# denyingmxd/CFPNet

Hardware: AMD Instinct MI355X
Metric: depth maps/sec @ 480x640 bf16 (whole job; per_gpu = value / n_gpus); abs_rel vs CPU oracle (higher is better)
Workload: dtype bf16; 1 GPU; batch=8 480x640 RGB + 8x8-zone ToF, eval forward incl. the prob output [B,256,H/2,W/2] written in the storage dtype (bf16: 2 bytes/element); layers=hist2image combine1 image x2 (CFPNet), parallelism=single GPU

## Files before the change

### cfpnet_amd/csrc/conv3x3_halo.hip

```cpp
#include "igemm_core.h"

namespace {

__device__ __attribute__((aligned(16))) unsigned int g_zero16h[4] = {0u, 0u, 0u, 0u};

using gptr_t = const __attribute__((address_space(1))) void*;
using lptr_t = __attribute__((address_space(3))) void*;
__device__ __forceinline__ void glds16(const void* g, unsigned char* lds_wave_base) {
  __builtin_amdgcn_global_load_lds((gptr_t)g, (lptr_t)lds_wave_base, 16, 0, 0);
}
template <int N> __device__ __forceinline__ void wait_vmcnt() { asm volatile("s_waitcnt vmcnt(%0)" ::"n"(N) : "memory"); }

struct HaloP {
  int PP;
  int CPT;
  int tiles_x, tiles_y;
  int n_blocks;
  FastDiv dcpt;
};

template <typename H, int NT, int WN, int STAGES, bool UP = false, int STRIDE = 1>
__global__ __launch_bounds__(256, 2) void conv3x3_halo_kernel(ConvP p, HaloP hp) {
  constexpr int WM = 4 / WN;
  constexpr int TH = 4 * WM;
  constexpr int HC = 15 * STRIDE + 3;
  constexpr int HPIX = ((TH - 1) * STRIDE + 3) * HC;
  static_assert(!(UP && STRIDE != 1), "the upsampling loader is stride 1");
  constexpr int NPAD = NT * WN * 16;
  constexpr int NBG = NPAD / 8;
  constexpr int NB = (NBG + 3) / 4;
  constexpr int WSTAGE = NPAD * 128;
  constexpr int LB = UP ? 4 : 6;
  static_assert((STAGES - 2) * NB <= 63, "vmcnt field");
  extern __shared__ __attribute__((aligned(16))) unsigned char smem[];
  unsigned char* sW = smem;
  unsigned char* sX = smem + STAGES * WSTAGE;

  const int tid = threadIdx.x;
  const int lane = tid & 63;
  const int wave = __builtin_amdgcn_readfirstlane(tid >> 6);
  const int wm = wave / WN, wn = wave % WN;
  const int fr = lane & 15, fq = lane >> 4;
  const int rsub = lane >> 3;
  const int lc = (lane & 7) ^ rsub;

  int bid = xcd_remap(blockIdx.x, gridDim.x);
  const int n_base = (bid % hp.n_blocks) * NPAD; bid /= hp.n_blocks;
  const int tx_ = bid % hp.tiles_x; bid /= hp.tiles_x;
  const int ty_ = bid % hp.tiles_y;
  const int b = bid / hp.tiles_y;
  const int x0 = tx_ * 16, y0 = ty_ * TH;

  const H* __restrict__ in = reinterpret_cast<const H*>(p.in) + (long long)b * p.H * p.W * p.in_ld;
  const H* __restrict__ wt = reinterpret_cast<const H*>(p.w);
  const H* zsrc = reinterpret_cast<const H*>(g_zero16h);
  const int nk = (p.K + 63) >> 6;

  const H* b_ptr[NB];
  unsigned b_okmask = 0;
#pragma unroll
  for (int j = 0; j < NB; ++j) {
    const int n = n_base + ((j * 4 + wave) % NBG) * 8 + rsub;
    const bool ok = n < p.Cout;
    if (ok) b_okmask |= 1u << j;
    b_ptr[j] = wt + (long long)(ok ? n : 0) * p.K;
  }
  auto issue = [&](int ks, int buf) {
    unsigned char* s = sW + buf * WSTAGE;
    const int kk = (ks * 8 + lc) * 8;
    const bool kok = kk < p.K;
#pragma unroll
    for (int j = 0; j < NB; ++j) {
      const bool ok = kok && ((b_okmask >> j) & 1u);
      glds16(ok ? b_ptr[j] + kk : zsrc, s + ((j * 4 + wave) % NBG) * 1024);
    }
  };
#pragma unroll
  for (int s = 0; s < STAGES - 1; ++s)
    if (s < nk) issue(s, s);

  {
    const int nitems = HPIX * hp.CPT;
    const H* __restrict__ low = nullptr;
    int upc = 0;
    if constexpr (UP) { low = reinterpret_cast<const H*>(p.up_src) + (long long)b * p.up_H * p.up_W * p.up_ld; upc = p.up_C >> 3; }
    for (int base = 0; base < nitems; base += 256 * LB) {
      u32x4 v[LB][UP ? 4 : 1];
      int dst[LB];
      float lyx[LB][UP ? 2 : 1];
      bool blend[LB];
#pragma unroll
      for (int n = 0; n < LB; ++n) {
        const int i = base + tid + n * 256;
        unsigned upx, uch;
        fd_rowcol((unsigned)i, hp.dcpt, upx, uch);
        const int px = (int)upx, ch = (int)uch;
        const int hy = px / HC, hx = px - hy * HC;
        const int y = y0 * STRIDE - p.pad_t + hy, x = x0 * STRIDE - p.pad_l + hx;
        const bool ok = i < nitems && (unsigned)y < (unsigned)p.H && (unsigned)x < (unsigned)p.W;
        dst[n] = i < nitems ? px * hp.PP + ch * 16 : -1;
        blend[n] = false;
#pragma unroll
        for (int t = 0; t < (UP ? 4 : 1); ++t) v[n][t] = u32x4{0u, 0u, 0u, 0u};
        if constexpr (UP) {
          if (ch < upc) {
            blend[n] = ok;
            const float fy = p.up_sy * (float)y, fx = p.up_sx * (float)x;
            const int ys = (int)fy, xs = (int)fx;
            lyx[n][0] = fy - (float)ys; lyx[n][1] = fx - (float)xs;
            if (ok) {
              const int dyo = (ys < p.up_H - 1 ? 1 : 0) * p.up_W * p.up_ld, dxo = (xs < p.up_W - 1 ? 1 : 0) * p.up_ld;
              const H* s00 = low + (ys * p.up_W + xs) * p.up_ld + ch * 8;
              v[n][0] = *reinterpret_cast<const u32x4*>(s00); v[n][1] = *reinterpret_cast<const u32x4*>(s00 + dxo);
              v[n][2] = *reinterpret_cast<const u32x4*>(s00 + dyo); v[n][3] = *reinterpret_cast<const u32x4*>(s00 + dyo + dxo);
            }
            continue;
          }
        }
        if (ok) v[n][0] = *reinterpret_cast<const u32x4*>(in + (y * p.W + x) * p.in_ld + ch * 8);
      }
#pragma unroll
      for (int n = 0; n < LB; ++n) {
        if (dst[n] < 0) continue;
        if constexpr (UP) {
          if (blend[n]) {
            float t[4][8], o[8];
#pragma unroll
            for (int q = 0; q < 4; ++q) Vec<H>::load(reinterpret_cast<const H*>(&v[n][q]), t[q]);
            const float ly1 = lyx[n][0], lx1 = lyx[n][1], ly0 = 1.f - ly1, lx0 = 1.f - lx1;
#pragma unroll
            for (int e = 0; e < 8; ++e) o[e] = ly0 * (lx0 * t[0][e] + lx1 * t[1][e]) + ly1 * (lx0 * t[2][e] + lx1 * t[3][e]);
            Vec<H>::store(reinterpret_cast<H*>(sX + dst[n]), o);
            continue;
          }
        }
        *reinterpret_cast<u32x4*>(sX + dst[n]) = v[n][0];
      }
    }
  }

  f32x4 acc[4][NT];
#pragma unroll
  for (int g = 0; g < 4; ++g)
#pragma unroll
    for (int j = 0; j < NT; ++j) acc[g][j] = f32x4{0.f, 0.f, 0.f, 0.f};

  const int ntap_chunks = 9 * hp.CPT;
  int c_cc, c_dx = 0, c_off = 0, c_idx = fq;
  {
    const int tap = fq / hp.CPT;
    c_cc = fq - tap * hp.CPT;
    c_dx = tap;
    while (c_dx >= 3) { c_dx -= 3; c_off += HC * hp.PP; }
    c_off += c_dx * hp.PP;
  }
  const unsigned char* xrow = sX + ((wm * 4 * STRIDE) * HC + fr * STRIDE) * hp.PP;
  const int growb = STRIDE * HC * hp.PP;

  for (int ks = 0; ks < nk; ++ks) {
    const int buf = ks % STAGES;
    const int ahead = min(nk - 1 - ks, STAGES - 2);
    if (ahead >= 2) wait_vmcnt<(STAGES > 3 ? 2 : 1) * NB>();
    else if (ahead == 1) wait_vmcnt<NB>();
    else wait_vmcnt<0>();
    asm volatile("s_waitcnt lgkmcnt(0)" ::: "memory");
    __builtin_amdgcn_s_barrier();
    asm volatile("" ::: "memory");
    if (ks + STAGES - 1 < nk) issue(ks + STAGES - 1, (ks + STAGES - 1) % STAGES);
    const unsigned char* cW = sW + buf * WSTAGE + (wn * NT * 16) * 128;
#pragma unroll
    for (int s = 0; s < 2; ++s) {
      s16x8 wf[NT], xf[4];
      const int pc = ((s * 4 + fq) ^ (fr & 7)) * 16;
#pragma unroll
      for (int j = 0; j < NT; ++j) wf[j] = *reinterpret_cast<const s16x8*>(cW + (j * 16 + fr) * 128 + pc);
      const bool live = c_idx < ntap_chunks;
      const int xo = c_off + c_cc * 16;
#pragma unroll
      for (int g = 0; g < 4; ++g) xf[g] = *reinterpret_cast<const s16x8*>(live ? xrow + g * growb + xo : sX);
#pragma unroll
      for (int g = 0; g < 4; ++g)
#pragma unroll
        for (int j = 0; j < NT; ++j) acc[g][j] = mfma16<H>(wf[j], xf[g], acc[g][j]);
      c_idx += 4;
      c_cc += 4;
      while (c_cc >= hp.CPT) {
        c_cc -= hp.CPT;
        c_off += hp.PP;
        if (++c_dx == 3) { c_dx = 0; c_off += (HC - 3) * hp.PP; }
      }
    }
  }

  H* __restrict__ out = reinterpret_cast<H*>(p.out) + (long long)b * p.Ho * p.Wo * p.out_ld;
  const H* __restrict__ res = p.res ? reinterpret_cast<const H*>(p.res) + (long long)b * p.Ho * p.Wo * p.res_ld : nullptr;
  const int x = x0 + fr;
  f32x4 sc[NT], sh[NT];
#pragma unroll
  for (int j = 0; j < NT; ++j) {
    const int n = n_base + (wn * NT + j) * 16 + fq * 4;
    const bool ok = n < p.Cout;
    sc[j] = (ok && p.scale) ? *reinterpret_cast<const f32x4*>(p.scale + n) : f32x4{1.f, 1.f, 1.f, 1.f};
    sh[j] = (ok && p.shift) ? *reinterpret_cast<const f32x4*>(p.shift + n) : f32x4{0.f, 0.f, 0.f, 0.f};
  }
  with_act(p.act, [&](auto A) {
#pragma unroll
    for (int g = 0; g < 4; ++g) {
      const int y = y0 + wm * 4 + g;
      const bool pix_ok = y < p.Ho && x < p.Wo;
      const long long pix = (long long)y * p.Wo + x;
#pragma unroll
      for (int j = 0; j < NT; ++j) {
        const int n = n_base + (wn * NT + j) * 16 + fq * 4;
        float yv[4];
#pragma unroll
        for (int r = 0; r < 4; ++r) yv[r] = act_c16<decltype(A)::value>(acc[g][j][r] * sc[j][r] + sh[j][r]);
        uint2 pk;
        pk.x = pack2<H>(yv[0], yv[1]);
        pk.y = pack2<H>(yv[2], yv[3]);
        if (!(pix_ok && n < p.Cout)) continue;
        if (res) {
          const uint2 rr = *reinterpret_cast<const uint2*>(res + pix * p.res_ld + n);
          const H* ph = reinterpret_cast<const H*>(&pk);
          const H* rh = reinterpret_cast<const H*>(&rr);
          float o[4];
#pragma unroll
          for (int r = 0; r < 4; ++r) o[r] = to_f32<H>(ph[r]) + to_f32<H>(rh[r]);
          H oh[4];
#pragma unroll
          for (int r = 0; r < 4; ++r) oh[r] = from_f32<H>(o[r]);
          pk = *reinterpret_cast<const uint2*>(oh);
        }
        *reinterpret_cast<uint2*>(out + pix * p.out_ld + n) = pk;
      }
    }
  });
}

int g_halo_odd_pitch = 0;
int g_halo_stages = 0;

struct HCfg { int nt, wn; };
constexpr HCfg kHCfg[] = {
    {1, 1},
    {2, 1},
    {4, 1},
    {2, 2},
    {4, 2},
    {5, 2},
    {7, 2},
    {1, 2},
};
constexpr int kNumHCfg = sizeof(kHCfg) / sizeof(kHCfg[0]);

template <typename H, int NT, int WN, bool UP = false, int STRIDE = 1>
int launch_h(const ConvP& p, hipStream_t s) {
  constexpr int TH = 4 * (4 / WN);
  constexpr int NPAD = NT * WN * 16;
  HaloP hp;
  hp.n_blocks = cdiv(p.Cout, NPAD);
  hp.CPT = p.Cin / 8;
  hp.dcpt = make_fastdiv((unsigned)hp.CPT);
  if ((long long)p.H * p.W * p.in_ld >= (1ll << 31)) return -1;
  int slots = hp.CPT;
  if (STRIDE == 1 && hp.CPT > 1) { while ((slots & 3) != 2) ++slots; }
  else if ((slots & 1) == 0) ++slots;
  if (g_halo_odd_pitch) { slots = hp.CPT; if ((slots & 1) == 0) ++slots; }
  hp.PP = slots * 16;
  hp.tiles_x = cdiv(p.Wo, 16); hp.tiles_y = cdiv(p.Ho, TH);
  const int hpix = ((TH - 1) * STRIDE + 3) * (15 * STRIDE + 3);
  const size_t halo = (size_t)hpix * hp.PP;
  const long long tiles = (long long)p.B * hp.tiles_x * hp.tiles_y * hp.n_blocks;
  int stages = g_halo_stages ? g_halo_stages : 2;
  const size_t lds = (size_t)stages * NPAD * 128 + halo;
  if (lds > 160 * 1024 || tiles >= (1ll << 31)) return -1;
#define HL(ST)                                                                                                                      \
  do {                                                                                                                              \
    auto k = conv3x3_halo_kernel<H, NT, WN, ST, UP, STRIDE>;                                                                        \
    static bool attr = false;                                                                                                       \
    if (!attr) { if (hipFuncSetAttribute((const void*)k, hipFuncAttributeMaxDynamicSharedMemorySize, 160 * 1024) != hipSuccess) return -2; attr = true; } \
    hipLaunchKernelGGL(k, dim3((unsigned)tiles), dim3(256), lds, s, p, hp);                                                         \
  } while (0)
  if constexpr (UP || STRIDE != 1) { HL(2); } else { if (stages == 4) HL(4); else if (stages == 3) HL(3); else HL(2); }
#undef HL
  return 0;
}

}

int conv3x3_halo_num_variants() { return kNumHCfg; }
void conv3x3_halo_debug_stages(int v) { g_halo_stages = v; }
void conv3x3_halo_debug_odd_pitch(int v) { g_halo_odd_pitch = v; }

bool conv3x3_halo_takes(const ConvP& p) {
  return p.KH == 3 && p.KW == 3 && (p.stride == 1 || (p.stride == 2 && p.up_src == nullptr)) && p.dil <= 1 && p.Cin % 8 == 0 && p.Cin >= 8 && p.Cin <= 128 && p.Cout % 8 == 0 &&
         p.Cout <= 512 && p.ln_gamma == nullptr && p.rows_per_batch == 0 && p.k2 == 0 && p.K == 9 * p.Cin &&
         p.pad_t >= 0 && p.pad_l >= 0 && p.pad_t <= 2 && p.pad_l <= 2;
}

int conv3x3_halo_launch(int v, const ConvP& p, hipStream_t s) {
  if (v < 0) {
    const long long t16 = (long long)p.B * cdiv(p.Wo, 16) * cdiv(p.Ho, 16);
    if (p.up_src != nullptr && p.Cout > 64) return -3;
    if (p.up_src != nullptr) v = p.Cout <= 32 ? 7 : 3;
    else if (p.Cout <= 16) v = 0;
    else if (p.Cout <= 32) v = t16 >= 1024 ? 1 : 7;
    else if (p.Cout <= 64) v = t16 >= 1024 ? 2 : 3;
    else if (p.Cout <= 128) v = 4;
    else if (p.Cout <= 160) v = 5;
    else v = 4;
  }
  if (v >= kNumHCfg) return -3;
  if (p.up_src != nullptr) {
#define HU(NT, WN) (p.f16 ? launch_h<f16_t, NT, WN, true>(p, s) : launch_h<bf16_t, NT, WN, true>(p, s))
    switch (v) {
      case 0: return HU(1, 1);
      case 1: return HU(2, 1);
      case 2: return HU(4, 1);
      case 3: return HU(2, 2);
      case 7: return HU(1, 2);
      default: return -3;
    }
#undef HU
  }
  if (p.stride == 2) {
#define HS(NT, WN) (p.f16 ? launch_h<f16_t, NT, WN, false, 2>(p, s) : launch_h<bf16_t, NT, WN, false, 2>(p, s))
    switch (v) {
      case 0: return HS(1, 1);
      case 1: return HS(2, 1);
      case 2: return HS(4, 1);
      case 3: return HS(2, 2);
      case 4: return HS(4, 2);
      case 5: return HS(5, 2);
      case 7: return HS(1, 2);
      default: return -3;
    }
#undef HS
  }
#define HV(NT, WN) (p.f16 ? launch_h<f16_t, NT, WN>(p, s) : launch_h<bf16_t, NT, WN>(p, s))
  switch (v) {
    case 0: return HV(1, 1);
    case 1: return HV(2, 1);
    case 2: return HV(4, 1);
    case 3: return HV(2, 2);
    case 4: return HV(4, 2);
    case 5: return HV(5, 2);
    case 6: return HV(7, 2);
    case 7: return HV(1, 2);
    default: return -3;
  }
#undef HV
}
```

### cfpnet_amd/csrc/igemm_core.h

```cpp
#pragma once
#include "common.h"

struct ConvP {
  const void* in;
  const void* w;
  void* out;
  const void* res;
  const float* scale;
  const float* shift;
  int in_ld, out_ld, res_ld;
  int B, H, W, Cin, Ho, Wo, Cout;
  int KH, KW, stride, pad_t, pad_l;
  int M, K;
  int act;
  int pointwise;
  const float* ln_gamma;
  const float* ln_beta;
  float ln_eps;
  int rows_per_batch;
  long long w_bstride;
  int f16;
  int k2;
  const void* up_src;
  int up_ld, up_C, up_H, up_W;
  float up_sy, up_sx;
  int probe;
  float* mom;
  int dil;
};

int igemm2_num_variants();
void igemm2_variant_shape(int v, int* bm, int* bn, int* stages);
int igemm2_launch(int v, const ConvP& p, float* slabs, int splits, hipStream_t s);

int igemm_x3_num_variants();
void igemm_x3_variant_shape(int v, int* bm, int* bn, int* stages);
constexpr int CFP_TICKET_SLOTS = 1024;
int igemm_x3_launch(int v, const ConvP& p, float* slabs, int splits, hipStream_t s, unsigned* tickets = nullptr);
int bin_head_x3_launch(const void* x, int x_ld, const void* w, const float* bias, const float* centers, float* prob, float* pred, int B, int HW,
                       int Cin, hipStream_t s);

int conv3x3_halo_x3_num_variants();
bool conv3x3_halo_x3_takes(const ConvP& p);
size_t conv3x3_halo_x3_lds(int v, const ConvP& p);
int conv3x3_halo_x3_launch(int v, const ConvP& p, hipStream_t s);

int conv3x3_num_variants();
void conv3x3_variant_shape(int v, int* th, int* bn);
int conv3x3_launch(int v, const ConvP& p, hipStream_t s);

int conv3x3_halo_num_variants();
void conv3x3_halo_debug_stages(int v);
void conv3x3_halo_debug_odd_pitch(int v);
bool conv3x3_halo_takes(const ConvP& p);
int conv3x3_halo_launch(int v, const ConvP& p, hipStream_t s);

template <typename T, int BN, int NTHR>
__device__ __forceinline__ void tile_moments(const T* sC, int CP, int rows_valid, int n0, int Cout, float* __restrict__ mom_tile, int tid) {
  constexpr int TPC = NTHR / BN;
  static_assert(NTHR % BN == 0 && TPC >= 1 && TPC <= 64 && (TPC & (TPC - 1)) == 0, "threads per channel");
  const int c = tid / TPC, part = tid % TPC;
  const float shift = to_f32<T>(sC[c]);
  float n = 0.f, s1 = 0.f, s2 = 0.f;
  for (int r = part; r < rows_valid; r += TPC) {
    const float v = to_f32<T>(sC[r * CP + c]) - shift;
    s1 += v; s2 = fmaf(v, v, s2); n += 1.f;
  }
  float mean = n > 0.f ? shift + s1 / n : 0.f;
  float m2 = n > 0.f ? fmaxf(s2 - s1 * s1 / n, 0.f) : 0.f;
#pragma unroll
  for (int o = 1; o < TPC; o <<= 1) {
    const float bn = __shfl_xor(n, o, 64), bmean = __shfl_xor(mean, o, 64), bm2 = __shfl_xor(m2, o, 64);
    const bool up = (part & o) != 0;
    const float an = up ? bn : n, amean = up ? bmean : mean, am2 = up ? bm2 : m2;
    const float cn = up ? n : bn, cmean = up ? mean : bmean, cm2 = up ? m2 : bm2;
    const float tn = an + cn;
    if (tn > 0.f) {
      const float d = cmean - amean, f = cn / tn;
      mean = amean + d * f; m2 = am2 + cm2 + d * d * an * f; n = tn;
    } else { mean = 0.f; m2 = 0.f; n = 0.f; }
  }
  if (part == 0 && n0 + c < Cout) { mom_tile[n0 + c] = mean; mom_tile[Cout + n0 + c] = m2; }
}

__device__ __forceinline__ int swz(int row, int chunk) {
  int q = (row >> 2) & 3;
  int g = (4 - q) & 3;
  return chunk ^ g;
}

template <typename T, int BM, int BN, int WM, int WN>
__device__ __forceinline__ void igemm_mainloop(const ConvP& p, int m0, int n0, int ks_begin, int ks_end,
                                               unsigned char* smem, f32x4 (&acc)[BM / WM / 16][BN / WN / 16]) {
  constexpr int VE = Vec<T>::N;
  constexpr int BK = 4 * VE;
  constexpr int TM = BM / WM / 16;
  constexpr int TN = BN / WN / 16;
  constexpr int A_ROWS = BM / 64;
  constexpr int B_ROWS = (BN + 63) / 64;
  constexpr bool kBf16 = sizeof(T) == 2;
  auto sA = [&](int st) -> unsigned char* { return smem + st * ((BM + BN) * 64); };
  auto sB = [&](int st) -> unsigned char* { return smem + st * ((BM + BN) * 64) + BM * 64; };

  const int tid = threadIdx.x;
  const int lane = tid & 63;
  const int wave = tid >> 6;
  const int wm = wave / WN, wn = wave % WN;

  const T* __restrict__ in = reinterpret_cast<const T*>(p.in);
  const T* __restrict__ wt = reinterpret_cast<const T*>(p.w);

  const int ld_row = tid >> 2;
  const int ld_chunk = tid & 3;
  long long a_base[A_ROWS];
  int a_hi0[A_ROWS], a_wi0[A_ROWS];
  bool a_ok[A_ROWS];
#pragma unroll
  for (int i = 0; i < A_ROWS; ++i) {
    int m = m0 + ld_row + 64 * i;
    a_ok[i] = m < p.M;
    int mm = a_ok[i] ? m : 0;
    if (p.pointwise) {
      a_base[i] = (long long)mm * p.in_ld;
      a_hi0[i] = 0;
      a_wi0[i] = 0;
    } else {
      int wo = mm % p.Wo;
      int t = mm / p.Wo;
      int ho = t % p.Ho;
      int b = t / p.Ho;
      a_hi0[i] = ho * p.stride - p.pad_t;
      a_wi0[i] = wo * p.stride - p.pad_l;
      a_base[i] = (long long)b * p.H * p.W * p.in_ld;
    }
  }
  bool b_ok[B_ROWS];
  long long b_base[B_ROWS];
#pragma unroll
  for (int i = 0; i < B_ROWS; ++i) {
    int r = ld_row + 64 * i;
    int n = n0 + r;
    b_ok[i] = (r < BN) && (n < p.Cout);
    b_base[i] = (long long)(b_ok[i] ? n : 0) * p.K;
  }

  u32x4 ra[A_ROWS], rb[B_ROWS];
  const u32x4 zero4 = {0u, 0u, 0u, 0u};

  int t_k = -1, t_cc = 0, t_kh = 0, t_kw = 0;
  const bool dil_pow2 = (p.dil & (p.dil - 1)) == 0;
  const int dil_shift = 31 - __clz(p.dil);
  auto load_tiles = [&](int k0) {
    int k = k0 + ld_chunk * VE;
    bool kok = k < p.K;
    int kh = 0, kw = 0, cc = k;
    if (!p.pointwise) {
      if (k == t_k + BK && t_k >= 0) {
        t_cc += BK;
        while (t_cc >= p.Cin) {
          t_cc -= p.Cin;
          if (++t_kw == p.KW) { t_kw = 0; ++t_kh; }
        }
      } else {
        int tap = k / p.Cin;
        t_cc = k - tap * p.Cin;
        t_kh = tap / p.KW;
        t_kw = tap - t_kh * p.KW;
      }
      t_k = k;
      cc = t_cc; kh = t_kh; kw = t_kw;
    }
#pragma unroll
    for (int i = 0; i < A_ROWS; ++i) {
      int hi = a_hi0[i] + kh, wi = a_wi0[i] + kw;
      bool ok = a_ok[i] && kok;
      long long off = a_base[i] + cc;
      if (!p.pointwise) {
        if (p.dil > 1 && dil_pow2) {
          ok = ok && hi >= 0 && wi >= 0 && ((hi | wi) & (p.dil - 1)) == 0;
          hi >>= dil_shift; wi >>= dil_shift;
        } else if (p.dil > 1) {
          ok = ok && hi >= 0 && wi >= 0 && hi % p.dil == 0 && wi % p.dil == 0;
          hi /= p.dil; wi /= p.dil;
        }
        ok = ok && hi >= 0 && hi < p.H && wi >= 0 && wi < p.W;
        off += ((long long)hi * p.W + wi) * p.in_ld;
      }
      ra[i] = ok ? *reinterpret_cast<const u32x4*>(in + off) : zero4;
    }
#pragma unroll
    for (int i = 0; i < B_ROWS; ++i) {
      rb[i] = (b_ok[i] && kok) ? *reinterpret_cast<const u32x4*>(wt + b_base[i] + k) : zero4;
    }
  };
  auto store_tiles = [&](int st) {
#pragma unroll
    for (int i = 0; i < A_ROWS; ++i) {
      int r = ld_row + 64 * i;
      *reinterpret_cast<u32x4*>(sA(st) + r * 64 + swz(r, ld_chunk) * 16) = ra[i];
    }
#pragma unroll
    for (int i = 0; i < B_ROWS; ++i) {
      int r = ld_row + 64 * i;
      if (r < BN) *reinterpret_cast<u32x4*>(sB(st) + r * 64 + swz(r, ld_chunk) * 16) = rb[i];
    }
  };

#pragma unroll
  for (int i = 0; i < TM; ++i)
#pragma unroll
    for (int j = 0; j < TN; ++j) acc[i][j] = f32x4{0.f, 0.f, 0.f, 0.f};

  load_tiles(ks_begin * BK);
  store_tiles(0);
  __syncthreads();

  const int fr = lane & 15;
  const int fq = lane >> 4;

  for (int ks = ks_begin; ks < ks_end; ++ks) {
    const int st = (ks - ks_begin) & 1;
    if (ks + 1 < ks_end) load_tiles((ks + 1) * BK);

    const unsigned char* cA = sA(st) + (wm * (BM / WM)) * 64;
    const unsigned char* cB = sB(st) + (wn * (BN / WN)) * 64;
    if constexpr (kBf16) {
      s16x8 af[TM], bfr[TN];
#pragma unroll
      for (int i = 0; i < TM; ++i) {
        int r = i * 16 + fr;
        af[i] = *reinterpret_cast<const s16x8*>(cA + r * 64 + swz(r, fq) * 16);
      }
#pragma unroll
      for (int j = 0; j < TN; ++j) {
        int r = j * 16 + fr;
        bfr[j] = *reinterpret_cast<const s16x8*>(cB + r * 64 + swz(r, fq) * 16);
      }
#pragma unroll
      for (int i = 0; i < TM; ++i)
#pragma unroll
        for (int j = 0; j < TN; ++j)
          acc[i][j] = mfma16<T>(af[i], bfr[j], acc[i][j]);
    } else {
#pragma unroll
      for (int kk = 0; kk < 4; ++kk) {
        float af[TM], bfr[TN];
#pragma unroll
        for (int i = 0; i < TM; ++i) {
          int r = i * 16 + fr;
          af[i] = *reinterpret_cast<const float*>(cA + r * 64 + swz(r, kk) * 16 + fq * 4);
        }
#pragma unroll
        for (int j = 0; j < TN; ++j) {
          int r = j * 16 + fr;
          bfr[j] = *reinterpret_cast<const float*>(cB + r * 64 + swz(r, kk) * 16 + fq * 4);
        }
#pragma unroll
        for (int i = 0; i < TM; ++i)
#pragma unroll
          for (int j = 0; j < TN; ++j)
            acc[i][j] = __builtin_amdgcn_mfma_f32_16x16x4f32(af[i], bfr[j], acc[i][j], 0, 0, 0);
      }
    }
    if (ks + 1 < ks_end) store_tiles(st ^ 1);
    __syncthreads();
  }
}
```

### cfpnet_amd/engine.py

```python
from __future__ import annotations

import math
import os
from typing import Dict, List, Optional, Sequence, Tuple

import torch

from . import hip, ops, spec
from .geometry import FusionGeometry, gsa_keys
from .ops import Act

_BN_EPS = 1e-5


def _same_pad(size: int, k: int, s: int) -> Tuple[int, int]:
    total = max((math.ceil(size / s) - 1) * s + k - size, 0)
    return total // 2, total - total // 2


_STREAMS: Dict = {}
_CONCURRENT: Dict[str, list] = {}


def concurrent_streams(device, want: int = 4, pool: int = 16) -> list:
    import time
    key = str(torch.device(device))
    got = _CONCURRENT.get(key)
    if got is not None and len(got) >= want:
        return got[:want]
    cand = [torch.cuda.Stream(device=device) for _ in range(pool)]
    cycles = 1_000_000
    if not hasattr(torch.cuda, "_sleep"):
        _CONCURRENT[key] = cand[:max(want, 4)]
        return _CONCURRENT[key][:want]

    def spin(ids):
        torch.cuda.synchronize(device)
        t0 = time.perf_counter()
        for i in ids:
            with torch.cuda.stream(cand[i]):
                torch.cuda._sleep(cycles)
        torch.cuda.synchronize(device)
        return time.perf_counter() - t0

    spin([0])
    base = min(spin([0]) for _ in range(3))
    chosen = [0]
    for j in range(1, pool):
        if len(chosen) >= want:
            break
        if all(min(spin([k, j]) for _ in range(2)) < 1.5 * base for k in chosen):
            chosen.append(j)
    _CONCURRENT[key] = [cand[i] for i in chosen]
    return _CONCURRENT[key][:want]


def _shared_stream(device, role):
    key = (str(torch.device(device)), role)
    st = _STREAMS.get(key)
    if st is None:
        if isinstance(role, tuple) and role[0] == "lane":
            conc = concurrent_streams(device)
            st = conc[role[1] % len(conc)]
        else:
            st = torch.cuda.Stream(device=device)
        _STREAMS[key] = st
    return st


class Engine:
    def __init__(self, state_dict: Dict[str, torch.Tensor], *, layer_names: Sequence[str], n_bins: int = 256,
                 min_val: float = 1e-3, max_val: float = 10.0, norm: str = "linear", change_embedding: bool = True,
                 no_skip_inside: bool = False, stem_act: bool = False, dtype=None, device="cuda:0",
                 zone_sample_num: int = 16, base_resolution=spec.BASE_RESOLUTION, x3: Optional[bool] = None):
        if dtype is None:
            dtype, x3 = torch.float32, (True if x3 is None else x3)
        x3 = bool(x3)
        hip.load()
        self.base_resolution = tuple(base_resolution)
        self.fusion = spec.fusion_table(self.base_resolution)
        if not torch.cuda.is_available():
            raise RuntimeError("cfpnet_amd.Engine needs a GPU: the product path has no CPU fallback")
        assert dtype in (torch.bfloat16, torch.float16, torch.float32)
        self.layer_names = list(layer_names)
        self.n_bins, self.min_val, self.max_val = n_bins, float(min_val), float(max_val)
        self.norm = {"linear": 0, "softmax": 1, "sigmoid": 2}[norm]
        self.change_embedding, self.no_skip_inside, self.stem_act = change_embedding, no_skip_inside, stem_act
        self.dtype, self.device = dtype, torch.device(device)
        assert not x3 or dtype == torch.float32, "x3 is a matrix-math mode of float32 storage"
        self.x3 = bool(x3)
        self.cdt = hip.F32X3 if self.x3 else ops.DT[dtype]
        self.tickets = self.x3 and os.environ.get("CFP_SPLITK_TICKETS", "0") == "1"
        self.zone_sample_num = zone_sample_num
        self.weights2 = os.environ.get("CFP_WEIGHTS2", "0") == "1"
        self.diffuse_cin = os.environ.get("CFP_DIFFUSE_CIN", "1") == "1"
        self.mbconv_fused = os.environ.get("CFP_MBCONV_FUSED", "0") == "1"
        self.se2 = dtype in (torch.bfloat16, torch.float16) and os.environ.get("CFP_SE2", "1") == "1"
        self.se2_x3 = os.environ.get("CFP_SE2_X3", "1") if self.x3 else "0"
        self._dbg_round = {}
        for item in filter(None, os.environ.get("CFP_DEBUG_ROUND", "").split(",")):
            n, d = item.split(":")
            self._dbg_round[n] = {"f16": torch.float16, "bf16": torch.bfloat16}[d]
        self.up_fused = os.environ.get("CFP_UP_FUSED", "4")
        self.up_fused_x3 = os.environ.get("CFP_UP_FUSED_X3", "")
        self.cat_pad = os.environ.get("CFP_CAT_PAD", "1") == "1" and not self.up_fused_x3
        self.lkpm_fused = os.environ.get("CFP_LKPM_FUSED", "1") != "0"
        self.tail_q = os.environ.get("CFP_TAIL_Q", "1") == "1"
        self.lkpm_min_rows = int(os.environ.get("CFP_LKPM_MIN_ROWS", "30000"))
        self.sr_ln_fused = os.environ.get("CFP_SR_LN_FUSED", "1") == "1"
        self.head_fused = os.environ.get("CFP_HEAD_FUSED", "1") != "0"
        hl = os.environ.get("CFP_HEAD_HILO", "00")
        self.head_hilo = (hl[0] == "1", hl[1] == "1")
        self.half = dtype in (torch.bfloat16, torch.float16)
        self.ve = 8 if self.half else 4
        self.P: Dict[str, torch.Tensor] = {}
        self._plans: Dict[tuple, dict] = {}
        self._graph = None
        self._splitk_ws: Optional[torch.Tensor] = None
        self._capturing = False
        self._side = _shared_stream(self.device, "side")
        self._lane = 0
        self.use_side_stream = os.environ.get("CFP_NO_SIDE_STREAM", "0") != "1"
        self._lane_streams: Dict[int, Tuple[torch.cuda.Stream, torch.cuda.Stream]] = {}
        self._lanes_active = 1
        self._slots = None
        self._slot_next = 0
        self._lane_ws: Dict[int, torch.Tensor] = {}
        self.load_state_dict(state_dict)

    def _dev(self, t: torch.Tensor, dtype=None) -> torch.Tensor:
        return t.detach().to(device=self.device, dtype=dtype or torch.float32).contiguous()

    def _pack_conv(self, w: torch.Tensor, w2: bool = False) -> torch.Tensor:
        w = w.detach().float()
        if w.dim() == 2:
            w = w[:, :, None, None]
        elif w.dim() == 3:
            w = w[:, :, :, None]
        co, ci, kh, kw = w.shape
        if kh * kw > 1:
            w = ops.round_taps(w, self.dtype)
        cip = (ci + 7) // 8 * 8
        if cip != ci:
            w = torch.nn.functional.pad(w, (0, 0, 0, 0, 0, cip - ci))
        flat = w.permute(0, 2, 3, 1).reshape(co, kh * kw * cip)
        if w2 and self.weights2 and self.half and kh * kw == 1:
            return ops.pack_w2(flat, self.dtype).to(self.device)
        if kh * kw == 1 and self.diffuse_cin and self.dtype == torch.float16:
            flat = ops.round_taps(flat.reshape(co, 1, kh * kw * cip), self.dtype).reshape(co, -1)
        if self.x3:
            return ops.pack_w_x3(self._dev(flat))
        return self._dev(flat, self.dtype)

    def _fold_bn(self, sd, bn: Optional[str], bias: Optional[torch.Tensor], co: int, eps: float):
        if bn is None:
            scale = torch.ones(co)
            shift = bias.detach().float().clone() if bias is not None else torch.zeros(co)
        else:
            g, b = sd[bn + ".weight"].float(), sd[bn + ".bias"].float()
            m, v = sd[bn + ".running_mean"].float(), sd[bn + ".running_var"].float()
            scale = g / torch.sqrt(v + eps)
            shift = b - m * scale
            if bias is not None:
                shift = shift + bias.detach().float() * scale
        return self._dev(scale), self._dev(shift)

    def _conv(self, sd, name: str, wkey: str, bkey: Optional[str] = None, bn: Optional[str] = None, eps: float = _BN_EPS, w2: bool = True):
        w = sd[wkey]
        self.P[name + ".w"] = self._pack_conv(w, w2)
        s, t = self._fold_bn(sd, bn, sd[bkey] if bkey else None, w.shape[0], eps)
        self.P[name + ".s"], self.P[name + ".t"] = s, t

    def _loftr_pack(self, sd, p: str, self_attn: bool):
        D = sd[p + ".q_proj.weight"].shape[0]
        if self_attn:
            self.P[p + ".qkv"] = self._pack_conv(torch.cat([sd[p + ".q_proj.weight"], sd[p + ".k_proj.weight"], sd[p + ".v_proj.weight"]], 0), True)
        else:
            self.P[p + ".q"] = self._pack_conv(sd[p + ".q_proj.weight"], True)
        self.P[p + ".kv"] = self._pack_conv(torch.cat([sd[p + ".k_proj.weight"], sd[p + ".v_proj.weight"]], 0), True)
        self.P[p + ".q1"] = self._pack_conv(sd[p + ".q_proj.weight"])
        self.P[p + ".merge"] = self._pack_conv(sd[p + ".merge.weight"])
        self.P[p + ".mlp0"] = self._pack_conv(sd[p + ".mlp.0.weight"])
        self.P[p + ".mlp2"] = self._pack_conv(sd[p + ".mlp.2.weight"])
        for n in ("norm1", "norm2"):
            self.P[f"{p}.{n}.g"], self.P[f"{p}.{n}.b"] = self._dev(sd[f"{p}.{n}.weight"]), self._dev(sd[f"{p}.{n}.bias"])

    def load_state_dict(self, sd: Dict[str, torch.Tensor]):
        self.P.clear()
        self._graph = None
        e = "img_encoder"
        EPS = spec.ENC_BN_EPS
        self._conv(sd, "stem", f"{e}.conv0.0.weight", bn=f"{e}.conv0.1", eps=EPS)
        self.rgb_hilo = self.half and os.environ.get("CFP_RGB_HILO", "1") == "1"
        if self.rgb_hilo:
            w = self.P["stem.w"].reshape(-1, 9, 8).clone()
            w[:, :, 3:6] = w[:, :, 0:3]
            self.P["stem.w"] = w.reshape(w.shape[0], 72).contiguous()
        for b in spec.ENC_BLOCKS:
            q = f"{e}.{b.prefix}"
            if b.kind == "cn":
                self._conv(sd, q + ".conv", q + ".conv.weight", bn=q + ".bn1", eps=EPS)
            elif b.kind == "er":
                self._conv(sd, q + ".exp", q + ".conv_exp.weight", bn=q + ".bn1", eps=EPS)
                self._conv(sd, q + ".pwl", q + ".conv_pwl.weight", bn=q + ".bn2", eps=EPS)
            else:
                self._conv(sd, q + ".pw", q + ".conv_pw.weight", bn=q + ".bn1", eps=EPS)
                if self.half and self.mbconv_fused and b.stride == 1 and not self.weights2:
                    self.P[q + ".pw.wimg"] = ops.pack_mbconv_pw(self.P[q + ".pw.w"].float().cpu(), self.dtype).to(self.device)
                wd = ops.round_taps(sd[q + ".conv_dw.weight"].float(), self.dtype)
                self.P[q + ".dw.w"] = self._dev(wd.reshape(wd.shape[0], 9).t(), self.dtype)
                self.P[q + ".dw.s"], self.P[q + ".dw.t"] = self._fold_bn(sd, q + ".bn2", None, wd.shape[0], EPS)
                self.P[q + ".se.wr"] = self._dev(sd[q + ".se.conv_reduce.weight"].reshape(b.se_rd, b.mid))
                self.P[q + ".se.br"] = self._dev(sd[q + ".se.conv_reduce.bias"])
                self.P[q + ".se.we_t"] = self._dev(sd[q + ".se.conv_expand.weight"].reshape(b.mid, b.se_rd).t())
                self.P[q + ".se.be"] = self._dev(sd[q + ".se.conv_expand.bias"])
                self._conv(sd, q + ".pwl", q + ".conv_pwl.weight", bn=q + ".bn3", eps=EPS, w2=False)
                self.P[q + ".pwl.w32"] = self._dev(sd[q + ".conv_pwl.weight"].reshape(b.cout, b.mid))
        parts, layout, off = [], [], 0
        for ex in (1, 2, 3):
            q = f"hist_encoder.hist_extractor{ex}.pointnet_encoder"
            for j in (1, 2, 3):
                w = sd[f"{q}.conv{j}.weight"].detach().float()
                w = w.reshape(w.shape[0], -1)
                co, ci = w.shape
                sc, sh = self._fold_bn(sd, f"{q}.bn{j}", sd[f"{q}.conv{j}.bias"], co, _BN_EPS)
                row = []
                for t in (w.reshape(-1), sc.cpu(), sh.cpu()):
                    row.append(off)
                    parts.append(t.reshape(-1).cpu())
                    off += (t.numel() + 3) // 4 * 4
                    if t.numel() % 4:
                        parts.append(torch.zeros(4 - t.numel() % 4))
                layout.append((row[0], row[1], row[2], ci, co))
        self.P["hist.blob"] = self._dev(torch.cat(parts))
        self._hist_layout = layout
        d = "decoder"
        self._conv(sd, d + ".conv4", d + ".conv4.weight", d + ".conv4.bias")
        for i in (1, 2, 3, 4):
            q = f"{d}.up{i}._net"
            if self.x3 and self.cat_pad:
                wfull = sd[q + ".0.weight"]
                cpad = (wfull.shape[1] + 31) // 32 * 32
                self.P[f"{d}.up{i}.a.wpad"] = self._pack_conv(torch.nn.functional.pad(wfull.detach().float(), (0, 0, 0, 0, 0, cpad - wfull.shape[1])))
            self._conv(sd, f"{d}.up{i}.a", q + ".0.weight", q + ".0.bias", bn=q + ".1")
            if self.x3 and str(i) in self.up_fused_x3:
                wfull = sd[q + ".0.weight"].detach().float()
                cup = wfull.shape[1] - spec.DEC_ENC_CH[i]
                self.P[f"{d}.up{i}.a.wcat"] = ops.pack_w_x3_cat(self._dev(wfull.permute(0, 2, 3, 1).contiguous()), cup)
            self._conv(sd, f"{d}.up{i}.b", q + ".3.weight", q + ".3.bias", bn=q + ".4")
        for n in ("conv3", "conv2", "conv1", "conv0"):
            self._conv(sd, f"{d}.{n}", f"{d}.{n}.weight", f"{d}.{n}.bias")
        for name in self.fusion:
            q = f"{d}.{name}"
            self.P[q + ".pe"] = self._dev(sd[q + ".positional_encodings"])
            self.P[q + ".pe2"] = self._dev(sd[q + ".positional_encodings2"])
            for i, ln in enumerate(self.layer_names):
                l = f"{q}.layers.{i}"
                if ln == "hist2image":
                    self._loftr_pack(sd, l, False)
                elif ln == "image":
                    self._loftr_pack(sd, l + ".lga.encoder_layer", True)
                    self._loftr_pack(sd, l + ".gsa.encoder_layer", False)
                    self._conv(sd, l + ".gsa.sr", l + ".gsa.sr.weight", l + ".gsa.sr.bias")
                    self.P[l + ".gsa.norm.g"], self.P[l + ".gsa.norm.b"] = self._dev(sd[l + ".gsa.norm.weight"]), self._dev(sd[l + ".gsa.norm.bias"])
                elif ln == "combine1":
                    t = l + ".transformer_path"
                    self.P[t + ".qkv"] = self._pack_conv(torch.cat([sd[t + ".q_proj.weight"], sd[t + ".k_proj.weight"], sd[t + ".v_proj.weight"]], 0), True)
                    self._conv(sd, t + ".conv1", t + ".conv1.weight", bn=t + ".bn1")
                    self._conv(sd, t + ".conv2", t + ".conv2.weight", bn=t + ".bn2")
                    k = l + ".large_kernel_path"
                    wd = sd[k + ".dwconv2.weight"].float()
                    kk = wd.shape[-1]
                    self.P[k + ".dw.w"] = self._dev(wd[:, 0].transpose(1, 2).reshape(wd.shape[0], kk * kk))
                    if self.half and kk in (7, 15, 31):
                        self.P[k + ".dw.tb"] = ops.toeplitz_bands(wd, self.dtype).to(self.device)
                    elif self.x3 and kk in (7, 15, 31) and os.environ.get("CFP_X3_DWLARGE", "1") != "0":
                        self.P[k + ".dw.tb"] = ops.toeplitz_bands_x3(wd).to(self.device)
                    self.P[k + ".dw.s"], self.P[k + ".dw.t"] = self._fold_bn(sd, k + ".bn1", sd[k + ".dwconv2.bias"], wd.shape[0], _BN_EPS)
                    self.P[k + ".norm.g"], self.P[k + ".norm.b"] = self._dev(sd[k + ".norm.weight"]), self._dev(sd[k + ".norm.bias"])
                    self._conv(sd, k + ".pw1", k + ".pwconv1.weight", k + ".pwconv1.bias")
                    self._conv(sd, k + ".pw2", k + ".pwconv2.weight", k + ".pwconv2.bias")
                else:
                    raise NotImplementedError(ln)
        h = "depth_head"
        w0 = sd[d + ".conv0.weight"].detach().float()
        self.P[d + ".conv0.w32"] = self._dev(w0.permute(0, 2, 3, 1).reshape(w0.shape[0], -1))
        self.P[d + ".conv0.b32"] = self._dev(sd[d + ".conv0.bias"])
        self._conv(sd, h + ".conv3x3", h + ".conv3x3.weight", h + ".conv3x3.bias")
        self.P[h + ".w1x1"] = self._dev(sd[h + ".conv1x1.weight"].reshape(128, 128).t())
        for i in (0, 2, 4):
            self.P[f"{h}.r{i}.w"], self.P[f"{h}.r{i}.b"] = self._dev(sd[f"{h}.regressor.{i}.weight"].t()), self._dev(sd[f"{h}.regressor.{i}.bias"])
        self._conv(sd, "conv_out", "conv_out.0.weight", "conv_out.0.bias", w2=False)
        if self.half and self.n_bins == 256:
            self.P["conv_out.wp"] = ops.permute_wout(sd["conv_out.0.weight"], self.dtype, hilo=self.head_hilo[0],
                                                   diffuse=self.diffuse_cin and self.dtype == torch.float16).to(self.device)

    def _act(self, plan, key: str, rows: int, C: int, ld: Optional[int] = None, zero: bool = False) -> Act:
        bufs = plan["bufs"]
        if key not in bufs:
            bufs[key] = ops.new_act(rows, C, self.dtype, self.device, ld, zero)
        a = bufs[key]
        assert a.rows == rows and a.ld == (ld or C), key
        return Act(a.buf, 0, C)

    def _buf(self, plan, key: str, shape, dtype, zero: bool = False) -> torch.Tensor:
        bufs = plan["bufs"]
        if key not in bufs:
            bufs[key] = (torch.zeros if zero else torch.empty)(shape, dtype=dtype, device=self.device)
        assert tuple(bufs[key].shape) == tuple(shape), key
        return bufs[key]

    def _f32(self, plan, key: str, n: int) -> torch.Tensor:
        bufs = plan["bufs"]
        if key not in bufs:
            bufs[key] = torch.empty(max(n, 1), dtype=torch.float32, device=self.device)
        assert bufs[key].numel() >= n, key
        return bufs[key]

    def _cv(self, name, x: Act, out: Act, B, H, W, k, stride=1, pads=None, act=hip.ACT_NONE, residual=None):
        if pads is None:
            p = (k - 1) // 2
            pt = pl = p
            Ho, Wo = (H + 2 * p - k) // stride + 1, (W + 2 * p - k) // stride + 1
        else:
            (pt, pb), (pl, pr) = pads
            Ho, Wo = (H + pt + pb - k) // stride + 1, (W + pl + pr - k) // stride + 1
        ops.conv2d(x, self.P[name + ".w"], self.P[name + ".s"], self.P[name + ".t"], out, B, H, W, k, k, stride, pt, pl,
                   Ho, Wo, act, residual, self._ws(B * Ho * Wo, out.C, k * k * x.C))
        return Ho, Wo

    def _lin(self, wname, x: Act, out: Act, rows, act=hip.ACT_NONE, residual=None, st: Optional[str] = None, ln=None):
        ops.linear(x, self.P[wname], self.P[st + ".s"] if st else None, self.P[st + ".t"] if st else None, out, rows, act, residual,
                   None if ln is not None else self._ws(rows, out.C, x.C), ln)

    def _ws(self, M: int, Cout: int, K: int) -> Optional[torch.Tensor]:
        need = ops.conv2d_ws_bytes(M, Cout, K, self.cdt)
        if need == 0:
            return None
        if self.tickets:
            need += hip.CONV_TICKET_BYTES
        ws = self._lane_ws.get(self._lane)
        if ws is None or ws.numel() * 4 < need:
            if self._capturing:
                raise RuntimeError("split-K workspace must be sized by a warm-up forward before graph capture")
            if self.tickets:
                ws = ops.ticket_ws(need - hip.CONV_TICKET_BYTES, self.device)
            else:
                ws = torch.empty((need + 3) // 4, dtype=torch.float32, device=self.device)
            self._lane_ws[self._lane] = ws
        return ws

    def _dbg(self, name: str, a: Act):
        if self._dbg_round:
            for pat, dt in self._dbg_round.items():
                if name == pat or (pat.endswith("*") and name.startswith(pat[:-1])):
                    t = a.torch()
                    t.copy_(t.to(dt).to(t.dtype))

    def _encoder(self, plan, rgb: torch.Tensor, B, H, W, taps):
        e = "img_encoder"
        x8 = self._act(plan, "rgb8", B * H * W, 8)
        (ops.rgb_to_nhwc8_hilo if self.rgb_hilo else ops.rgb_to_nhwc8)(rgb, x8, B, H, W)
        pads = (_same_pad(H, 3, 2), _same_pad(W, 3, 2))
        h, w = math.ceil(H / 2), math.ceil(W / 2)
        x = self._act(plan, "stem", B * h * w, spec.ENC_STEM_OUT)
        self._cv("stem", x8, x, B, H, W, 3, 2, pads, hip.ACT_SILU if self.stem_act else hip.ACT_NONE)
        self._dbg("stem", x)
        tap_acts: List[Act] = []
        for bi, b in enumerate(spec.ENC_BLOCKS):
            q = f"{e}.{b.prefix}"
            ho, wo = math.ceil(h / b.stride), math.ceil(w / b.stride)
            pads = (_same_pad(h, 3, b.stride), _same_pad(w, 3, b.stride))
            if bi in spec.ENC_TAPS:
                out = plan["tap_dst"][spec.ENC_TAPS[bi]]
            else:
                out = self._act(plan, f"enc{bi}", B * ho * wo, b.cout)
            res = x if b.skip else None
            if b.kind == "cn":
                self._cv(q + ".conv", x, out, B, h, w, 3, b.stride, pads, hip.ACT_SILU, res)
            elif b.kind == "er":
                mid = self._act(plan, f"enc{bi}.mid", B * ho * wo, b.mid)
                self._cv(q + ".exp", x, mid, B, h, w, 3, b.stride, pads, hip.ACT_SILU)
                self._dbg(f"enc{bi}.mid", mid)
                self._cv(q + ".pwl", mid, out, B, ho, wo, 1, 1, None, hip.ACT_NONE, res)
            else:
                mid2 = self._act(plan, f"enc{bi}.dw", B * ho * wo, b.mid)
                mbp = ops.mbconv_plan(B, h, w, x.C, b.mid) if (q + ".pw.wimg") in self.P else None
                if mbp is not None:
                    ns = mbp[0]
                    part = self._f32(plan, f"enc{bi}.sum", B * ns * b.mid)
                    ops.mbconv_expand_dw(x, self.P[q + ".pw.wimg"], self.P[q + ".pw.s"], self.P[q + ".pw.t"], self.P[q + ".dw.w"],
                                         self.P[q + ".dw.s"], self.P[q + ".dw.t"], mid2, part, B, h, w)
                elif ((self.se2 or self.se2_x3 == "1" or (self.se2_x3 == "auto" and not ops.PLAN_IN_FLIGHT)) and b.se_rd <= 64
                      and ops.dwconv3x3_se_parts(B, ho, wo, b.mid, b.stride, ops.DT[self.dtype]) > 0):
                    mid = self._act(plan, f"enc{bi}.mid", B * h * w, b.mid)
                    self._cv(q + ".pw", x, mid, B, h, w, 1, 1, None, hip.ACT_SILU)
                    K = ops.dwconv3x3_se_parts(B, ho, wo, b.mid, b.stride, ops.DT[self.dtype])
                    hpart = self._f32(plan, f"enc{bi}.hpart", B * K * b.se_rd)
                    ops.dwconv3x3_se(mid, self.P[q + ".dw.w"], self.P[q + ".dw.s"], self.P[q + ".dw.t"], mid2, self.P[q + ".se.wr"], hpart,
                                     B, h, w, b.stride, pads[0][0], pads[1][0], ho, wo, hip.ACT_SILU)
                    if self.x3:
                        wb = self._buf(plan, f"enc{bi}.wb", (B, b.cout, (b.mid + 31) // 32 * 64), torch.float16, zero=True)
                    else:
                        wb = self._buf(plan, f"enc{bi}.wb", (B, b.cout, b.mid), self.dtype)
                    ops.se_gate_fold2(hpart, K, 1.0 / (ho * wo), self.P[q + ".se.br"], self.P[q + ".se.we_t"], self.P[q + ".se.be"],
                                      self.P[q + ".pwl.w32"], wb, B, b.cout, b.mid, b.se_rd, x3=self.x3)
                    ops.conv2d(mid2, wb, self.P[q + ".pwl.s"], self.P[q + ".pwl.t"], out, B, ho, wo, 1, 1, 1, 0, 0, ho, wo, hip.ACT_NONE,
                               res, self._piw_ws(plan, bi, B, ho * wo, b.cout, b.mid), per_image_weights=True)
                    x, h, w = out, ho, wo
                    if bi in spec.ENC_TAPS:
                        tap_acts.append(out)
                        if taps is not None:
                            taps[f"enc{spec.ENC_TAPS[bi]}"] = self._nchw(out, B, h, w)
                    continue
                else:
                    mid = self._act(plan, f"enc{bi}.mid", B * h * w, b.mid)
                    self._cv(q + ".pw", x, mid, B, h, w, 1, 1, None, hip.ACT_SILU)
                    ns = ops.dwconv3x3_strips(B, ho, wo, b.mid, b.stride, ops.DT[self.dtype])
                    part = self._f32(plan, f"enc{bi}.sum", B * ns * b.mid)
                    self._dbg(f"enc{bi}.mid", mid)
                    ops.dwconv3x3_sum(mid, self.P[q + ".dw.w"], self.P[q + ".dw.s"], self.P[q + ".dw.t"], mid2, part, B, h, w, b.stride,
                                      pads[0][0], pads[1][0], ho, wo, hip.ACT_SILU)
                    self._dbg(f"enc{bi}.dw", mid2)
                if self.x3:
                    wb = self._buf(plan, f"enc{bi}.wb", (B, b.cout, (b.mid + 31) // 32 * 64), torch.float16, zero=True)
                else:
                    wb = self._buf(plan, f"enc{bi}.wb", (B, b.cout, b.mid), self.dtype)
                ops.se_gate_fold(part, ns, 1.0 / (ho * wo), self.P[q + ".se.wr"], self.P[q + ".se.br"], self.P[q + ".se.we_t"],
                                 self.P[q + ".se.be"], self.P[q + (".pwl.w32" if self.x3 else ".pwl.w")], wb, B, b.cout, b.mid, b.se_rd)
                ops.conv2d(mid2, wb, self.P[q + ".pwl.s"], self.P[q + ".pwl.t"], out, B, ho, wo, 1, 1, 1, 0, 0, ho, wo, hip.ACT_NONE,
                           res, self._piw_ws(plan, bi, B, ho * wo, b.cout, b.mid), per_image_weights=True)
            self._dbg(f"enc{bi}", out)
            x, h, w = out, ho, wo
            if bi in spec.ENC_TAPS:
                tap_acts.append(out)
                if taps is not None:
                    taps[f"enc{spec.ENC_TAPS[bi]}"] = self._nchw(out, B, h, w)
        return tap_acts

    def _hist_encoder(self, plan, hist: torch.Tensor, R: int, taps):
        outs = [self._act(plan, f"hist.{ex}", R, c) for ex, c in zip((1, 2, 3), spec.HIST_CHANNELS)]
        self._hist_pe_fused = taps is None and os.environ.get("CFP_NO_PE_FUSE", "0") != "1"
        pe = [self.P[f"decoder.cross_atten{ex}.pe2"] for ex in (1, 2, 3)] if self._hist_pe_fused else (None, None, None)
        ops.hist_encoder(hist.reshape(-1), self.P["hist.blob"], self._hist_layout, outs, R, pe, self.zone_sample_num)
        if taps is not None:
            for ex, o in enumerate(outs):
                taps[f"hist{ex}"] = o.torch().float().cpu()
        return outs

    def _kv_state(self, plan, tag, p, src: Act, rows_s, D, heads, kvmode: dict):
        d = D // heads
        kvb = self._act(plan, f"{tag}.kvsrc", rows_s, 2 * D)
        self._lin(p + ".kv", src, kvb, rows_s)
        G = kvmode["groups"]
        kv = self._f32(plan, f"{tag}.kv", G * heads * d * d)
        ks = self._f32(plan, f"{tag}.ks", G * heads * d)
        nws = ops.attn_kv_ws_floats(kvmode["NB"], kvmode["Hk"], kvmode["Wk"], kvmode["th"], kvmode["tw"], heads, d)
        ws = self._f32(plan, f"{tag}.kvws", nws)
        ops.attn_kv_reduce(kvb.slice(0, D), kvb.slice(D, D), kv, ks, ws, kvmode["NB"], kvmode["Hk"], kvmode["Wk"], kvmode["th"], kvmode["tw"],
                           kvmode["clip"], kvmode["count_pad"], kvmode["v_length"], heads, d)
        return kv, ks

    def _loftr(self, plan, tag, p, xb: Act, rows_q, src: Optional[Act], rows_s, heads, out: Act, kvmode: dict, apmode: dict, pre=None):
        D = xb.C // 2
        d = D // heads
        x = xb.slice(0, D)
        qb = self._act(plan, f"{tag}.qkv", rows_q, 3 * D)
        fused_tail = self.half or (self.x3 and os.environ.get("CFP_X3_TAIL", "1") != "0")
        tail_q = fused_tail and self.tail_q
        if pre is not None and tail_q:
            kv, ks = pre
            ops.loftr_tail(None, kv, ks, x, out, self.P[p + ".q1"], self.P[p + ".merge"], self.P[p + ".mlp0"], self.P[p + ".mlp2"],
                           (self.P[p + ".norm1.g"], self.P[p + ".norm1.b"]), (self.P[p + ".norm2.g"], self.P[p + ".norm2.b"]),
                           apmode["NB"], apmode["Hq"], apmode["Wq"], apmode["qth"], apmode["qtw"], kvmode["v_length"], heads)
            return
        if src is None and tail_q:
            self._lin(p + ".kv", x, qb.slice(D, 2 * D), rows_q)
            kA, vA = qb.slice(D, D), qb.slice(2 * D, D)
        elif src is None:
            self._lin(p + ".qkv", x, qb, rows_q)
            kA, vA = qb.slice(D, D), qb.slice(2 * D, D)
        else:
            if not tail_q:
                self._lin(p + ".q", x, qb.slice(0, D), rows_q)
            kvb = self._act(plan, f"{tag}.kvsrc", rows_s, 2 * D)
            self._lin(p + ".kv", src, kvb, rows_s)
            kA, vA = kvb.slice(0, D), kvb.slice(D, D)
        G = kvmode["groups"]
        kv = self._f32(plan, f"{tag}.kv", G * heads * d * d)
        ks = self._f32(plan, f"{tag}.ks", G * heads * d)
        nws = ops.attn_kv_ws_floats(kvmode["NB"], kvmode["Hk"], kvmode["Wk"], kvmode["th"], kvmode["tw"], heads, d)
        ws = self._f32(plan, f"{tag}.kvws", nws)
        ops.attn_kv_reduce(kA, vA, kv, ks, ws, kvmode["NB"], kvmode["Hk"], kvmode["Wk"], kvmode["th"], kvmode["tw"],
                           kvmode["clip"], kvmode["count_pad"], kvmode["v_length"], heads, d)
        if fused_tail:
            ops.loftr_tail(None if tail_q else qb.slice(0, D), kv, ks, x, out, self.P[p + ".q1"] if tail_q else None,
                           self.P[p + ".merge"], self.P[p + ".mlp0"], self.P[p + ".mlp2"],
                           (self.P[p + ".norm1.g"], self.P[p + ".norm1.b"]), (self.P[p + ".norm2.g"], self.P[p + ".norm2.b"]),
                           apmode["NB"], apmode["Hq"], apmode["Wq"], apmode["qth"], apmode["qtw"], kvmode["v_length"], heads)
            return
        msg = self._act(plan, f"{tag}.msg", rows_q, D)
        ops.attn_apply(qb.slice(0, D), kv, ks, msg, apmode["NB"], apmode["Hq"], apmode["Wq"], apmode["qth"], apmode["qtw"],
                       (0, 0, 0, 0), kvmode["v_length"], heads, d)
        self._lin(p + ".merge", msg, xb.slice(D, D), rows_q, ln=(self.P[p + ".norm1.g"], self.P[p + ".norm1.b"], 1e-5))
        hid = self._act(plan, f"{tag}.hid", rows_q, 2 * D)
        self._lin(p + ".mlp0", xb, hid, rows_q, hip.ACT_RELU)
        self._lin(p + ".mlp2", hid, out, rows_q, residual=x, ln=(self.P[p + ".norm2.g"], self.P[p + ".norm2.b"], 1e-5))

    def _piw_ws(self, plan, bi: int, B: int, hw: int, cout: int, k: int):
        if not self.x3:
            return None
        _, sp = ops.conv2d_plan(B * hw, cout, k, hip.F32X3, hw, B, 1, 1)
        if sp <= 1:
            return None
        if not self.tickets:
            return self._f32(plan, f"enc{bi}.piw_ws", sp * B * hw * cout)
        bufs, key = plan["bufs"], f"enc{bi}.piw_ws"
        if key not in bufs:
            bufs[key] = ops.ticket_ws(sp * B * hw * cout * 4, self.device)
        return bufs[key]

    def _fusion(self, plan, name: str, x: Act, feat1: Act, zone_valid: torch.Tensor, geo: FusionGeometry, B, H, W, out: Act,
                pos_offset, taps):
        D, (Hm, Wm), lk = self.fusion[name]
        p = f"decoder.{name}"
        ws = spec.window_size((Hm, Wm))
        M = B * H * W
        Z = geo.zone_num * geo.zone_num
        N = self.zone_sample_num
        tok = [self._act(plan, f"{name}.tokA", M, 2 * D), self._act(plan, f"{name}.tokB", M, 2 * D)]
        cur = 0
        if torch.is_tensor(pos_offset):
            assert pos_offset.dtype == torch.int32 and pos_offset.numel() == 2 and pos_offset.is_cuda
            d0 = tok[0].slice(0, D)
            hip.call("cfp_add_rowtable_dev", x.ptr, x.ld, self.P[p + ".pe"].data_ptr(), d0.ptr, d0.ld, M, x.C, H, W, Hm, Wm,
                     pos_offset.data_ptr(), x.dt, hip.current_stream())
        else:
            oy, ox = pos_offset
            ops.add_rowtable(x, self.P[p + ".pe"], tok[0].slice(0, D), M, H, W, Wm, oy, ox)
        emb0 = None
        if not self.change_embedding:
            emb0 = self._act(plan, f"{name}.emb0", M, D)
            ops.copy_rows(tok[0].slice(0, D), emb0, M)
        if self._hist_pe_fused:
            src = feat1
        else:
            src = self._act(plan, f"{name}.src", B * Z * N, D)
            ops.add_rowtable(feat1, self.P[p + ".pe2"], src, B * Z * N, 1, N, N, 0, 0)
        gh, gw = geo.grid_h, geo.grid_w
        Mz = B * gh * gw
        y0, y1, x0, x1 = geo.clipped(H, W)
        rect = (geo.sy_wo, geo.sx_wo, geo.tzh, geo.tzw)

        last = len(self.layer_names) - 1
        direct_out = False
        for i, ln in enumerate(self.layer_names):
            l = f"{p}.layers.{i}"
            tag = f"{name}.L{i}"
            final_dst = out if (i == last and taps is None and os.environ.get("CFP_NO_DIRECT_OUT", "0") != "1") else None
            if ln == "hist2image":
                zin = self._act(plan, f"{name}.zin", Mz, 2 * D)
                zsrc = tok[cur].slice(0, D) if self.change_embedding else emb0
                ops.resize_bilinear(zsrc, H, W, rect, zin.slice(0, D), gh, gw, (0, 0, gh, gw), B)
                zout = self._act(plan, f"{name}.zout", Mz, D)
                self._loftr(plan, f"{name}.x2i", l, zin, Mz, src, B * Z * N, spec.X2I_HEADS, zout,
                            dict(groups=B * Z, NB=B * Z, Hk=1, Wk=N, th=1, tw=N, clip=(0, 1, 0, N), count_pad=False, v_length=float(N)),
                            dict(NB=B, Hq=gh, Wq=gw, qth=geo.p1, qtw=geo.p2), pre=plan.get("x2i_kv", {}).get((name, i)))
                ops.resize_bilinear(zout, gh, gw, (0, 0, gh, gw), tok[cur].slice(0, D), H, W, rect, B, zone_valid=zone_valid,
                                    zn=geo.zone_num, p1=geo.p1, p2=geo.p2, accumulate=not self.no_skip_inside)
            elif ln == "image":
                nh, nw = math.ceil(H / ws), math.ceil(W / ws)
                self._loftr(plan, f"{name}.lsa", l + ".lga.encoder_layer", tok[cur], M, None, 0, spec.TWINS_HEADS, tok[cur ^ 1].slice(0, D),
                            dict(groups=B * nh * nw, NB=B, Hk=H, Wk=W, th=ws, tw=ws, clip=(0, H, 0, W), count_pad=True, v_length=float(ws * ws)),
                            dict(NB=B, Hq=H, Wq=W, qth=ws, qtw=ws))
                cur ^= 1
                hk, wk = gsa_keys(H, W, ws)
                keys = self._act(plan, f"{name}.gsa.keys", B * hk * wk, D)
                if self.x3 and self.sr_ln_fused:
                    ops.conv2d(tok[cur].slice(0, D), self.P[l + ".gsa.sr.w"], self.P[l + ".gsa.sr.s"], self.P[l + ".gsa.sr.t"], keys,
                               B, H, W, ws, ws, ws, 0, 0, hk, wk, ws=self._ws(B * hk * wk, D, ws * ws * D),
                               ln=(self.P[l + ".gsa.norm.g"], self.P[l + ".gsa.norm.b"], 1e-5))
                else:
                    kraw = self._act(plan, f"{name}.gsa.kraw", B * hk * wk, D)
                    ops.conv2d(tok[cur].slice(0, D), self.P[l + ".gsa.sr.w"], self.P[l + ".gsa.sr.s"], self.P[l + ".gsa.sr.t"], kraw,
                               B, H, W, ws, ws, ws, 0, 0, hk, wk, ws=self._ws(B * hk * wk, D, ws * ws * D))
                    ops.layernorm(kraw, self.P[l + ".gsa.norm.g"], self.P[l + ".gsa.norm.b"], 1e-5, keys, B * hk * wk)
                S = hk * wk
                self._loftr(plan, f"{name}.gsa", l + ".gsa.encoder_layer", tok[cur], M, keys, B * S, spec.TWINS_HEADS,
                            final_dst if final_dst is not None else tok[cur ^ 1].slice(0, D),
                            dict(groups=B, NB=B, Hk=1, Wk=S, th=1, tw=S, clip=(0, 1, 0, S), count_pad=False, v_length=float(S)),
                            dict(NB=B, Hq=H, Wq=W, qth=H, qtw=W))
                cur ^= 1
                direct_out = final_dst is not None
            elif ln == "combine1":
                t = l + ".transformer_path"
                heads = spec.X2I_HEADS
                d = D // heads
                xin = tok[cur]
                qb = self._act(plan, f"{name}.dapm.qkv", M, 3 * D)
                self._lin(t + ".qkv", xin.slice(0, D), qb, M)
                n_in = (y1 - y0) * (x1 - x0)
                kv = self._f32(plan, f"{name}.dapm.kv", B * heads * d * d)
                ks = self._f32(plan, f"{name}.dapm.ks", B * heads * d)
                wsb = self._f32(plan, f"{name}.dapm.ws", ops.attn_kv_ws_floats(B, H, W, H, W, heads, d))
                ops.attn_kv_reduce(qb.slice(D, D), qb.slice(2 * D, D), kv, ks, wsb, B, H, W, H, W, (y0, y1, x0, x1), False,
                                   float(max(n_in, 1)), heads, d)
                ops.attn_apply(qb.slice(0, D), kv, ks, xin.slice(D, D), B, H, W, H, W, (y0, y1, x0, x1), float(max(n_in, 1)), heads, d)
                c1 = self._act(plan, f"{name}.dapm.c1", M, D)
                self._cv(t + ".conv1", xin, c1, B, H, W, 3)
                self._cv(t + ".conv2", c1, tok[cur ^ 1].slice(0, D), B, H, W, 3, residual=xin.slice(0, D))
                cur ^= 1
                k = l + ".large_kernel_path"
                xin = tok[cur]
                t1 = self._act(plan, f"{name}.lk.t1", M, D)
                if (k + ".dw.tb") in self.P:
                    ops.dwconv_large_mfma(xin.slice(0, D), self.P[k + ".dw.tb"], self.P[k + ".dw.s"], self.P[k + ".dw.t"], t1, B, H, W, lk,
                                          hip.ACT_RELU)
                else:
                    ops.dwconv_large(xin.slice(0, D), self.P[k + ".dw.w"], self.P[k + ".dw.s"], self.P[k + ".dw.t"], t1, B, H, W, lk, hip.ACT_RELU)
                lk_dst = final_dst if final_dst is not None else tok[cur ^ 1].slice(0, D)
                if ((self.half and not self.weights2) or (self.x3 and os.environ.get("CFP_X3_TAIL", "1") != "0")) and self.lkpm_fused and D in (32, 64, 128) and M >= self.lkpm_min_rows:
                    ops.lkpm_tail(t1, xin.slice(0, D), lk_dst, self.P[k + ".pw1.w"], self.P[k + ".pw1.t"], self.P[k + ".pw2.w"], self.P[k + ".pw2.t"],
                                  self.P[k + ".norm.g"], self.P[k + ".norm.b"], M)
                else:
                    t2 = self._act(plan, f"{name}.lk.t2", M, D)
                    ops.layernorm(t1, self.P[k + ".norm.g"], self.P[k + ".norm.b"], 1e-6, t2, M)
                    h4 = self._act(plan, f"{name}.lk.h4", M, 4 * D)
                    self._lin(k + ".pw1.w", t2, h4, M, hip.ACT_GELU, None, k + ".pw1")
                    self._lin(k + ".pw2.w", h4, lk_dst, M, hip.ACT_NONE, xin.slice(0, D), k + ".pw2")
                cur ^= 1
                direct_out = final_dst is not None
            else:
                raise NotImplementedError(ln)
            if taps is not None:
                taps[f"{p}.layers.{i}"] = tok[cur].slice(0, D).torch().float().cpu().reshape(B, H * W, D)
        if not direct_out:
            ops.copy_rows(tok[cur].slice(0, D), out, M)

    def _nchw(self, a: Act, B, H, W) -> torch.Tensor:
        return a.torch().float().cpu().reshape(B, H, W, a.C).permute(0, 3, 1, 2).contiguous()

    @torch.no_grad()
    def forward_lanes(self, input_data: dict, lanes: int, *, return_prob: bool = True, pos_offsets: Optional[dict] = None):
        rgb = input_data["rgb"]
        B = rgb.shape[0]
        lanes = max(1, min(lanes, B))
        if lanes == 1:
            return self.forward(input_data, return_prob=return_prob, pos_offsets=pos_offsets)
        dev = self.device
        add = input_data["additional"]
        H, W = rgb.shape[-2:]
        edges = torch.empty(B, self.n_bins + 1, dtype=torch.float32, device=dev)
        pred = torch.empty(B, 1, H // 2, W // 2, dtype=torch.float32, device=dev)
        prob = torch.empty(B, self.n_bins, H // 2, W // 2, dtype=self.dtype, device=dev) if return_prob else None
        main = torch.cuda.current_stream(dev)
        bounds = [B * i // lanes for i in range(lanes + 1)]
        for i in range(lanes):
            if i not in self._lane_streams and i > 0:
                self._lane_streams[i] = (_shared_stream(dev, ("lane", i)), _shared_stream(dev, ("lane-side", i)))
        rgb_d = rgb.to(device=dev, dtype=torch.float32).contiguous()
        hist_d = add["hist_data"].to(device=dev, dtype=torch.float32).contiguous()
        mask_d = add["mask"].to(device=dev).to(torch.uint8).contiguous()
        self._lanes_active = lanes
        for i in range(lanes):
            b0, b1 = bounds[i], bounds[i + 1]
            sub = {"rgb": rgb_d[b0:b1], "additional": {"hist_data": hist_d[b0:b1], "mask": mask_d[b0:b1],
                                                       "rect_data": add.get("rect_data"), "patch_info": add["patch_info"]}}
            outs = (edges[b0:b1], pred[b0:b1], prob[b0:b1] if prob is not None else None)
            if i == 0:
                self.forward(sub, return_prob=return_prob, pos_offsets=pos_offsets, lane=0, out=outs)
            else:
                st = self._lane_streams[i][0]
                st.wait_stream(main)
                with torch.cuda.stream(st):
                    self.forward(sub, return_prob=return_prob, pos_offsets=pos_offsets, lane=i, out=outs)
        for i in range(1, lanes):
            main.wait_stream(self._lane_streams[i][0])
        self._lane = 0
        self._lanes_active = 1
        return edges, pred, prob

    def capture(self, input_data: dict, *, return_prob: bool = True, pos_offsets: Optional[dict] = None, lanes: int = 1,
                inflight: int = 1, adopt_inputs: bool = False):
        dev = self.device
        add = input_data["additional"]
        B = input_data["rgb"].shape[0]
        H, W = input_data["rgb"].shape[-2:]
        lanes = max(1, min(lanes, B))
        self._slots = None
        self._slot_next = 0
        if inflight > 1:
            return self._capture_inflight(input_data, inflight, return_prob, pos_offsets)
        if adopt_inputs:
            assert lanes == 1, "adopt_inputs: single-graph capture only"
            m = add["mask"]
            for t, dts in ((input_data["rgb"], (torch.float32,)), (add["hist_data"], (torch.float32,)), (m, (torch.uint8, torch.bool))):
                assert t.device == dev and t.dtype in dts and t.is_contiguous(), "adopt_inputs: device tensors in the kernels' own types"
            static = {"rgb": input_data["rgb"], "additional": {"hist_data": add["hist_data"], "mask": m.view(torch.uint8) if m.dtype == torch.bool else m,
                                                               "rect_data": add.get("rect_data"), "patch_info": add["patch_info"]}}
        else:
            static = {"rgb": input_data["rgb"].to(device=dev, dtype=torch.float32).contiguous().clone(),
                      "additional": {"hist_data": add["hist_data"].to(device=dev, dtype=torch.float32).contiguous().clone(),
                                     "mask": add["mask"].to(device=dev).to(torch.uint8).contiguous().clone(),
                                     "rect_data": add.get("rect_data"), "patch_info": add["patch_info"]}}
        edges = torch.empty(B, self.n_bins + 1, dtype=torch.float32, device=dev)
        pred = torch.empty(B, 1, H // 2, W // 2, dtype=torch.float32, device=dev)
        prob = torch.empty(B, self.n_bins, H // 2, W // 2, dtype=self.dtype, device=dev) if return_prob else None
        bounds = [B * i // lanes for i in range(lanes + 1)]
        subs, outs = [], []
        for i in range(lanes):
            b0, b1 = bounds[i], bounds[i + 1]
            sa = static["additional"]
            subs.append({"rgb": static["rgb"][b0:b1], "additional": {"hist_data": sa["hist_data"][b0:b1], "mask": sa["mask"][b0:b1],
                                                                     "rect_data": sa["rect_data"], "patch_info": sa["patch_info"]}})
            outs.append((edges[b0:b1], pred[b0:b1], prob[b0:b1] if prob is not None else None))
            if i not in self._lane_streams:
                self._lane_streams[i] = (_shared_stream(dev, ("lane", i)), _shared_stream(dev, ("lane-side", i)))
        graphs = []
        self._graph = None
        self._lanes_active = lanes
        cur = torch.cuda.current_stream(dev)
        for i in range(lanes):
            st = self._lane_streams[i][0]
            st.wait_stream(cur)
            with torch.cuda.stream(st):
                for _ in range(2):
                    self.forward(subs[i], return_prob=return_prob, pos_offsets=pos_offsets, lane=i, out=outs[i])
            torch.cuda.synchronize(dev)
            g = torch.cuda.CUDAGraph()
            self._capturing = True
            try:
                with torch.cuda.graph(g, stream=st):
                    self.forward(subs[i], return_prob=return_prob, pos_offsets=pos_offsets, lane=i, out=outs[i])
            finally:
                self._capturing = False
            graphs.append(g)
        torch.cuda.synchronize(dev)
        self._lane = 0
        self._lanes_active = 1
        self._graph = (graphs, static, (edges, pred, prob))
        return edges, pred, prob

    def plan_mode(self, throughput: bool):
        ops.PLAN_IN_FLIGHT = bool(throughput) and os.environ.get("CFP_TPUT_PLAN", "1") != "0"

    def _capture_inflight(self, input_data, inflight, return_prob, pos_offsets):
        self.plan_mode(True)
        try:
            return self._capture_inflight_impl(input_data, inflight, return_prob, pos_offsets)
        finally:
            self.plan_mode(False)

    def _capture_inflight_impl(self, input_data, inflight, return_prob, pos_offsets):
        dev = self.device
        add = input_data["additional"]
        B = input_data["rgb"].shape[0]
        H, W = input_data["rgb"].shape[-2:]
        streams = concurrent_streams(dev, want=inflight)
        self._graph = None
        self._lanes_active = max(2, len(streams))
        cur = torch.cuda.current_stream(dev)
        slots = []
        for si, st in enumerate(streams):
            static = {"rgb": input_data["rgb"].to(device=dev, dtype=torch.float32).contiguous().clone(),
                      "additional": {"hist_data": add["hist_data"].to(device=dev, dtype=torch.float32).contiguous().clone(),
                                     "mask": add["mask"].to(device=dev).to(torch.uint8).contiguous().clone(),
                                     "rect_data": add.get("rect_data"), "patch_info": add["patch_info"]}}
            out = (torch.empty(B, self.n_bins + 1, dtype=torch.float32, device=dev),
                   torch.empty(B, 1, H // 2, W // 2, dtype=torch.float32, device=dev),
                   torch.empty(B, self.n_bins, H // 2, W // 2, dtype=self.dtype, device=dev) if return_prob else None)
            st.wait_stream(cur)
            with torch.cuda.stream(st):
                for _ in range(2):
                    self.forward(static, return_prob=return_prob, pos_offsets=pos_offsets, lane=si, out=out)
            torch.cuda.synchronize(dev)
            g = torch.cuda.CUDAGraph()
            self._capturing = True
            try:
                with torch.cuda.graph(g, stream=st):
                    self.forward(static, return_prob=return_prob, pos_offsets=pos_offsets, lane=si, out=out)
            finally:
                self._capturing = False
            slots.append({"graph": g, "static": static, "out": out, "stream": st, "event": torch.cuda.Event()})
        torch.cuda.synchronize(dev)
        self._lane = 0
        self._lanes_active = 1
        self._slots = slots
        return slots[0]["out"]

    def replay_async(self, input_data: Optional[dict] = None):
        dev = self.device
        cur = torch.cuda.current_stream(dev)
        if not self._slots:
            out = self.replay(input_data)
            ev = torch.cuda.Event()
            ev.record(cur)
            return out, ev
        slot = self._slots[self._slot_next % len(self._slots)]
        self._slot_next += 1
        st = slot["stream"]
        with torch.cuda.stream(st):
            if input_data is not None:
                st.wait_stream(cur)
                static = slot["static"]
                static["rgb"].copy_(input_data["rgb"], non_blocking=True)
                static["additional"]["hist_data"].copy_(input_data["additional"]["hist_data"], non_blocking=True)
                static["additional"]["mask"].copy_(input_data["additional"]["mask"].to(torch.uint8), non_blocking=True)
            slot["graph"].replay()
            slot["event"].record(st)
        return slot["out"], slot["event"]

    def capture_best(self, input_data: dict, *, return_prob: bool = True, pos_offsets: Optional[dict] = None,
                     candidates: Sequence = (("lanes", 1), ("inflight", 2), ("inflight", 3), ("inflight", 4), ("inflight", 6)),
                     reps: int = 16, allow_inflight: bool = True):
        import time
        B = input_data["rgb"].shape[0]
        times = {}
        seen = []
        for kind, n in candidates:
            n = max(1, int(n))
            if kind == "lanes":
                n = min(n, B)
            elif not allow_inflight:
                continue
            if (kind, n) in seen:
                continue
            seen.append((kind, n))
            last = f"{kind}:{n}"
            if kind == "lanes":
                self.capture(input_data, return_prob=return_prob, pos_offsets=pos_offsets, lanes=n)
                run = self.replay
            else:
                self.capture(input_data, return_prob=return_prob, pos_offsets=pos_offsets, inflight=n)
                if len(self._slots) < n:
                    continue
                run = self.replay_async
            for _ in range(2 * n + 2):
                run()
            torch.cuda.synchronize(self.device)
            t0 = time.perf_counter()
            for _ in range(reps):
                run()
            torch.cuda.synchronize(self.device)
            times[f"{kind}:{n}"] = (time.perf_counter() - t0) / reps * 1e3
        best = min(times, key=times.get)
        kind, n = best.split(":")
        n = int(n)
        if best != last:
            if kind == "lanes":
                self.capture(input_data, return_prob=return_prob, pos_offsets=pos_offsets, lanes=n)
            else:
                self.capture(input_data, return_prob=return_prob, pos_offsets=pos_offsets, inflight=n)
        return (kind, n), times

    def replay(self, input_data: Optional[dict] = None):
        if self._slots:
            out, ev = self.replay_async(input_data)
            torch.cuda.current_stream(self.device).wait_event(ev)
            return out
        if self._graph is None:
            raise RuntimeError("Engine.replay() before capture()")
        graphs, static, out = self._graph
        dev = self.device
        cur = torch.cuda.current_stream(dev)
        if input_data is not None:
            static["rgb"].copy_(input_data["rgb"], non_blocking=True)
            static["additional"]["hist_data"].copy_(input_data["additional"]["hist_data"], non_blocking=True)
            m = input_data["additional"]["mask"]
            if m.dtype == torch.bool and m.is_cuda:
                static["additional"]["mask"].view(torch.bool).copy_(m, non_blocking=True)
            else:
                static["additional"]["mask"].copy_(m.to(torch.uint8), non_blocking=True)
        if len(graphs) == 1:
            st = self._lane_streams[0][0]
            st.wait_stream(cur)
            with torch.cuda.stream(st):
                graphs[0].replay()
            cur.wait_stream(st)
            return out
        for i, g in enumerate(graphs):
            st = self._lane_streams[i][0]
            st.wait_stream(cur)
            with torch.cuda.stream(st):
                g.replay()
        for i in range(len(graphs)):
            cur.wait_stream(self._lane_streams[i][0])
        return out

    def _plan(self, B, H, W) -> dict:
        key = (B, H, W, self._lane)
        if key not in self._plans:
            self._plans[key] = {"bufs": {}}
        return self._plans[key]

    @torch.no_grad()
    def forward(self, input_data: dict, *, return_prob: bool = True, pos_offsets: Optional[dict] = None,
                taps: Optional[dict] = None, img_features: Optional[Sequence[torch.Tensor]] = None, lane: int = 0,
                out: Optional[tuple] = None):
        self._lane = lane
        side = self._lane_streams[lane][1] if lane in self._lane_streams else self._side
        if not self.use_side_stream or self._lanes_active > 1:
            side = torch.cuda.current_stream(self.device)
        rgb = input_data["rgb"]
        add = input_data["additional"]
        B, _, H, W = rgb.shape
        assert H % 32 == 0 and W % 32 == 0, "input height/width must be multiples of 32"
        dev = self.device
        plan = self._plan(B, H, W)
        pos_offsets = pos_offsets or {}
        hs = [H // 2, H // 4, H // 8, H // 16, H // 32]
        wsz = [W // 2, W // 4, W // 8, W // 16, W // 32]
        e, c = spec.DEC_ENC_CH, spec.DEC_CH
        cp = (lambda n: (n + 31) // 32 * 32) if (self.x3 and self.cat_pad) else (lambda n: n)
        zc = self.x3 and self.cat_pad
        cat = [None,
               self._act(plan, "cat1", B * hs[3] * wsz[3], cp(c[0] + e[1]), zero=zc),
               self._act(plan, "cat2", B * hs[2] * wsz[2], cp(c[1] + e[2]), zero=zc),
               self._act(plan, "cat3", B * hs[1] * wsz[1], cp(c[2] + e[3]), zero=zc),
               self._act(plan, "cat4", B * hs[0] * wsz[0], cp(c[3] + e[4]), zero=zc)]
        b4 = self._act(plan, "tap4", B * hs[4] * wsz[4], e[0])
        plan["tap_dst"] = [cat[4].slice(c[3], e[4]), cat[3].slice(c[2], e[3]), cat[2].slice(c[1], e[2]),
                           cat[1].slice(c[0], e[1]), b4]
        main = torch.cuda.current_stream(dev)
        hist = add["hist_data"].to(device=dev, dtype=torch.float32).contiguous()
        zone_valid = add["mask"].to(device=dev).to(torch.uint8).contiguous()
        Z, N = hist.shape[1], hist.shape[2]
        side.wait_stream(main)
        with torch.cuda.stream(side):
            hfeat = self._hist_encoder(plan, hist, B * Z * N, taps)
            plan["x2i_kv"] = {}
            if (self.half or (self.x3 and os.environ.get("CFP_X3_TAIL", "1") != "0")) and self.tail_q and self._hist_pe_fused and os.environ.get("CFP_X2I_HOIST", "1") == "1":
                for fname, feat in (("cross_atten3", hfeat[2]), ("cross_atten2", hfeat[1]), ("cross_atten1", hfeat[0])):
                    D = self.fusion[fname][0]
                    for i, ln in enumerate(self.layer_names):
                        if ln == "hist2image":
                            plan["x2i_kv"][(fname, i)] = self._kv_state(
                                plan, f"{fname}.x2i{i}", f"decoder.{fname}.layers.{i}", feat, B * Z * N, D, spec.X2I_HEADS,
                                dict(groups=B * Z, NB=B * Z, Hk=1, Wk=N, th=1, tw=N, clip=(0, 1, 0, N), count_pad=False, v_length=float(N)))
        if img_features is not None:
            for f, dst in zip(img_features, plan["tap_dst"]):
                dst.torch().copy_(f.permute(0, 2, 3, 1).reshape(-1, f.shape[1]).to(device=dev, dtype=self.dtype))
        else:
            self._encoder(plan, rgb.to(device=dev, dtype=torch.float32).contiguous(), B, H, W, taps)

        pinfo = add["patch_info"]

        def fuse(name, x, feat, hh, ww, out):
            Wm = self.fusion[name][1][1]
            geo = FusionGeometry.from_patch_info(pinfo, self.base_resolution[1] / Wm)
            assert geo.zone_num * geo.zone_num == Z
            self._fusion(plan, name, x, feat, zone_valid, geo, B, hh, ww, out, pos_offsets.get(name, (0, 0)), taps)

        def up(i, src: Act, hs_, ws_, hd, wd):
            M = B * hd * wd
            t1 = self._act(plan, f"up{i}.a", M, c[i])
            fits = hd > 1 and wd > 1 and B * hd * wd * cat[i].ld * 2 < 2 ** 31 - 65536 and hs_ * ws_ * src.ld * 2 < 2 ** 31 - 65536
            if self.x3 and str(i) in self.up_fused_x3 and src.C % 32 == 0 and taps is None and hd > 1 and wd > 1:
                n = f"decoder.up{i}.a"
                ops.upsample_cat_conv3x3(src, hs_, ws_, cat[i].slice(src.C, e[i]), self.P[n + ".wcat"], self.P[n + ".s"], self.P[n + ".t"],
                                         t1, B, hd, wd, hip.ACT_LRELU, x3=True)
            elif self.half and str(i) in self.up_fused and src.C % 64 == 0 and taps is None and fits:
                n = f"decoder.up{i}.a"
                ops.upsample_cat_conv3x3(src, hs_, ws_, cat[i].slice(src.C, e[i]), self.P[n + ".w"], self.P[n + ".s"], self.P[n + ".t"],
                                         t1, B, hd, wd, hip.ACT_LRELU)
            else:
                ops.resize_bilinear(src, hs_, ws_, (0, 0, hs_, ws_), cat[i].slice(0, src.C), hd, wd, (0, 0, hd, wd), B)
                n = f"decoder.up{i}.a"
                if (n + ".wpad") in self.P and M >= 30000:
                    ops.conv2d(cat[i], self.P[n + ".wpad"], self.P[n + ".s"], self.P[n + ".t"], t1, B, hd, wd, 3, 3, 1, 1, 1, hd, wd, hip.ACT_LRELU,
                               None, self._ws(M, t1.C, 9 * cat[i].C))
                else:
                    self._cv(n, cat[i].slice(0, src.C + e[i]), t1, B, hd, wd, 3, act=hip.ACT_LRELU)
            t2 = self._act(plan, f"up{i}.b", M, c[i])
            self._cv(f"decoder.up{i}.b", t1, t2, B, hd, wd, 3, act=hip.ACT_LRELU)
            return t2

        main.wait_stream(side)
        xd4 = self._act(plan, "xd4", B * hs[4] * wsz[4], c[0])
        self._cv("decoder.conv4", b4, xd4, B, hs[4], wsz[4], 1)
        x = xd4
        ph, pw = hs[4], wsz[4]
        for i, (fname, feat) in enumerate((("cross_atten3", hfeat[2]), ("cross_atten2", hfeat[1]), ("cross_atten1", hfeat[0])), start=1):
            hh, ww = hs[4 - i], wsz[4 - i]
            t = up(i, x, ph, pw, hh, ww)
            if taps is not None:
                taps[f"up{i}"] = self._nchw(t, B, hh, ww)
            D = c[i + 1]
            dcat = self._act(plan, f"dcat{i}", B * hh * ww, 2 * D)
            self._cv(f"decoder.conv{4 - i}", t, dcat.slice(0, D), B, hh, ww, 1)
            fuse(fname, dcat.slice(0, D), feat, hh, ww, dcat.slice(D, D))
            if taps is not None:
                taps[f"conv{4 - i}"] = self._nchw(dcat.slice(0, D), B, hh, ww)
                taps[fname] = self._nchw(dcat.slice(D, D), B, hh, ww)
            x, ph, pw = dcat, hh, ww
        t = up(4, x, ph, pw, hs[0], wsz[0])
        Mh = B * hs[0] * wsz[0]
        HWh = hs[0] * wsz[0]
        unet = self._act(plan, "unet", Mh, 128)
        fused_head = self.half and self.head_fused and self.n_bins == 256 and HWh % 16 == 0 and HWh >= 128 and "conv_out.wp" in self.P
        ram = self._act(plan, "ram", Mh, 128) if (not fused_head or taps is not None) else None
        edges = out[0] if out is not None else torch.empty(B, self.n_bins + 1, dtype=torch.float32, device=dev)
        centers = self._f32(plan, "head.centers", B * self.n_bins)
        h = "depth_head"
        ns = max(1, min(64, HWh // 256))
        bsum = self._f32(plan, "head.bsum", B * ns * t.C)
        msum = self._f32(plan, "head.msum", B * 128)
        if os.environ.get("CFP_OLD_SUMS", "0") == "1":
            self._cv("decoder.conv0", t, unet, B, hs[0], wsz[0], 3)
        side.wait_stream(main)
        with torch.cuda.stream(side):
            ops.channel_sum(t, bsum, B, HWh, ns)
            ops.conv3x3_mean(bsum, ns, t, self.P["decoder.conv0.w32"], self.P["decoder.conv0.b32"], msum, B, hs[0], wsz[0], 128)
            ops.bin_regressor(msum, 1, 1.0 / HWh, self.P[h + ".w1x1"], self.P[h + ".r0.w"], self.P[h + ".r0.b"], self.P[h + ".r2.w"],
                              self.P[h + ".r2.b"], self.P[h + ".r4.w"], self.P[h + ".r4.b"], self.min_val, self.max_val, self.norm,
                              edges, centers, B, 128, 256, self.n_bins)
        if os.environ.get("CFP_OLD_SUMS", "0") != "1":
            self._cv("decoder.conv0", t, unet, B, hs[0], wsz[0], 3)
        if not fused_head:
            self._cv("depth_head.conv3x3", unet, ram, B, hs[0], wsz[0], 3)
        main.wait_stream(side)
        pred = out[1] if out is not None else torch.empty(B, 1, hs[0], wsz[0], dtype=torch.float32, device=dev)
        if out is not None:
            prob = out[2] if return_prob else None
        else:
            prob = torch.empty(B, self.n_bins, hs[0], wsz[0], dtype=self.dtype, device=dev) if return_prob else None
        if fused_head:
            ops.depth_head_fused(unet, self.P[h + ".conv3x3.w"], self.P[h + ".conv3x3.s"], self.P[h + ".conv3x3.t"], self.P["conv_out.wp"],
                                 self.P["conv_out.t"], centers, prob, pred, B, hs[0], wsz[0], ram_out=ram, ram_hilo=self.head_hilo[1])
        elif (self.half or self.x3) and self.n_bins == 256 and HWh % 8 == 0 and os.environ.get("CFP_BIN_HEAD_FUSED", "1") != "0":
            ops.bin_head_fused(ram, self.P["conv_out.w"], self.P["conv_out.t"], centers, prob, pred, B, HWh)
        else:
            logits = self._act(plan, "logits", Mh, self.n_bins)
            self._lin("conv_out.w", ram, logits, Mh, hip.ACT_NONE, None, "conv_out")
            ops.bin_softmax(logits, centers, prob, pred, B, HWh, self.n_bins)
        if taps is not None:
            taps["unet_out"] = self._nchw(unet, B, hs[0], wsz[0])
            taps["ram"] = self._nchw(ram, B, hs[0], wsz[0])
        return edges, pred, prob
```

### cfpnet_amd/hip.py

```python
from __future__ import annotations

import ctypes as C
import os
from typing import Optional

_HERE = os.path.dirname(os.path.abspath(__file__))
LIB_PATH = os.environ.get("CFP_HIP_LIB") or os.path.join(_HERE, "libcfpnet_hip.so")

F32, BF16, F16 = 0, 1, 2
F32X3 = 3
ACT_NONE, ACT_RELU, ACT_LRELU, ACT_SILU, ACT_GELU, ACT_SIGMOID = range(6)
TOF_SAMPLE_UNIFORM, TOF_SAMPLE_ICDF = 0, 1
HEAD_WOUT_HILO, HEAD_RAM_HILO = 1, 2
CONV_PER_IMAGE, CONV_W2, CONV_IN_FLIGHT, CONV_X3, CONV_WS_TICKETS = 1, 2, 4, 8, 16
CONV_TICKET_BYTES = 4096

_p, _i, _f, _sz, _ll = C.c_void_p, C.c_int, C.c_float, C.c_size_t, C.c_longlong

SIGNATURES = {
    "cfp_version": (_i, []),
    "cfp_last_error": (C.c_char_p, []),
    "cfp_conv2d_nhwc": (_i, [_p, _i, _p, _p, _p, _p, _i, _p, _i] + [_i] * 14 + [_p, _sz, _p]),
    "cfp_conv2d_nhwc_ex": (_i, [_p, _i, _p, _p, _p, _p, _i, _p, _i] + [_i] * 14 + [_p, _p, _f, _i, _p, _sz, _p]),
    "cfp_conv2d_nhwc_moments": (_i, [_p, _i, _p, _p, _p, _i] + [_i] * 13 + [_p, _sz, _p, _sz, _p, _p, _p]),
    "cfp_conv2d_ws_bytes": (_sz, [_i, _i, _i, _i]),
    "cfp_pack_w_x3_elems": (_sz, [_ll, _i]),
    "cfp_pack_w_x3": (_i, [_p, _p, _ll, _i, _p]),
    "cfp_conv2d_plan": (_i, [_i] * 8 + [_p, _p]),
    "cfp_debug_set": (_i, [_i, _i]),
    "cfp_conv2d_variant": (_i, [_i, _i]),
    "cfp_dwconv3x3_nhwc": (_i, [_p, _i, _p, _p, _p, _p, _i] + [_i] * 11 + [_p]),
    "cfp_dwconv3x3_strips": (_i, [_i] * 6),
    "cfp_dwconv3x3_launch_slots": (_i, [_i] * 10),
    "cfp_dwconv3x3_sum_nhwc": (_i, [_p, _i, _p, _p, _p, _p, _i, _p] + [_i] * 11 + [_p]),
    "cfp_se_fold": (_i, [_p, _p, _p, _p, _p, _i, _i, _i, _i, _i, _p]),
    "cfp_se_gate_fold": (_i, [_p, _i, _f, _p, _p, _p, _p, _p, _p, _i, _i, _i, _i, _i, _p]),
    "cfp_dwconv3x3_se_parts": (_i, [_i, _i, _i, _i, _i, _i]),
    "cfp_dwconv3x3_se_nhwc": (_i, [_p, _i, _p, _p, _p, _p, _i, _p, _i, _p] + [_i] * 11 + [_p]),
    "cfp_se_gate_fold2": (_i, [_p, _i, _f, _p, _p, _p, _p, _p, _i, _i, _i, _i, _i, _p]),
    "cfp_dwconv_large_nhwc": (_i, [_p, _i, _p, _p, _p, _p, _i] + [_i] * 7 + [_p]),
    "cfp_dwconv_large_toeplitz_elems": (_sz, [_i, _i]),
    "cfp_dwconv_large_toeplitz": (_i, [_p, _p, _i, _i, _i, _i, _p]),
    "cfp_dwconv_large_mfma_nhwc": (_i, [_p, _i, _p, _p, _p, _p, _i] + [_i] * 7 + [_p]),
    "cfp_channel_sum": (_i, [_p, _i, _p, _i, _i, _i, _i, _i, _p]),
    "cfp_se_hidden": (_i, [_p, _i, _f, _p, _p, _p, _i, _i, _i, _p]),
    "cfp_se_scale": (_i, [_p, _i, _p, _p, _p, _i, _i, _i, _i, _i, _p]),
    "cfp_scale_channels": (_i, [_p, _i, _p, _i, _i, _i, _i, _p]),
    "cfp_layernorm": (_i, [_p, _i, _p, _p, _f, _p, _i, _p, _i, _i, _i, _i, _p]),
    "cfp_attn_kv_ws_floats": (_sz, [_i] * 7),
    "cfp_attn_kv_reduce": (_i, [_p, _i, _p, _i, _p, _p, _p] + [_i] * 10 + [_f, _i, _i, _i, _p]),
    "cfp_attn_apply": (_i, [_p, _i, _p, _p, _p, _i] + [_i] * 9 + [_f, _f, _i, _i, _i, _p]),
    "cfp_loftr_tail": (_i, [_p, _i, _p, _p, _p, _i, _p, _i, _p, _p, _p, _p, _p, _p, _p, _p, _f] + [_i] * 5 + [_f, _f, _i, _i, _i, _p]),
    "cfp_resize_bilinear": (_i, [_p, _i] + [_i] * 6 + [_p, _i] + [_i] * 6 + [_p] + [_i] * 7 + [_p]),
    "cfp_add_rowtable": (_i, [_p, _i, _p, _p, _i] + [_i] * 8 + [_p]),
    "cfp_upsample_cat_conv3x3": (_i, [_p, _i, _i, _i, _i, _p, _i, _i, _p, _p, _p, _p, _i] + [_i] * 6 + [_p]),
    "cfp_copy_rows": (_i, [_p, _i, _p, _i, _i, _i, _i, _p]),
    "cfp_copy_rows2": (_i, [_p, _i, _p, _i, _i, _p, _i, _p, _i, _i, _i, _i, _p]),
    "cfp_rgb_to_nhwc8": (_i, [_p, _p, _i, _i, _i, _i, _p]),
    "cfp_rgb_to_nhwc8_hilo": (_i, [_p, _p, _i, _i, _i, _i, _p]),
    "cfp_scalar_to_rows8": (_i, [_p, _p, _i, _i, _p]),
    "cfp_silog_ws_bytes": (_sz, [_i, _i, _i]),
    "cfp_silog_loss_fwd": (_i, [_p, _i, _i, _p, _p, _i, _i, _i, _i, _p, _sz, _p, _p]),
    "cfp_silog_loss_bwd": (_i, [_p, _p, _f, _i, _i, _i, _i, _i, _i, _p, _p]),
    "cfp_adamw_step": (_i, [_p, _p, _p, _p, C.c_longlong, _f, _f, _f, _f, _f, _i, _p, _p]),
    "cfp_grad_clip_ws_bytes": (_sz, []),
    "cfp_grad_clip_factor": (_i, [_p, C.c_longlong, _f, _p, _sz, _p, _p]),
    "cfp_tof_hist_sim": (_i, [_p, C.c_longlong, _i, _i, _i, _i, _i, _i, _i, _p, _i, _f, _i, C.c_double, _i, _p, _p, _i, _i, _p, _p, _p, _p, _p, _p]),
    "cfp_tof_sample_points": (_i, [_p, _p, _p, _p, C.c_longlong, _i, _i, _p, _p]),
    "cfp_eval_metrics_ws_bytes": (_sz, [_i]),
    "cfp_eval_metrics": (_i, [_p, _i, _i, _p, _i, _i, _i, _i, _i, _f, _f, _p, _sz, _p, _p]),
    "cfp_conv2d_wgrad_ws_bytes": (_sz, [_i, _i, _i]),
    "cfp_grad_absmax": (_i, [_p, _i, _ll, _i, _p, _p]),
    "cfp_grad_scale": (_i, [_p, _i, _i, _i, _i, _i, _i, _p, _p, _p, _i, _p]),
    "cfp_conv2d_wgrad_x3": (_i, [_p, _i, _p, _i, _p] + [_i] * 12 + [_f, _p, _p, _sz, _p, _p]),
    "cfp_conv2d_dgrad_x3_ws_bytes": (_sz, [_i] * 6),
    "cfp_conv2d_dgrad_x3": (_i, [_p, _i, _p, _p, _i, _p, _i] + [_i] * 12 + [_p, _p, _sz, _p]),
    "cfp_pack_w_x3_blocks": (_i, [_ll, _i]),
    "cfp_pack_w_x3_batch": (_i, [_p, _p, _p, _i, _i, _p]),
    "cfp_conv2d_wgrad": (_i, [_p, _i, _p, _i, _p] + [_i] * 12 + [_f, _i, _p, _sz, _p]),
    "cfp_conv2d_wgrad_bias": (_i, [_p, _i, _p, _i, _p, _p] + [_i] * 12 + [_f, _f, _i, _p, _sz, _p]),
    "cfp_conv2d_wgrad_deferred": (_i, [_p, _i, _p, _i, _p, _p] + [_i] * 12 + [_f, _f, _i, _p, _sz, _p, _p]),
    "cfp_wgrad_reduce_jobs": (_i, [_p, _i, _p]),
    "cfp_conv2d_weight_flip": (_i, [_p, _p, _i, _i, _i, _i, _i, _p]),
    "cfp_weight_flip_blocks": (_i, [_ll]),
    "cfp_conv2d_weight_flip_batch": (_i, [_p, _p, _p, _i, _i, _i, _p]),
    "cfp_conv2d_dgrad": (_i, [_p, _i, _p, _p, _i] + [_i] * 14 + [_p, _sz, _p]),
    "cfp_bn_ws_bytes": (_sz, [_i]),
    "cfp_bn_train_stats": (_i, [_p, _i, C.c_longlong, _i, _i, _p, _p, _f, _f] + [_p] * 7 + [_p, _sz, _p]),
    "cfp_bn_train_stats_partials": (_i, [_p, _i, C.c_longlong, C.c_longlong, _i, _p, _p, _f, _f] + [_p] * 7 + [_p]),
    "cfp_scale_shift_act": (_i, [_p, _i, _p, _p, _i, _p, _i, C.c_longlong, _i, _i, _p]),
    "cfp_scale_shift_act_res": (_i, [_p, _i, _p, _p, _i, _p, _i, _p, _i, C.c_longlong, _i, _i, _p]),
    "cfp_bn_train_bwd": (_i, [_p, _i, _p, _i, C.c_longlong, _i, _i, _p, _p, _p, _p, _i, _p, _p, _p, _i, _p, _sz, _p]),
    "cfp_colsum": (_i, [_p, _i, C.c_longlong, _i, _i, _p, _p, _sz, _p]),
    "cfp_act_bwd": (_i, [_p, _i, _p, _i, _i, _p, _i, C.c_longlong, _i, _i, _p]),
    "cfp_layernorm_bwd_ws_bytes": (_sz, [C.c_longlong, _i]),
    "cfp_layernorm_bwd": (_i, [_p, _i, _p, _i, _p, _f, _p, _i, _i, _p, _p, C.c_longlong, _i, _i, _p, _sz, _p]),
    "cfp_layernorm_bwd_deferred": (_i, [_p, _i, _p, _i, _p, _f, _p, _i, _i, _p, _p, C.c_longlong, _i, _i, _p, _sz, _p, _p]),
    "cfp_axpby": (_i, [_p, _i, _p, _i, _f, _f, _p, _i, C.c_longlong, _i, _i, _p]),
    "cfp_rowtable_grad": (_i, [_p, _i, _p, _i, _i, _i, _i, _i, _i, _i, _f, _i, _p]),
    "cfp_se_train_ws_floats": (_sz, [_i, _i, _i]),
    "cfp_se_train_fwd": (_i, [_p, _i, _f] + [_p] * 7 + [_i, _i, _i, _p]),
    "cfp_se_train_bwd": (_i, [_p] * 12 + [_f, _f, _i, _i, _i, _p]),
    "cfp_channel_dot": (_i, [_p, _i, _p, _i, _p, _i, _i, _i, _i, _p]),
    "cfp_bcast_fma": (_i, [_p, _i, _p, _p, _p, _i, _i, _i, _i, _i, _p]),
    "cfp_dwconv3x3_dgrad": (_i, [_p, _i, _p, _p, _i] + [_i] * 11 + [_p]),
    "cfp_dwconv3x3_wgrad_ws_bytes": (_sz, [_i]),
    "cfp_dwconv3x3_wgrad": (_i, [_p, _i, _p, _i, _p] + [_i] * 9 + [_f, _i, _p, _sz, _p]),
    "cfp_dwconv3x3_wgrad_deferred": (_i, [_p, _i, _p, _i, _p] + [_i] * 9 + [_f, _i, _p, _sz, _p, _p]),
    "cfp_index_rows": (_i, [_p, _i, _p, _p, _i, C.c_longlong, _i, _i, _i, _p]),
    "cfp_resize_bilinear_bwd": (_i, [_p, _i, _p, _i, _i, _i, _i, _i, _i, _i, _i, _i, _p]),
    "cfp_bin_centers": (_i, [_p, _f, _f, _p, _p, _i, _i, _p]),
    "cfp_bin_centers_bwd": (_i, [_p, _f, _f, _p, _i, _i, _p]),
    "cfp_softmax_expect_ws_bytes": (_sz, [_i, _i, _i]),
    "cfp_softmax_expect": (_i, [_p, _i, _p, _p, _p, _p, _i, _p, _i, _i, _i, _i, _p, _sz, _p]),
    "cfp_linattn_state_bytes": (_sz, [_i, _i, _i]),
    "cfp_linattn_ws_bytes": (_sz, [_i, _i, _i, _i, _i]),
    "cfp_linattn_fwd": (_i, [_p, _i, _p, _i, _p, _i, _p, _i, _p, _i, _i, _i, _i, _i, _f, _i, _p, _sz, _p]),
    "cfp_linattn_bwd": (_i, [_p, _i, _p, _i, _p, _i, _p, _i, _p, _p, _i, _p, _i, _p, _i, _i, _i, _i, _i, _i, _f, _i, _p, _sz, _p]),
    "cfp_linattn_fwd_dev": (_i, [_p, _i, _p, _i, _p, _i, _p, _i, _p, _i, _i, _i, _i, _i, _f, _i, _p, _sz, _p, _p]),
    "cfp_linattn_bwd_dev": (_i, [_p, _i, _p, _i, _p, _i, _p, _i, _p, _p, _i, _p, _i, _p, _i, _i, _i, _i, _i, _i, _f, _i, _p, _sz, _p, _p]),
    "cfp_zone_crop": (_i, [_p, _i, _p, _p, _i] + [_i] * 7 + [_i, _p]),
    "cfp_zone_crop_bwd": (_i, [_p, _i, _p, _p, _i] + [_i] * 7 + [_i, _p]),
    "cfp_zone_paste": (_i, [_p, _i, _p, _i, _p, _p, _i] + [_i] * 7 + [_i, _p]),
    "cfp_zone_paste_bwd": (_i, [_p, _i, _p, _p, _i] + [_i] * 7 + [_i, _p]),
    "cfp_zone_rect_rows": (_i, [_p, _i, _p, _p, _i] + [_i] * 6 + [_i, _p]),
    "cfp_dwconv_large_wgrad_ws_bytes": (_sz, [_i, _i, _i, _i, _i]),
    "cfp_dwconv_large_wgrad": (_i, [_p, _i, _p, _i, _p, _i, _i, _i, _i, _i, _f, _i, _p, _sz, _p]),
    "cfp_row_normalize": (_i, [_p, _p, _p, _i, _i, _p]),
    "cfp_add_rowtable_dev": (_i, [_p, _i, _p, _p, _i, _i, _i, _i, _i, _i, _i, _p, _i, _p]),
    "cfp_rowtable_grad_dev": (_i, [_p, _i, _p, _i, _i, _i, _i, _i, _i, _p, _f, _i, _p]),
    "cfp_nyu_augment": (_i, [_p, _p, _i, _i, _i, _p, _p, _p, _i, _i, C.POINTER(C.c_float), C.POINTER(C.c_float), _p, _p, _p]),
    "cfp_nyu_rotate": (_i, [_p, _p, _p, _p, _i, _i, _i, _p, _p]),
    "cfp_bin_regressor": (_i, [_p, _i, _f] + [_p] * 7 + [_f, _f, _i, _p, _p, _i, _i, _i, _i, _p]),
    "cfp_bin_softmax": (_i, [_p, _i, _p, _p, _p, _i, _i, _i, _i, _p]),
    "cfp_conv3x3_mean": (_i, [_p, _i, _p, _i, _p, _p, _p, _i, _i, _i, _i, _i, _i, _p]),
    "cfp_lkpm_tail": (_i, [_p, _i, _p, _i, _p, _i, _p, _p, _p, _p, _p, _p, _f, _i, _i, _i, _p]),
    "cfp_mbconv_plan": (_i, [_i, _i, _i, _i, _i, _p, _p]),
    "cfp_mbconv_expand_dw": (_i, [_p, _i, _p, _p, _p, _p, _p, _p, _p, _i, _p, _i, _i, _i, _i, _i, _i, _p]),
    "cfp_hist_encoder": (_i, [_p, _p, _p, _p, _p, _p, _p, _p, _p, _i, _i, _i, _p]),
    "cfp_depth_head_fused": (_i, [_p, _i, _p, _p, _p, _p, _p, _p, _p, _p, _p, _i, _i, _i, _i, _i, _p]),
    "cfp_bin_head_fused": (_i, [_p, _i, _p, _p, _p, _p, _p, _i, _i, _i, _i, _p]),
}

class WgradJob(C.Structure):
    _fields_ = [("slabs", C.c_void_p), ("dw", C.c_void_p), ("db", C.c_void_p), ("n", C.c_longlong), ("n_dw", C.c_longlong),
                ("nsplit", C.c_int), ("ew", C.c_int), ("beta", C.c_float), ("beta_b", C.c_float)]


_lib: Optional[C.CDLL] = None


def load() -> C.CDLL:
    global _lib
    if _lib is not None:
        return _lib
    if not os.path.exists(LIB_PATH):
        raise RuntimeError(
            f"{LIB_PATH} not found: build the HIP extension first "
            f"(`python -c 'import __graft_entry__ as g; g.build()'` or `make -C cfpnet_amd/csrc`). "
            "There is no CPU fallback for the product path.")
    import torch
    lib = C.CDLL(LIB_PATH)
    for name, (res, args) in SIGNATURES.items():
        fn = getattr(lib, name)
        fn.restype = res
        fn.argtypes = args
    _lib = lib
    return lib


def last_error() -> str:
    return load().cfp_last_error().decode()


def call(name: str, *args):
    rc = getattr(load(), name)(*args)
    if rc != 0:
        raise RuntimeError(f"{name} failed ({rc}): {last_error()}")


def ptr(t) -> int:
    return 0 if t is None else t.data_ptr()


def current_stream() -> int:
    import torch
    return torch.cuda.current_stream().cuda_stream
```

### cfpnet_amd/ops.py

```python
from __future__ import annotations

import os
from dataclasses import dataclass
from typing import Optional, Tuple

import torch

from . import hip

DT = {torch.float32: hip.F32, torch.bfloat16: hip.BF16, torch.float16: hip.F16}


@dataclass
class Act:
    buf: torch.Tensor
    c0: int
    C: int

    @property
    def rows(self) -> int:
        return self.buf.shape[0]

    @property
    def ld(self) -> int:
        return self.buf.shape[1]

    @property
    def ptr(self) -> int:
        return self.buf.data_ptr() + self.c0 * self.buf.element_size()

    @property
    def dt(self) -> int:
        return DT[self.buf.dtype]

    def slice(self, c0: int, C: int) -> "Act":
        assert 0 <= c0 and c0 + C <= self.C
        return Act(self.buf, self.c0 + c0, C)

    def torch(self) -> torch.Tensor:
        return self.buf[:, self.c0:self.c0 + self.C]


def new_act(rows: int, C: int, dtype, device, ld: Optional[int] = None, zero: bool = False) -> Act:
    ld = ld or C
    f = torch.zeros if zero else torch.empty
    return Act(f((rows, ld), dtype=dtype, device=device), 0, C)


def _s():
    return hip.current_stream()


def ticket_ws(slab_bytes: int, device) -> torch.Tensor:
    ws = torch.zeros((hip.CONV_TICKET_BYTES + slab_bytes + 3) // 4, dtype=torch.float32, device=device)
    ws.cfp_tickets = True
    return ws


def conv2d_ws_bytes(M: int, Cout: int, K: int, dt: int) -> int:
    return int(hip.load().cfp_conv2d_ws_bytes(M, Cout, K, dt))


PLAN_IN_FLIGHT = False


def conv2d(x: Act, w: torch.Tensor, scale, shift, out: Act, B, H, W, KH, KW, stride, pad_t, pad_l, Ho, Wo,
           act=hip.ACT_NONE, residual: Optional[Act] = None, ws: Optional[torch.Tensor] = None, ln=None,
           per_image_weights: bool = False):
    tickets = getattr(ws, "cfp_tickets", False)
    assert x.rows >= B * H * W and out.rows >= B * Ho * Wo
    K = KH * KW * x.C
    wshape = (B, out.C, K) if per_image_weights else (out.C, K)
    x3 = x.buf.dtype == torch.float32 and w.dtype == torch.float16
    if x3:
        wshape = wshape[:-1] + ((K + 31) // 32 * 64,)
    w2 = (not x3) and (not per_image_weights) and KH * KW == 1 and tuple(w.shape) == (out.C, 2 * ((K + 63) // 64) * 64)
    assert (x3 or w.dtype == x.buf.dtype) and (w2 or tuple(w.shape) == wshape) and w.is_contiguous(), (w.shape, wshape)
    g, b, eps = ln if ln is not None else (None, None, 0.0)
    hip.call("cfp_conv2d_nhwc_ex", x.ptr, x.ld, w.data_ptr(), hip.ptr(scale), hip.ptr(shift),
             residual.ptr if residual else 0, residual.ld if residual else 0, out.ptr, out.ld,
             B, H, W, x.C, out.C, KH, KW, stride, pad_t, pad_l, Ho, Wo, act, x.dt,
             hip.ptr(g), hip.ptr(b), float(eps),
             int(per_image_weights) | (hip.CONV_W2 if w2 else 0) | (hip.CONV_IN_FLIGHT if PLAN_IN_FLIGHT else 0) | (hip.CONV_X3 if x3 else 0) |
             (hip.CONV_WS_TICKETS if tickets and ws is not None else 0),
             hip.ptr(ws), ws.numel() * ws.element_size() if ws is not None else 0, _s())


def conv2d_moments(x: Act, w: torch.Tensor, bias, out: Act, B, H, W, KH, KW, stride, pad_t, pad_l, Ho, Wo, ws: Optional[torch.Tensor] = None):
    import ctypes
    M = B * Ho * Wo
    assert w.dtype == x.buf.dtype and tuple(w.shape) == (out.C, KH * KW * x.C) and w.is_contiguous()
    mom = torch.empty(((M + 63) // 64) * 2 * out.C, dtype=torch.float32, device=x.buf.device)
    ns, rps = ctypes.c_int(0), ctypes.c_int(0)
    hip.call("cfp_conv2d_nhwc_moments", x.ptr, x.ld, w.data_ptr(), hip.ptr(bias), out.ptr, out.ld, B, H, W, x.C, out.C, KH, KW, stride,
             pad_t, pad_l, Ho, Wo, x.dt, hip.ptr(ws), ws.numel() * ws.element_size() if ws is not None else 0, mom.data_ptr(), mom.numel(),
             ctypes.byref(ns), ctypes.byref(rps), _s())
    return mom, ns.value, rps.value


GEN2_TILES = [(128, 128, 3), (128, 128, 2), (128, 64, 3), (128, 64, 4), (64, 64, 3), (64, 64, 4), (256, 32, 3), (256, 32, 2),
              (128, 32, 3), (128, 32, 4), (256, 16, 2), (128, 16, 4), (64, 128, 3), (64, 64, 2), (128, 64, 2), (64, 128, 2), (128, 32, 2),
              (32, 64, 3), (32, 128, 3), (64, 64, 2), (64, 64, 3), (64, 128, 2)]
X3_ONLY_TILES = [(256, 128, 2), (256, 64, 2), (64, 64, 2), (128, 64, 2), (128, 128, 2), (64, 128, 2),
                 (128, 128, 2), (128, 64, 2), (64, 64, 2), (256, 64, 2), (128, 32, 2), (256, 128, 2),
                 (64, 64, 2), (128, 32, 2), (64, 128, 2)]
X3_ADIRECT = range(28, 34)
X3_OCC = range(34, 37)
GEN1_TILES = [(256, 16), (256, 32), (128, 64), (128, 128)]
DIRECT3_TILES = [(8, 128), (8, 64), (16, 64), (16, 32), (8, 32), (16, 16)]


def conv2d_kernel_name(variant: int, splits: int, dt: int) -> str:
    t = {hip.BF16: "bf16", hip.F16: "f16"}.get(dt, "f32")
    if variant >= 500:
        n = "conv3x3_halo_x3"
    elif variant >= 400:
        bm, bn, st = (GEN2_TILES + X3_ONLY_TILES)[variant - 400]
        n = f"igemm_x3<{bm}x{bn},s{st}" + (",kg2>" if 19 <= variant - 400 <= 21 else ",ad>" if variant - 400 in X3_ADIRECT else ",occ>" if variant - 400 in X3_OCC else ">")
    elif variant >= 300:
        n = f"conv3x3_halo<{t}>"
    elif variant >= 200:
        th, bn = DIRECT3_TILES[variant - 200]
        n = f"conv3x3_direct<{t},{th}x16px,{bn}>"
    elif variant >= 100:
        bm, bn, st = GEN2_TILES[variant - 100]
        n = f"igemm2<{t},{bm}x{bn},s{st}" + (",kg2>" if variant - 100 >= 19 else ">")
    else:
        bm, bn = GEN1_TILES[variant]
        n = f"conv_igemm<{t},{bm}x{bn}>"
    return n + (f"+splitK" if splits > 1 else "")


def conv2d_plan(M: int, Cout: int, K: int, dt: int, rows_per_batch: int = 0, B: int = 1, KH: int = 1, stride: int = 1):
    import ctypes
    v, s = ctypes.c_int(0), ctypes.c_int(0)
    hip.load().cfp_conv2d_plan(M, Cout, K, KH, stride, dt, rows_per_batch, B, ctypes.byref(v), ctypes.byref(s))
    return v.value, s.value


def linear(x: Act, w: torch.Tensor, scale, shift, out: Act, rows: int, act=hip.ACT_NONE, residual: Optional[Act] = None,
           ws: Optional[torch.Tensor] = None, ln=None):
    conv2d(x, w, scale, shift, out, 1, 1, rows, 1, 1, 1, 0, 0, 1, rows, act, residual, ws, ln)


def dwconv3x3(x: Act, w, scale, shift, out: Act, B, H, W, stride, pad_t, pad_l, Ho, Wo, act):
    hip.call("cfp_dwconv3x3_nhwc", x.ptr, x.ld, w.data_ptr(), scale.data_ptr(), shift.data_ptr(), out.ptr, out.ld,
             B, H, W, x.C, stride, pad_t, pad_l, Ho, Wo, act, x.dt, _s())


def dwconv3x3_strips(B: int, Ho: int, Wo: int, C: int, stride: int, dt: int) -> int:
    return int(hip.load().cfp_dwconv3x3_strips(B, Ho, Wo, C, stride, dt))


def dwconv3x3_sum(x: Act, w, scale, shift, out: Act, partial: torch.Tensor, B, H, W, stride, pad_t, pad_l, Ho, Wo, act):
    assert partial.dtype == torch.float32 and partial.numel() >= B * dwconv3x3_strips(B, Ho, Wo, x.C, stride, x.dt) * x.C
    hip.call("cfp_dwconv3x3_sum_nhwc", x.ptr, x.ld, w.data_ptr(), scale.data_ptr(), shift.data_ptr(), out.ptr, out.ld,
             partial.data_ptr(), B, H, W, x.C, stride, pad_t, pad_l, Ho, Wo, act, x.dt, _s())


def se_fold(w_proj: torch.Tensor, w_out: torch.Tensor, hidden, we_t, be, B, Cout, C, R):
    assert w_proj.shape == (Cout, C) and w_out.shape == (B, Cout, C) and w_proj.dtype == w_out.dtype and we_t.shape == (R, C)
    hip.call("cfp_se_fold", w_proj.data_ptr(), w_out.data_ptr(), hidden.data_ptr(), we_t.data_ptr(), be.data_ptr(),
             B, Cout, C, R, DT[w_proj.dtype], _s())


def se_gate_fold(partial, nsplit, inv_hw, wr, br, we_t, be, w_proj: torch.Tensor, w_out: torch.Tensor, B, Cout, C, R):
    x3 = w_proj.dtype == torch.float32 and w_out.dtype == torch.float16
    assert w_proj.shape == (Cout, C) and w_out.shape == ((B, Cout, (C + 31) // 32 * 64) if x3 else (B, Cout, C)) and (x3 or w_proj.dtype == w_out.dtype)
    assert we_t.shape == (R, C) and wr.shape == (R, C) and partial.numel() >= B * nsplit * C
    hip.call("cfp_se_gate_fold", partial.data_ptr(), nsplit, float(inv_hw), wr.data_ptr(), br.data_ptr(), we_t.data_ptr(), be.data_ptr(),
             w_proj.data_ptr(), w_out.data_ptr(), B, Cout, C, R, hip.F32X3 if x3 else DT[w_proj.dtype], _s())


def dwconv3x3_se_parts(B: int, Ho: int, Wo: int, C: int, stride: int, dt: int) -> int:
    return int(hip.load().cfp_dwconv3x3_se_parts(B, Ho, Wo, C, stride, dt))


def dwconv3x3_se(x: Act, w, scale, shift, out: Act, w_reduce: torch.Tensor, hpart: torch.Tensor, B, H, W, stride, pad_t, pad_l, Ho, Wo, act):
    R = w_reduce.shape[0]
    assert w_reduce.dtype == torch.float32 and w_reduce.shape == (R, x.C) and hpart.dtype == torch.float32
    assert hpart.numel() >= B * dwconv3x3_se_parts(B, Ho, Wo, x.C, stride, x.dt) * R
    hip.call("cfp_dwconv3x3_se_nhwc", x.ptr, x.ld, w.data_ptr(), scale.data_ptr(), shift.data_ptr(), out.ptr, out.ld,
             w_reduce.data_ptr(), R, hpart.data_ptr(), B, H, W, x.C, stride, pad_t, pad_l, Ho, Wo, act, x.dt, _s())


def se_gate_fold2(hpart, K, inv_hw, br, we_t, be, w_proj32: torch.Tensor, w_out: torch.Tensor, B, Cout, C, R, x3: bool = False):
    assert w_proj32.shape == (Cout, C) and w_proj32.dtype == torch.float32
    assert w_out.shape == ((B, Cout, (C + 31) // 32 * 64) if x3 else (B, Cout, C)) and (not x3 or w_out.dtype == torch.float16)
    assert we_t.shape == (R, C) and hpart.dtype == torch.float32 and hpart.numel() >= B * K * R
    hip.call("cfp_se_gate_fold2", hpart.data_ptr(), K, float(inv_hw), br.data_ptr(), we_t.data_ptr(), be.data_ptr(),
             w_proj32.data_ptr(), w_out.data_ptr(), B, Cout, C, R, hip.F32X3 if x3 else DT[w_out.dtype], _s())


def dwconv_large(x: Act, w, scale, shift, out: Act, B, H, W, k, act):
    hip.call("cfp_dwconv_large_nhwc", x.ptr, x.ld, w.data_ptr(), scale.data_ptr(), shift.data_ptr(), out.ptr, out.ld,
             B, H, W, x.C, k, act, x.dt, _s())


def _bracket16(w: torch.Tensor, dtype):
    r16 = w.to(dtype)
    r = r16.float()
    bits = r16.view(torch.int16).to(torch.int32)
    toward_inf = torch.where(r >= 0, bits + 1, bits - 1)
    toward_ninf = torch.where(r > 0, bits - 1, bits + 1)
    toward_ninf = torch.where(r16.view(torch.int16) == 0, torch.full_like(bits, -32767), toward_ninf)
    toward_inf = torch.where(r16.view(torch.int16) == -32768, torch.ones_like(bits), toward_inf)
    nxt_up = toward_inf.to(torch.int16).view(dtype).float()
    nxt_dn = toward_ninf.to(torch.int16).view(dtype).float()
    up = torch.where(r >= w, r, nxt_up)
    down = torch.where(r <= w, r, nxt_dn)
    return down, up


def pack_w_x3(w2d: torch.Tensor) -> torch.Tensor:
    assert w2d.is_cuda and w2d.dtype == torch.float32 and w2d.dim() == 2 and w2d.is_contiguous()
    rows, k = w2d.shape
    out = torch.empty(rows, (k + 31) // 32 * 64, dtype=torch.float16, device=w2d.device)
    hip.call("cfp_pack_w_x3", w2d.data_ptr(), out.data_ptr(), rows, k, _s())
    if os.environ.get("CFP_X3_DIAG_TWO_TERM", "0") == "1":
        out.view(rows, -1, 2, 32)[:, :, 1, :] = 0
    return out


def pack_w2(w2d: torch.Tensor, dtype) -> torch.Tensor:
    w2d = w2d.detach().float()
    co, k = w2d.shape
    kp = (k + 63) // 64 * 64
    hi = w2d.to(dtype)
    lo = (w2d - hi.float()).to(dtype)
    out = torch.zeros(co, 2 * kp, dtype=dtype)
    out[:, :k] = hi
    out[:, kp:kp + k] = lo
    return out.contiguous()


def round_taps(w: torch.Tensor, dtype, bracket: bool = True) -> torch.Tensor:
    w = w.detach().float()
    if dtype == torch.float32 or w.shape[-1] * w.shape[-2] == 1:
        return w
    kh, kw = w.shape[-2], w.shape[-1]
    order = [r * kw + (c if r % 2 == 0 else kw - 1 - c) for r in range(kh) for c in range(kw)]
    flat = w.reshape(-1, kh * kw)
    if not bracket:
        out = torch.empty_like(flat)
        e = torch.zeros_like(flat[:, 0])
        for t in order:
            v = flat[:, t] + e
            q = v.to(dtype).float()
            e = v - q
            out[:, t] = q
        return out.reshape(w.shape)
    down, up = _bracket16(flat, dtype)
    import numpy as np
    f, dn, upn = flat.numpy(), down.numpy(), up.numpy()
    out = np.empty_like(f)
    e = np.zeros(f.shape[0], dtype=np.float32)
    for t in order:
        v = f[:, t] + e
        take_down = np.abs(v - dn[:, t]) <= np.abs(upn[:, t] - v)
        q = np.where(take_down, dn[:, t], upn[:, t])
        e = v - q
        out[:, t] = q
    return torch.from_numpy(out).reshape(w.shape)


def toeplitz_bands(w: torch.Tensor, dtype) -> torch.Tensor:
    w = w.detach().float().cpu()
    if w.dim() == 4:
        w = w[:, 0]
    w = round_taps(w, dtype)
    C, k, _ = w.shape
    halo = (k - 1) // 2
    lm = (halo + 7) // 8 * 8
    nh = (16 + lm + halo + 31) // 32
    lane = torch.arange(64)
    h = torch.arange(nh)
    e = torch.arange(8)
    kx = 32 * h[:, None, None] + 8 * (lane[None, :, None] // 16) + e[None, None, :] - (lm - halo) - (lane[None, :, None] % 16)
    ok = (kx >= 0) & (kx < k)
    g = w[:, :, kx.clamp(0, k - 1)]
    g = torch.where(ok[None, None], g, torch.zeros(()))
    assert g.numel() == int(hip.load().cfp_dwconv_large_toeplitz_elems(C, k))
    return g.contiguous().to(dtype)


def toeplitz_bands_x3(w: torch.Tensor) -> torch.Tensor:
    w = w.detach().float().cpu()
    if w.dim() == 4:
        w = w[:, 0]
    hi = w.to(torch.float16)
    lo = (w - hi.float()).to(torch.float16)
    return torch.stack([toeplitz_bands(hi.float(), torch.float16), toeplitz_bands(lo.float(), torch.float16)]).contiguous()


def toeplitz_bands_dev(w: torch.Tensor, dtype, flip: bool = False) -> torch.Tensor:
    C, k, _ = w.shape
    assert w.dtype == torch.float32 and w.is_contiguous()
    out = torch.empty(int(hip.load().cfp_dwconv_large_toeplitz_elems(C, k)), dtype=dtype, device=w.device)
    hip.call("cfp_dwconv_large_toeplitz", w.data_ptr(), out.data_ptr(), C, k, int(flip), DT[dtype], _s())
    return out


def dwconv_large_mfma(x: Act, tb: torch.Tensor, scale, shift, out: Act, B, H, W, k, act):
    x3 = x.buf.dtype == torch.float32 and tb.dtype == torch.float16
    assert not x3 or tb.shape[0] == 2
    hip.call("cfp_dwconv_large_mfma_nhwc", x.ptr, x.ld, tb.data_ptr(), scale.data_ptr(), shift.data_ptr(), out.ptr, out.ld,
             B, H, W, x.C, k, act, hip.F32X3 if x3 else x.dt, _s())


def channel_sum(x: Act, partial: torch.Tensor, B, HW, nsplit):
    assert partial.dtype == torch.float32 and partial.numel() >= B * nsplit * x.C
    hip.call("cfp_channel_sum", x.ptr, x.ld, partial.data_ptr(), B, HW, x.C, nsplit, x.dt, _s())


def se_hidden(partial, nsplit, inv_hw, wr, br, hidden, B, C, R):
    hip.call("cfp_se_hidden", partial.data_ptr(), nsplit, float(inv_hw), wr.data_ptr(), br.data_ptr(), hidden.data_ptr(),
             B, C, R, _s())


def se_scale(x: Act, hidden, we_t, be, B, HW, R):
    assert we_t.shape == (R, x.C)
    hip.call("cfp_se_scale", x.ptr, x.ld, hidden.data_ptr(), we_t.data_ptr(), be.data_ptr(), B, HW, x.C, R, x.dt, _s())


def scale_channels(x: Act, gate, B, HW):
    hip.call("cfp_scale_channels", x.ptr, x.ld, gate.data_ptr(), B, HW, x.C, x.dt, _s())


def layernorm(x: Act, gamma, beta, eps, out: Act, rows, residual: Optional[Act] = None):
    hip.call("cfp_layernorm", x.ptr, x.ld, gamma.data_ptr(), beta.data_ptr(), float(eps),
             residual.ptr if residual else 0, residual.ld if residual else 0, out.ptr, out.ld, rows, x.C, x.dt, _s())


def attn_kv_ws_floats(NB, Hk, Wk, th, tw, heads, d) -> int:
    return int(hip.load().cfp_attn_kv_ws_floats(NB, Hk, Wk, th, tw, heads, d))


def attn_kv_reduce(k: Act, v: Act, kv, ksum, ws, NB, Hk, Wk, th, tw, clip, count_pad, v_length, heads, d):
    cy0, cy1, cx0, cx1 = clip
    hip.call("cfp_attn_kv_reduce", k.ptr, k.ld, v.ptr, v.ld, kv.data_ptr(), ksum.data_ptr(), hip.ptr(ws),
             NB, Hk, Wk, th, tw, cy0, cy1, cx0, cx1, int(count_pad), float(v_length), heads, d, k.dt, _s())


def attn_apply(q: Act, kv, ksum, out: Act, NB, Hq, Wq, qth, qtw, excl, v_length, heads, d, eps=1e-6):
    ey0, ey1, ex0, ex1 = excl
    hip.call("cfp_attn_apply", q.ptr, q.ld, kv.data_ptr(), ksum.data_ptr(), out.ptr, out.ld,
             NB, Hq, Wq, qth, qtw, ey0, ey1, ex0, ex1, float(v_length), float(eps), heads, d, q.dt, _s())


def loftr_tail(q: Optional[Act], kv, ksum, x: Act, out: Act, w_q, w_merge, w_mlp0, w_mlp2, ln1, ln2, NB, Hq, Wq, qth, qtw, v_length,
               heads, eps=1e-6, ln_eps=1e-5):
    D = x.C
    x3 = x.buf.dtype == torch.float32 and w_merge.dtype == torch.float16
    assert (q is None) != (w_q is None), "loftr_tail: give either q or w_q"
    k1, k2 = (2 * D, 4 * D) if x3 else (D, 2 * D)
    assert out.C == D and w_merge.shape == (D, k1) and w_mlp0.shape == (2 * D, k2) and w_mlp2.shape == (D, k2)
    assert q is None or q.C == D
    assert w_q is None or w_q.shape == (D, k1)
    hip.call("cfp_loftr_tail", q.ptr if q is not None else None, q.ld if q is not None else 0, kv.data_ptr(), ksum.data_ptr(), x.ptr, x.ld,
             out.ptr, out.ld, w_q.data_ptr() if w_q is not None else None, w_merge.data_ptr(),
             w_mlp0.data_ptr(), w_mlp2.data_ptr(), ln1[0].data_ptr(), ln1[1].data_ptr(), ln2[0].data_ptr(), ln2[1].data_ptr(),
             float(ln_eps), NB, Hq, Wq, qth, qtw, float(v_length), float(eps), heads, D, hip.F32X3 if x3 else x.dt, _s())


def resize_bilinear(src: Act, Hs, Ws, srect, dst: Act, Hd, Wd, drect, B, zone_valid=None, zn=0, p1=0, p2=0,
                    accumulate=False):
    sy0, sx0, sh, sw = srect
    dy0, dx0, dh, dw = drect
    assert src.C == dst.C
    hip.call("cfp_resize_bilinear", src.ptr, src.ld, Hs, Ws, sy0, sx0, sh, sw, dst.ptr, dst.ld, Hd, Wd, dy0, dx0, dh, dw,
             hip.ptr(zone_valid), zn, p1, p2, int(accumulate), B, src.C, src.dt, _s())


def add_rowtable(x: Act, table, out: Act, rows, H, W, Wt, oy, ox):
    assert table.dtype == torch.float32 and table.shape[1] == x.C
    hip.call("cfp_add_rowtable", x.ptr, x.ld, table.data_ptr(), out.ptr, out.ld, rows, x.C, H, W, Wt, oy, ox, x.dt, _s())


def copy_rows(x: Act, out: Act, rows):
    hip.call("cfp_copy_rows", x.ptr, x.ld, out.ptr, out.ld, rows, x.C, x.dt, _s())


def upsample_cat_conv3x3(low: Act, Hs, Ws, skip: Act, w, scale, shift, out: Act, B, H, W, act, x3: bool = False):
    if x3:
        assert low.dt == skip.dt == out.dt == hip.F32 and w.dtype == torch.float16 and w.shape[-1] == 9 * (low.C + (skip.C + 31) // 32 * 32) * 2
        hip.call("cfp_upsample_cat_conv3x3", low.ptr, low.ld, Hs, Ws, low.C, skip.ptr, skip.ld, skip.C, w.data_ptr(),
                 hip.ptr(scale), hip.ptr(shift), out.ptr, out.ld, B, H, W, out.C, act, hip.F32X3, _s())
        return
    assert w.shape[-1] == 9 * (low.C + skip.C) and low.dt == skip.dt == out.dt
    hip.call("cfp_upsample_cat_conv3x3", low.ptr, low.ld, Hs, Ws, low.C, skip.ptr, skip.ld, skip.C, w.data_ptr(),
             hip.ptr(scale), hip.ptr(shift), out.ptr, out.ld, B, H, W, out.C, act, out.dt, _s())


def pack_w_x3_cat(w: torch.Tensor, cup: int) -> torch.Tensor:
    co, kh, kw, cin = w.shape
    assert kh == 3 and kw == 3 and cup % 32 == 0 and 0 < cup < cin
    csk = cin - cup
    pad = (csk + 31) // 32 * 32 - csk
    wp = torch.nn.functional.pad(w, (0, pad)) if pad else w
    return pack_w_x3(wp.reshape(co, 9 * (cup + csk + pad)).contiguous())


def copy_rows2(x0: Act, out0: Act, x1: Act, out1: Act, rows):
    assert x0.dt == x1.dt == out0.dt == out1.dt and out0.C == x0.C and out1.C == x1.C
    hip.call("cfp_copy_rows2", x0.ptr, x0.ld, out0.ptr, out0.ld, x0.C, x1.ptr, x1.ld, out1.ptr, out1.ld, x1.C, rows, x0.dt, _s())


def rgb_to_nhwc8(rgb: torch.Tensor, out: Act, B, H, W):
    assert rgb.dtype == torch.float32 and rgb.is_contiguous() and out.C == 8 and out.ld == 8
    hip.call("cfp_rgb_to_nhwc8", rgb.data_ptr(), out.ptr, B, H, W, out.dt, _s())


def rgb_to_nhwc8_hilo(rgb: torch.Tensor, out: Act, B, H, W):
    assert rgb.dtype == torch.float32 and rgb.is_contiguous() and out.C == 8 and out.ld == 8
    hip.call("cfp_rgb_to_nhwc8_hilo", rgb.data_ptr(), out.ptr, B, H, W, out.dt, _s())


def scalar_to_rows8(x: torch.Tensor, out: Act, rows):
    assert x.dtype == torch.float32 and x.is_contiguous() and out.C == 8 and out.ld == 8
    hip.call("cfp_scalar_to_rows8", x.data_ptr(), out.ptr, rows, out.dt, _s())


def bin_regressor(partial, nsplit, inv_hw, w1x1, w0, b0, w1, b1, w2, b2, min_val, max_val, norm, edges, centers, B, C,
                  hidden, nbins):
    hip.call("cfp_bin_regressor", partial.data_ptr(), nsplit, float(inv_hw), w1x1.data_ptr(), w0.data_ptr(), b0.data_ptr(),
             w1.data_ptr(), b1.data_ptr(), w2.data_ptr(), b2.data_ptr(), float(min_val), float(max_val), norm,
             edges.data_ptr(), centers.data_ptr(), B, C, hidden, nbins, _s())


def bin_softmax(logits: Act, centers, prob, pred, B, HW, nbins):
    hip.call("cfp_bin_softmax", logits.ptr, logits.ld, centers.data_ptr(), hip.ptr(prob), pred.data_ptr(), B, HW, nbins,
             logits.dt, _s())


def bin_head_fused(x: Act, w, bias, centers, prob, pred, B, HW):
    x3 = x.buf.dtype == torch.float32 and w.dtype == torch.float16
    assert not x3 or (tuple(w.shape) == (256, (x.C + 31) // 32 * 64) and (prob is None or prob.dtype == torch.float32))
    hip.call("cfp_bin_head_fused", x.ptr, x.ld, w.data_ptr(), bias.data_ptr(), centers.data_ptr(), hip.ptr(prob),
             pred.data_ptr(), B, HW, x.C, hip.F32X3 if x3 else x.dt, _s())


def permute_wout(w: torch.Tensor, dtype, hilo: bool = True, diffuse: bool = False) -> torch.Tensor:
    w = w.detach().float().reshape(w.shape[0], -1)
    assert w.shape == (256, 128)
    pos = torch.arange(128)
    kb, q, e = pos // 32, (pos % 32) // 8, pos % 8
    src = 32 * kb + 16 * (e // 4) + 4 * q + (e % 4)
    wp = w[:, src]
    hi = (round_taps(w.reshape(256, 1, 128), dtype).reshape(256, 128)[:, src] if diffuse else wp).to(dtype)
    planes = [hi]
    if hilo:
        planes.append((wp - hi.float()).to(dtype))
    return torch.stack(planes).contiguous()


def depth_head_fused(x: Act, w3, scale3, shift3, wout_perm: torch.Tensor, bias_out, centers, prob, pred, B, H, W, ram_out: Optional[Act] = None,
                     ram_hilo: bool = True, probe: int = 0):
    assert x.C == 128 and w3.shape == (128, 9 * 128) and wout_perm.shape[1:] == (256, 128) and wout_perm.dtype == x.buf.dtype
    flags = (hip.HEAD_WOUT_HILO if wout_perm.shape[0] == 2 else 0) | (hip.HEAD_RAM_HILO if ram_hilo else 0) | (probe << 8)
    if ram_out is not None:
        assert ram_out.ld == 128 and ram_out.C == 128
    hip.call("cfp_depth_head_fused", x.ptr, x.ld, w3.data_ptr(), hip.ptr(scale3), hip.ptr(shift3), wout_perm.data_ptr(), bias_out.data_ptr(),
             centers.data_ptr(), hip.ptr(prob), pred.data_ptr(), ram_out.ptr if ram_out is not None else 0, B, H, W, flags, x.dt, _s())


def hist_encoder(hist: torch.Tensor, blob: torch.Tensor, layout, outs, R: int, pe=(None, None, None), n_pe: int = 0):
    import ctypes
    assert hist.dtype == torch.float32 and hist.is_contiguous() and hist.numel() >= R and blob.dtype == torch.float32 and len(layout) == 9
    flat = [int(v) for row in layout for v in row]
    arr = (ctypes.c_int * len(flat))(*flat)
    for o, row in zip(outs, layout[2::3]):
        assert o.C == row[4] and o.ld == o.C and o.c0 == 0 and o.rows >= R
    for t, o in zip(pe, outs):
        assert t is None or (t.dtype == torch.float32 and tuple(t.shape) == (n_pe, o.C) and t.is_contiguous())
    hip.call("cfp_hist_encoder", hist.data_ptr(), blob.data_ptr(), ctypes.addressof(arr), outs[0].ptr, outs[1].ptr, outs[2].ptr,
             hip.ptr(pe[0]), hip.ptr(pe[1]), hip.ptr(pe[2]), n_pe, R, outs[0].dt, _s())


def conv3x3_mean(partial: torch.Tensor, nsplit, x: Act, w32: torch.Tensor, bias, msum: torch.Tensor, B, H, W, Cout):
    assert w32.dtype == torch.float32 and tuple(w32.shape) == (Cout, 9 * x.C) and msum.dtype == torch.float32 and msum.numel() >= B * Cout
    hip.call("cfp_conv3x3_mean", partial.data_ptr(), nsplit, x.ptr, x.ld, w32.data_ptr(), hip.ptr(bias), msum.data_ptr(), B, H, W, x.C, Cout, x.dt, _s())


def mbconv_plan(B, H, W, Cin, mid):
    import ctypes
    t, kp = ctypes.c_int(0), ctypes.c_int(0)
    rc = hip.load().cfp_mbconv_plan(B, H, W, Cin, mid, ctypes.byref(t), ctypes.byref(kp))
    return (t.value, kp.value) if rc == 0 else None


def pack_mbconv_pw(w2d: torch.Tensor, dtype) -> torch.Tensor:
    mid, cin = w2d.shape
    kp = (cin + 31) // 32 * 32
    out = torch.zeros(mid, kp + 8, dtype=dtype)
    out[:, :cin] = w2d.to(dtype)
    return out.contiguous()


def mbconv_expand_dw(x: Act, wpw: torch.Tensor, s1, t1, wdw: torch.Tensor, s2, t2, out: Act, partial: Optional[torch.Tensor], B, H, W):
    mid = out.C
    assert wpw.dtype == x.buf.dtype and wpw.shape[0] == mid and wdw.shape == (9, mid) and wdw.dtype == x.buf.dtype
    hip.call("cfp_mbconv_expand_dw", x.ptr, x.ld, wpw.data_ptr(), s1.data_ptr(), t1.data_ptr(), wdw.data_ptr(), s2.data_ptr(), t2.data_ptr(),
             out.ptr, out.ld, hip.ptr(partial), B, H, W, x.C, mid, x.dt, _s())


def lkpm_tail(t: Act, xin: Act, out: Act, w1, b1, w2, b2, ln_g, ln_b, rows, ln_eps=1e-6):
    D = t.C
    x3 = t.buf.dtype == torch.float32 and w1.dtype == torch.float16
    k1, k2 = (2 * D, 8 * D) if x3 else (D, 4 * D)
    assert xin.C == D and out.C == D and tuple(w1.shape) == (4 * D, k1) and tuple(w2.shape) == (D, k2) and (x3 or w1.dtype == t.buf.dtype)
    hip.call("cfp_lkpm_tail", t.ptr, t.ld, xin.ptr, xin.ld, out.ptr, out.ld, w1.data_ptr(), b1.data_ptr(), w2.data_ptr(), b2.data_ptr(),
             ln_g.data_ptr(), ln_b.data_ptr(), float(ln_eps), rows, D, hip.F32X3 if x3 else t.dt, _s())
```

### include/cfpnet_hip.h

```cpp
#ifndef CFPNET_HIP_H
#define CFPNET_HIP_H

#include <stddef.h>
#include <stdint.h>

#ifdef __cplusplus
extern "C" {
#endif

typedef void* cfp_stream_t;

enum { CFP_OK = 0, CFP_EINVAL = -1, CFP_ESHAPE = -2, CFP_EHIP = -3 };
enum { CFP_F32 = 0, CFP_BF16 = 1, CFP_F16 = 2 };
enum { CFP_F32X3 = 3 };
enum { CFP_TOF_SAMPLE_UNIFORM = 0, CFP_TOF_SAMPLE_ICDF = 1 };
enum { CFP_ACT_NONE = 0, CFP_ACT_RELU = 1, CFP_ACT_LRELU = 2, CFP_ACT_SILU = 3, CFP_ACT_GELU = 4, CFP_ACT_SIGMOID = 5 };

int cfp_version(void);
const char* cfp_last_error(void);

int cfp_conv2d_nhwc(const void* in, int in_ld, const void* w, const float* scale, const float* shift,
                    const void* residual, int res_ld, void* out, int out_ld,
                    int B, int H, int W, int Cin, int Cout, int KH, int KW, int stride,
                    int pad_t, int pad_l, int Ho, int Wo, int act, int dtype,
                    void* ws, size_t ws_bytes, cfp_stream_t stream);

enum { CFP_CONV_PER_IMAGE = 1, CFP_CONV_W2 = 2, CFP_CONV_IN_FLIGHT = 4, CFP_CONV_X3 = 8, CFP_CONV_WS_TICKETS = 16 };
#define CFP_CONV_TICKET_BYTES 4096
int cfp_conv2d_nhwc_ex(const void* in, int in_ld, const void* w, const float* scale, const float* shift,
                       const void* residual, int res_ld, void* out, int out_ld,
                       int B, int H, int W, int Cin, int Cout, int KH, int KW, int stride,
                       int pad_t, int pad_l, int Ho, int Wo, int act, int dtype,
                       const float* ln_gamma, const float* ln_beta, float ln_eps, int per_image_weights,
                       void* ws, size_t ws_bytes, cfp_stream_t stream);

size_t cfp_pack_w_x3_elems(long long rows, int K);
int cfp_pack_w_x3(const float* w, void* out, long long rows, int K, cfp_stream_t stream);

size_t cfp_conv2d_ws_bytes(int M, int Cout, int K, int dtype);

int cfp_conv2d_plan(int M, int Cout, int K, int KH, int stride, int dtype, int rows_per_batch, int B, int* variant,
                    int* splits);

int cfp_conv2d_variant(int M, int Cout);

int cfp_debug_set(int key, int value);

int cfp_dwconv3x3_nhwc(const void* in, int in_ld, const void* w, const float* scale, const float* shift,
                       void* out, int out_ld, int B, int H, int W, int C, int stride, int pad_t, int pad_l,
                       int Ho, int Wo, int act, int dtype, cfp_stream_t stream);

int cfp_dwconv3x3_strips(int B, int Ho, int Wo, int C, int stride, int dtype);
int cfp_dwconv3x3_launch_slots(int B, int H, int W, int Ho, int Wo, int C, int stride, int in_ld, int out_ld, int dtype);
int cfp_dwconv3x3_sum_nhwc(const void* in, int in_ld, const void* w, const float* scale, const float* shift,
                           void* out, int out_ld, float* partial, int B, int H, int W, int C, int stride,
                           int pad_t, int pad_l, int Ho, int Wo, int act, int dtype, cfp_stream_t stream);

int cfp_dwconv_large_nhwc(const void* in, int in_ld, const float* w, const float* scale, const float* shift,
                          void* out, int out_ld, int B, int H, int W, int C, int k, int act, int dtype,
                          cfp_stream_t stream);

size_t cfp_dwconv_large_toeplitz_elems(int C, int k);
int cfp_dwconv_large_toeplitz(const float* w, void* out, int C, int k, int flip, int dtype, cfp_stream_t stream);
int cfp_dwconv_large_mfma_nhwc(const void* in, int in_ld, const void* toeplitz, const float* scale, const float* shift,
                               void* out, int out_ld, int B, int H, int W, int C, int k, int act, int dtype,
                               cfp_stream_t stream);

int cfp_channel_sum(const void* in, int in_ld, float* partial, int B, int HW, int C, int nsplit, int dtype,
                    cfp_stream_t stream);

int cfp_se_hidden(const float* partial, int nsplit, float inv_hw, const float* w_reduce, const float* b_reduce,
                  float* hidden, int B, int C, int R, cfp_stream_t stream);

int cfp_se_scale(void* x, int ld, const float* hidden, const float* w_expand_t, const float* b_expand,
                 int B, int HW, int C, int R, int dtype, cfp_stream_t stream);

int cfp_se_fold(const void* w_proj, void* w_out, const float* hidden, const float* w_expand_t, const float* b_expand,
                int B, int Cout, int C, int R, int dtype, cfp_stream_t stream);

int cfp_mbconv_plan(int B, int H, int W, int Cin, int mid, int* tiles_per_image, int* KP);
int cfp_mbconv_expand_dw(const void* x, int x_ld, const void* wpw, const float* s1, const float* t1, const void* wdw,
                         const float* s2, const float* t2, void* out, int out_ld, float* partial, int B, int H, int W, int Cin,
                         int mid, int dtype, cfp_stream_t stream);

int cfp_se_gate_fold(const float* partial, int nsplit, float inv_hw, const float* w_reduce, const float* b_reduce,
                     const float* w_expand_t, const float* b_expand, const void* w_proj, void* w_out,
                     int B, int Cout, int C, int R, int dtype, cfp_stream_t stream);

int cfp_dwconv3x3_se_parts(int B, int Ho, int Wo, int C, int stride, int dtype);
int cfp_dwconv3x3_se_nhwc(const void* in, int in_ld, const void* w, const float* scale, const float* shift, void* out, int out_ld,
                          const float* w_reduce, int R, float* hpart, int B, int H, int W, int C, int stride, int pad_t, int pad_l,
                          int Ho, int Wo, int act, int dtype, cfp_stream_t stream);

int cfp_se_gate_fold2(const float* hpart, int K, float inv_hw, const float* b_reduce, const float* w_expand_t, const float* b_expand,
                      const float* w_proj, void* w_out, int B, int Cout, int C, int R, int dtype, cfp_stream_t stream);

int cfp_scale_channels(void* x, int ld, const float* gate, int B, int HW, int C, int dtype, cfp_stream_t stream);

int cfp_layernorm(const void* in, int in_ld, const float* gamma, const float* beta, float eps,
                  const void* residual, int res_ld, void* out, int out_ld, int rows, int C, int dtype,
                  cfp_stream_t stream);

size_t cfp_attn_kv_ws_floats(int NB, int Hk, int Wk, int th, int tw, int heads, int d);
int cfp_attn_kv_reduce(const void* k, int k_ld, const void* v, int v_ld, float* kv, float* ksum, float* ws,
                       int NB, int Hk, int Wk, int th, int tw, int cy0, int cy1, int cx0, int cx1,
                       int count_pad, float v_length, int heads, int d, int dtype, cfp_stream_t stream);

int cfp_attn_apply(const void* q, int q_ld, const float* kv, const float* ksum, void* out, int out_ld,
                   int NB, int Hq, int Wq, int qth, int qtw, int ey0, int ey1, int ex0, int ex1,
                   float v_length, float eps, int heads, int d, int dtype, cfp_stream_t stream);

int cfp_loftr_tail(const void* q, int q_ld, const float* kv, const float* ksum, const void* x, int x_ld,
                   void* out, int out_ld, const void* w_q, const void* w_merge, const void* w_mlp0, const void* w_mlp2,
                   const float* ln1_g, const float* ln1_b, const float* ln2_g, const float* ln2_b, float ln_eps,
                   int NB, int Hq, int Wq, int qth, int qtw, float v_length, float eps, int heads, int D,
                   int dtype, cfp_stream_t stream);

int cfp_resize_bilinear(const void* src, int src_ld, int Hs, int Ws, int sy0, int sx0, int sh, int sw,
                        void* dst, int dst_ld, int Hd, int Wd, int dy0, int dx0, int dh, int dw,
                        const uint8_t* zone_valid, int zn, int p1, int p2, int accumulate,
                        int B, int C, int dtype, cfp_stream_t stream);

int cfp_add_rowtable(const void* in, int in_ld, const float* table, void* out, int out_ld, int rows, int C,
                     int H, int W, int Wt, int oy, int ox, int dtype, cfp_stream_t stream);

int cfp_upsample_cat_conv3x3(const void* low, int low_ld, int Hs, int Ws, int Cup, const void* skip, int skip_ld, int Cskip,
                             const void* w, const float* scale, const float* shift, void* out, int out_ld, int B, int H, int W,
                             int Cout, int act, int dtype, cfp_stream_t stream);

int cfp_copy_rows(const void* in, int in_ld, void* out, int out_ld, int rows, int C, int dtype, cfp_stream_t stream);
int cfp_copy_rows2(const void* in0, int in0_ld, void* out0, int out0_ld, int C0, const void* in1, int in1_ld, void* out1, int out1_ld,
                   int C1, int rows, int dtype, cfp_stream_t stream);

int cfp_rgb_to_nhwc8(const float* rgb, void* out, int B, int H, int W, int dtype, cfp_stream_t stream);
int cfp_rgb_to_nhwc8_hilo(const float* rgb, void* out, int B, int H, int W, int dtype, cfp_stream_t stream);
int cfp_scalar_to_rows8(const float* in, void* out, int rows, int dtype, cfp_stream_t stream);

int cfp_hist_encoder(const float* hist, const float* blob, const int* layout, void* out0, void* out1, void* out2,
                     const float* pe0, const float* pe1, const float* pe2, int n_pe, int R, int dtype, cfp_stream_t stream);

int cfp_lkpm_tail(const void* t, int t_ld, const void* xin, int x_ld, void* out, int out_ld, const void* w1, const float* b1,
                  const void* w2, const float* b2, const float* ln_g, const float* ln_b, float ln_eps, int rows, int D, int dtype,
                  cfp_stream_t stream);

int cfp_bin_regressor(const float* partial, int nsplit, float inv_hw, const float* w1x1_t,
                      const float* w0_t, const float* b0, const float* w1_t, const float* b1,
                      const float* w2_t, const float* b2, float min_val, float max_val, int norm,
                      float* edges, float* centers, int B, int C, int hidden, int nbins, cfp_stream_t stream);

int cfp_conv3x3_mean(const float* partial, int nsplit, const void* in, int in_ld, const float* w, const float* bias, float* msum,
                     int B, int H, int W, int C, int Cout, int dtype, cfp_stream_t stream);

int cfp_bin_softmax(const void* logits, int ld, const float* centers, void* prob, float* pred,
                    int B, int HW, int nbins, int dtype, cfp_stream_t stream);

enum { CFP_HEAD_WOUT_HILO = 1, CFP_HEAD_RAM_HILO = 2 };
int cfp_depth_head_fused(const void* x, int x_ld, const void* w3, const float* scale3, const float* shift3,
                         const void* wout_perm, const float* bias_out, const float* centers, void* prob, float* pred,
                         void* ram_out, int B, int H, int W, int flags, int dtype, cfp_stream_t stream);

int cfp_bin_head_fused(const void* x, int x_ld, const void* w, const float* bias, const float* centers,
                       void* prob, float* pred, int B, int HW, int Cin, int dtype, cfp_stream_t stream);


size_t cfp_silog_ws_bytes(int B, int Ht, int Wt);
int cfp_silog_loss_fwd(const float* pred, int Hp, int Wp, const float* target, const unsigned char* mask, int Ht, int Wt,
                       int B, int interpolate, void* ws, size_t ws_bytes, float* stats, cfp_stream_t stream);
int cfp_silog_loss_bwd(const void* ws, const float* stats, float grad_loss, int Hp, int Wp, int Ht, int Wt, int B,
                       int interpolate, float* grad_pred, cfp_stream_t stream);

int cfp_adamw_step(float* param, const float* grad, float* exp_avg, float* exp_avg_sq, long long n, float lr,
                   float beta1, float beta2, float eps, float weight_decay, int step, const float* grad_scale,
                   cfp_stream_t stream);
size_t cfp_grad_clip_ws_bytes(void);
int cfp_grad_clip_factor(const float* grad, long long n, float max_norm, void* ws, size_t ws_bytes, float* out,
                         cfp_stream_t stream);


int cfp_tof_hist_sim(const float* depth, long long img_stride, int B, int H, int W, int zone_num, int zone_px, int sy0,
                     int sx0, const int* offsets, int offset_bound, float max_distance, int bins, double bin_width,
                     int floor_count, const float* w0, const float* w1, int nsamp, int sample_mode, double* fh, float* rect,
                     unsigned char* mask, float* pts, int* hist_out, cfp_stream_t stream);
int cfp_tof_sample_points(const double* fh, const unsigned char* mask, const float* w0, const float* w1, long long nzones,
                          int nsamp, int sample_mode, float* pts, cfp_stream_t stream);

size_t cfp_eval_metrics_ws_bytes(int B);
int cfp_eval_metrics(const float* pred, int Hp, int Wp, const float* gt, int H, int W, int B, int interpolate, int mode,
                     float lo, float hi, void* ws, size_t ws_bytes, double* out, cfp_stream_t stream);


size_t cfp_conv2d_wgrad_ws_bytes(int Cout, int K, int M);
int cfp_conv2d_wgrad(const void* x, int x_ld, const void* dy, int dy_ld, float* dw, int B, int H, int W, int Cin, int Cout,
                     int KH, int KW, int stride, int pad_t, int pad_l, int Ho, int Wo, float beta, int dtype, void* ws,
                     size_t ws_bytes, cfp_stream_t stream);
int cfp_conv2d_wgrad_bias(const void* x, int x_ld, const void* dy, int dy_ld, float* dw, float* db, int B, int H, int W, int Cin,
                          int Cout, int KH, int KW, int stride, int pad_t, int pad_l, int Ho, int Wo, float beta, float beta_b,
                          int dtype, void* ws, size_t ws_bytes, cfp_stream_t stream);
typedef struct cfp_wgrad_job {
  const float* slabs; float* dw; float* db;
  long long n, n_dw;
  int nsplit, ew;
  float beta, beta_b;
} cfp_wgrad_job;
int cfp_conv2d_wgrad_deferred(const void* x, int x_ld, const void* dy, int dy_ld, float* dw, float* db, int B, int H, int W, int Cin,
                              int Cout, int KH, int KW, int stride, int pad_t, int pad_l, int Ho, int Wo, float beta, float beta_b,
                              int dtype, void* ws, size_t ws_bytes, cfp_wgrad_job* job, cfp_stream_t stream);
int cfp_wgrad_reduce_jobs(const cfp_wgrad_job* jobs, int njobs, cfp_stream_t stream);
int cfp_dwconv3x3_wgrad_deferred(const void* x, int x_ld, const void* dy, int dy_ld, float* dw, int B, int H, int W, int C, int stride,
                                 int pad_t, int pad_l, int Ho, int Wo, float beta, int dtype, void* ws, size_t ws_bytes,
                                 cfp_wgrad_job* job, cfp_stream_t stream);
int cfp_layernorm_bwd_deferred(const void* x, int ld, const void* dy, int dy_ld, const float* gamma, float eps, void* dx, int dx_ld,
                               int accumulate, float* dgamma, float* dbeta, long long rows, int C, int dtype, void* ws, size_t ws_bytes,
                               cfp_wgrad_job* job, cfp_stream_t stream);
int cfp_conv2d_weight_flip(const void* w, void* wt, int Cout, int KH, int KW, int Cin, int dtype, cfp_stream_t stream);
int cfp_weight_flip_blocks(long long elems);
int cfp_conv2d_weight_flip_batch(const void* src_base, void* dst_base, const long long* desc, int n, int total_blocks, int dtype,
                                 cfp_stream_t stream);
int cfp_conv2d_dgrad(const void* dy, int dy_ld, const void* wt, void* dx, int dx_ld, int B, int H, int W, int Cin, int Cout,
                     int KH, int KW, int stride, int pad_t, int pad_l, int Ho, int Wo, int accumulate, int dtype, void* ws,
                     size_t ws_bytes, cfp_stream_t stream);

int cfp_grad_absmax(const float* x, int ld, long long rows, int C, int* dy_scale, cfp_stream_t stream);
int cfp_grad_scale(const float* dy, int ld, int B, int Ho, int Wo, int C, int dil, const int* dy_scale, float* out, float* inv, int n_inv,
                   cfp_stream_t stream);
int cfp_conv2d_wgrad_x3(const float* x, int x_ld, const float* dy, int dy_ld, float* dw, int B, int H, int W, int Cin, int Cout,
                        int KH, int KW, int stride, int pad_t, int pad_l, int Ho, int Wo, float beta, const int* dy_scale, void* ws,
                        size_t ws_bytes, cfp_wgrad_job* job, cfp_stream_t stream);
size_t cfp_conv2d_dgrad_x3_ws_bytes(int B, int Ho, int Wo, int Cout, int Cin, int stride);
int cfp_conv2d_dgrad_x3(const float* dy, int dy_ld, const void* wt, const float* res, int res_ld, float* dx, int dx_ld, int B, int H, int W,
                        int Cin, int Cout, int KH, int KW, int stride, int pad_t, int pad_l, int Ho, int Wo, const int* dy_scale,
                        void* ws, size_t ws_bytes, cfp_stream_t stream);
int cfp_pack_w_x3_blocks(long long rows, int K);
int cfp_pack_w_x3_batch(const float* src_base, void* dst_base, const long long* desc, int n, int total_blocks, cfp_stream_t stream);

int cfp_conv2d_nhwc_moments(const void* in, int in_ld, const void* w, const float* bias, void* out, int out_ld, int B, int H, int W,
                            int Cin, int Cout, int KH, int KW, int stride, int pad_t, int pad_l, int Ho, int Wo, int dtype,
                            void* ws, size_t ws_bytes, float* mom, size_t mom_floats, int* nsplit, int* rows_per_split,
                            cfp_stream_t stream);
int cfp_bn_train_stats_partials(const float* partial, int nsplit, long long rows, long long rows_per_split, int C, const float* gamma,
                                const float* beta, float eps, float momentum, float* running_mean, float* running_var, float* mean,
                                float* var, float* invstd, float* scale, float* shift, cfp_stream_t stream);

size_t cfp_bn_ws_bytes(int C);
int cfp_bn_train_stats(const void* x, int ld, long long rows, int C, int dtype, const float* gamma, const float* beta, float eps,
                       float momentum, float* running_mean, float* running_var, float* mean, float* var, float* invstd,
                       float* scale, float* shift, void* ws, size_t ws_bytes, cfp_stream_t stream);
int cfp_scale_shift_act(const void* x, int ld, const float* scale, const float* shift, int act, void* out, int out_ld,
                        long long rows, int C, int dtype, cfp_stream_t stream);
int cfp_scale_shift_act_res(const void* x, int ld, const float* scale, const float* shift, int act, const void* res, int res_ld,
                            void* out, int out_ld, long long rows, int C, int dtype, cfp_stream_t stream);
int cfp_bn_train_bwd(const void* x, int ld, const void* dy, int dy_ld, long long rows, int C, int dtype, const float* mean,
                     const float* invstd, const float* scale, const float* shift, int act, float* dgamma, float* dbeta,
                     void* dx, int dx_ld, void* ws, size_t ws_bytes, cfp_stream_t stream);

int cfp_colsum(const void* x, int ld, long long rows, int C, int dtype, float* out, void* ws, size_t ws_bytes, cfp_stream_t stream);
int cfp_act_bwd(const void* z, int ld, const void* dy, int dy_ld, int act, void* dz, int dz_ld, long long rows, int C, int dtype,
                cfp_stream_t stream);
size_t cfp_layernorm_bwd_ws_bytes(long long rows, int C);
int cfp_layernorm_bwd(const void* x, int ld, const void* dy, int dy_ld, const float* gamma, float eps, void* dx, int dx_ld,
                      int accumulate, float* dgamma, float* dbeta, long long rows, int C, int dtype, void* ws, size_t ws_bytes,
                      cfp_stream_t stream);

int cfp_axpby(const void* x, int x_ld, const void* y, int y_ld, float a, float b, void* out, int out_ld, long long rows, int C,
              int dtype, cfp_stream_t stream);
int cfp_rowtable_grad(const void* dx, int ld, float* dtable, int B, int H, int W, int C, int Wt, int oy, int ox, float beta,
                      int dtype, cfp_stream_t stream);
size_t cfp_se_train_ws_floats(int B, int C, int Rp);
int cfp_se_train_fwd(const float* partial, int nsplit, float inv_hw, const float* w1, const float* b1, const float* w2, const float* b2,
                     float* mean, float* z1, float* gate, int B, int C, int Rp, cfp_stream_t stream);
int cfp_se_train_bwd(const float* dgate, const float* gate, const float* z1, const float* mean, const float* w1, const float* w2,
                     float* dw1, float* db1, float* dw2, float* db2, float* add, float* ws, float inv_hw, float beta, int B, int C,
                     int Rp, cfp_stream_t stream);
int cfp_channel_dot(const void* x, int x_ld, const void* y, int y_ld, float* out, int B, int HW, int C, int dtype, cfp_stream_t stream);
int cfp_bcast_fma(const void* dy, int dy_ld, const float* gate, const float* add, void* dx, int dx_ld, int B, int HW, int C, int dtype,
                  cfp_stream_t stream);
int cfp_dwconv3x3_dgrad(const void* dy, int dy_ld, const void* w, void* dx, int dx_ld, int B, int H, int W, int C, int stride,
                        int pad_t, int pad_l, int Ho, int Wo, int accumulate, int dtype, cfp_stream_t stream);
size_t cfp_dwconv3x3_wgrad_ws_bytes(int C);
int cfp_dwconv3x3_wgrad(const void* x, int x_ld, const void* dy, int dy_ld, float* dw, int B, int H, int W, int C, int stride,
                        int pad_t, int pad_l, int Ho, int Wo, float beta, int dtype, void* ws, size_t ws_bytes, cfp_stream_t stream);

int cfp_index_rows(const void* x, int x_ld, const int* idx, void* out, int out_ld, long long n_out, int C, int accumulate, int dtype,
                   cfp_stream_t stream);
int cfp_resize_bilinear_bwd(const void* dy, int dy_ld, void* dx, int dx_ld, int B, int Hs, int Ws, int Hd, int Wd, int C,
                            int accumulate, int dtype, cfp_stream_t stream);
int cfp_bin_centers(const float* widths_normed, float min_val, float max_val, float* edges, float* centers, int B, int NB,
                    cfp_stream_t stream);
int cfp_bin_centers_bwd(const float* dcenters, float min_val, float max_val, float* dwidths_normed, int B, int NB, cfp_stream_t stream);
size_t cfp_softmax_expect_ws_bytes(int B, int HW, int NB);
int cfp_softmax_expect(const void* logits, int ld, const float* centers, float* pred, const float* dpred, void* dlogits, int dl_ld,
                       float* dcenters, int B, int HW, int NB, int dtype, void* ws, size_t ws_bytes, cfp_stream_t stream);

size_t cfp_linattn_state_bytes(int N, int heads, int d);
size_t cfp_linattn_ws_bytes(int N, int L, int S, int heads, int d);
int cfp_linattn_fwd(const void* q, int q_ld, const void* k, int k_ld, const void* v, int v_ld, void* out, int out_ld, float* state,
                    int N, int L, int S, int heads, int d, float eps, int dtype, void* ws, size_t ws_bytes, cfp_stream_t stream);
int cfp_linattn_bwd(const void* q, int q_ld, const void* k, int k_ld, const void* v, int v_ld, const void* dout, int do_ld,
                    const float* state, void* dq, int dq_ld, void* dk, int dk_ld, void* dv, int dv_ld, int N, int L, int S,
                    int heads, int d, float eps, int dtype, void* ws, size_t ws_bytes, cfp_stream_t stream);
int cfp_linattn_fwd_dev(const void* q, int q_ld, const void* k, int k_ld, const void* v, int v_ld, void* out, int out_ld, float* state,
                        int N, int L, int S, int heads, int d, float eps, int dtype, void* ws, size_t ws_bytes, const int* s_dev,
                        cfp_stream_t stream);
int cfp_linattn_bwd_dev(const void* q, int q_ld, const void* k, int k_ld, const void* v, int v_ld, const void* dout, int do_ld,
                        const float* state, void* dq, int dq_ld, void* dk, int dk_ld, void* dv, int dv_ld, int N, int L, int S,
                        int heads, int d, float eps, int dtype, void* ws, size_t ws_bytes, const int* s_dev, cfp_stream_t stream);

int cfp_zone_crop(const void* tok, int tok_ld, const int* rec, void* out, int out_ld, int B, int H, int W, int C, int zn, int p1, int p2,
                  int dtype, cfp_stream_t stream);
int cfp_zone_crop_bwd(const void* dz, int dz_ld, const int* rec, void* dtok, int dtok_ld, int B, int H, int W, int C, int zn, int p1, int p2,
                      int dtype, cfp_stream_t stream);
int cfp_zone_paste(const void* tok, int tok_ld, const void* z, int z_ld, const int* rec, void* out, int out_ld, int B, int H, int W, int C,
                   int zn, int p1, int p2, int dtype, cfp_stream_t stream);
int cfp_zone_paste_bwd(const void* dy, int dy_ld, const int* rec, void* dz, int dz_ld, int B, int H, int W, int C, int zn, int p1, int p2,
                       int dtype, cfp_stream_t stream);
int cfp_zone_rect_rows(const void* x, int x_ld, const int* rec, void* out, int out_ld, int B, int H, int W, int C, int cap, int mode,
                       int dtype, cfp_stream_t stream);

size_t cfp_dwconv_large_wgrad_ws_bytes(int B, int H, int W, int C, int k);
int cfp_dwconv_large_wgrad(const void* x, int x_ld, const void* dy, int dy_ld, float* dw, int B, int H, int W, int C, int k, float beta,
                           int dtype, void* ws, size_t ws_bytes, cfp_stream_t stream);

int cfp_row_normalize(const float* x, const float* dy, float* out, int rows, int C, cfp_stream_t stream);

int cfp_add_rowtable_dev(const void* in, int in_ld, const float* table, void* out, int out_ld, int rows, int C, int H, int W,
                         int Ht, int Wt, const int* oyox, int dtype, cfp_stream_t stream);
int cfp_rowtable_grad_dev(const void* dx, int ld, float* dtable, int B, int H, int W, int C, int Ht, int Wt, const int* oyox,
                          float beta, int dtype, cfp_stream_t stream);

int cfp_nyu_augment(const unsigned char* rgb_u8, const unsigned short* depth_mm, int B, int H0, int W0, const int* params_i,
                    const float* params_f, const double* colors, int H, int W, const float* mean3, const float* std3, float* image_out,
                    float* depth_out, cfp_stream_t stream);

int cfp_nyu_rotate(const unsigned char* rgb_u8, const unsigned short* depth_mm, unsigned char* rgb_out, unsigned short* depth_out,
                   int B, int H, int W, const double* matrices, cfp_stream_t stream);

#ifdef __cplusplus
}
#endif
#endif
```

Measured before the change: 3740 maps/s.

## Fuse 3x3 expand conv with following 1x1 projection in the halo kernel

Adds a PW variant of the halo 3x3 implicit-GEMM kernel. After the 3x3 accumulation it applies the BN and activation, stages the mid tile in LDS, and runs a second MFMA 1x1 GEMM using weights prefetched into the freed weight stage, with an optional residual add. The engine routes EfficientNet 'er' blocks and the decoder up3.b plus conv1 pair through it, removing the round trip of the mid activation through global memory and one launch per block. In exchange it uses more LDS, forces two pipeline stages, limits the shapes it accepts, and rounds the mid tensor to bf16 in LDS as before.

```diff
diff --git a/cfpnet_amd/csrc/conv3x3_halo.hip b/cfpnet_amd/csrc/conv3x3_halo.hip
--- a/cfpnet_amd/csrc/conv3x3_halo.hip
+++ b/cfpnet_amd/csrc/conv3x3_halo.hip
@@ -1,3 +1,5 @@
+#include <algorithm>
+
 #include "igemm_core.h"
 
 namespace {
@@ -17,9 +19,16 @@
   int tiles_x, tiles_y;
   int n_blocks;
   FastDiv dcpt;
+  const void* w2;
+  const float* scale2;
+  const float* shift2;
+  int Cout2, Kp;
+  float slope2;
+  int w2_kb;
+  int koff;
 };
 
-template <typename H, int NT, int WN, int STAGES, bool UP = false, int STRIDE = 1>
+template <typename H, int NT, int WN, int STAGES, bool UP = false, int STRIDE = 1, bool PW = false>
 __global__ __launch_bounds__(256, 2) void conv3x3_halo_kernel(ConvP p, HaloP hp) {
   constexpr int WM = 4 / WN;
   constexpr int TH = 4 * WM;
@@ -32,6 +41,7 @@
   constexpr int WSTAGE = NPAD * 128;
   constexpr int LB = UP ? 4 : 6;
   static_assert((STAGES - 2) * NB <= 63, "vmcnt field");
+  static_assert(!PW || (STAGES == 2 && !UP && WN <= 2), "the fused 1x1 takes stage 0 of two weight stages");
   extern __shared__ __attribute__((aligned(16))) unsigned char smem[];
   unsigned char* sW = smem;
   unsigned char* sX = smem + STAGES * WSTAGE;
@@ -75,9 +85,24 @@
       glds16(ok ? b_ptr[j] + kk : zsrc, s + ((j * 4 + wave) % NBG) * 1024);
     }
   };
+  const int sb = PW ? (nk & 1) : 0;
+  auto issue_w2 = [&](int buf) {
+    const unsigned char* g = reinterpret_cast<const unsigned char*>(hp.w2) + lane * 16;
+    for (int i = wave; i < hp.w2_kb; i += 4) glds16(g + i * 1024, sW + buf * WSTAGE + i * 1024);
+  };
 #pragma unroll
   for (int s = 0; s < STAGES - 1; ++s)
-    if (s < nk) issue(s, s);
+    if (s < nk) issue(s, (s + sb) % STAGES);
+
+  float* sK = reinterpret_cast<float*>(smem + hp.koff);
+  float k_sc = 1.f, k_sh = 0.f, k_sc2 = 1.f, k_sh2 = 0.f;
+  static_assert(!PW || NPAD <= 256, "one channel per thread");
+  if constexpr (PW) {
+    if (tid < p.Cout && p.scale) k_sc = p.scale[tid];
+    if (tid < p.Cout && p.shift) k_sh = p.shift[tid];
+    if (tid < hp.Cout2 && hp.scale2) k_sc2 = hp.scale2[tid];
+    if (tid < hp.Cout2 && hp.shift2) k_sh2 = hp.shift2[tid];
+  }
 
   {
     const int nitems = HPIX * hp.CPT;
@@ -139,6 +164,11 @@
     }
   }
 
+  if constexpr (PW) {
+    if (tid < NPAD) { sK[tid] = k_sc; sK[NPAD + tid] = k_sh; }
+    if (tid < 64) { sK[2 * NPAD + tid] = k_sc2; sK[2 * NPAD + 64 + tid] = k_sh2; }
+  }
+
   f32x4 acc[4][NT];
 #pragma unroll
   for (int g = 0; g < 4; ++g)
@@ -158,7 +188,7 @@
   const int growb = STRIDE * HC * hp.PP;
 
   for (int ks = 0; ks < nk; ++ks) {
-    const int buf = ks % STAGES;
+    const int buf = (ks + sb) % STAGES;
     const int ahead = min(nk - 1 - ks, STAGES - 2);
     if (ahead >= 2) wait_vmcnt<(STAGES > 3 ? 2 : 1) * NB>();
     else if (ahead == 1) wait_vmcnt<NB>();
@@ -166,7 +196,8 @@
     asm volatile("s_waitcnt lgkmcnt(0)" ::: "memory");
     __builtin_amdgcn_s_barrier();
     asm volatile("" ::: "memory");
-    if (ks + STAGES - 1 < nk) issue(ks + STAGES - 1, (ks + STAGES - 1) % STAGES);
+    if (ks + STAGES - 1 < nk) issue(ks + STAGES - 1, (ks + STAGES - 1 + sb) % STAGES);
+    else if constexpr (PW) issue_w2(0);
     const unsigned char* cW = sW + buf * WSTAGE + (wn * NT * 16) * 128;
 #pragma unroll
     for (int s = 0; s < 2; ++s) {
@@ -190,6 +221,117 @@
         if (++c_dx == 3) { c_dx = 0; c_off += (HC - 3) * hp.PP; }
       }
     }
+  }
+
+  if constexpr (PW) {
+    H* __restrict__ out = reinterpret_cast<H*>(p.out) + (long long)b * p.Ho * p.Wo * p.out_ld;
+    const H* __restrict__ res = p.res ? reinterpret_cast<const H*>(p.res) + (long long)b * p.Ho * p.Wo * p.res_ld : nullptr;
+    const int x = x0 + fr;
+    constexpr int NG = WN == 2 ? 2 : 4;
+    const int g0 = WN == 2 ? 2 * wn : 0;
+    uint2 pk[4][NT];
+    {
+      f32x4 sc[NT], sh[NT];
+#pragma unroll
+      for (int j = 0; j < NT; ++j) {
+        const int n = (wn * NT + j) * 16 + fq * 4;
+        sc[j] = *reinterpret_cast<const f32x4*>(sK + n);
+        sh[j] = *reinterpret_cast<const f32x4*>(sK + NPAD + n);
+      }
+      with_act(p.act, [&](auto A) {
+#pragma unroll
+        for (int g = 0; g < 4; ++g)
+#pragma unroll
+          for (int j = 0; j < NT; ++j) {
+            float yv[4];
+#pragma unroll
+            for (int r = 0; r < 4; ++r) yv[r] = act_c16<decltype(A)::value>(acc[g][j][r] * sc[j][r] + sh[j][r]);
+            pk[g][j].x = pack2<H>(yv[0], yv[1]);
+            pk[g][j].y = pack2<H>(yv[2], yv[3]);
+          }
+      });
+    }
+    asm volatile("s_waitcnt lgkmcnt(0)" ::: "memory");
+    __builtin_amdgcn_s_barrier();
+    asm volatile("" ::: "memory");
+    const int mpitch = hp.Kp * 2 + 16;
+    unsigned char* sM = smem + hp.w2_kb * 1024;
+#pragma unroll
+    for (int g = 0; g < 4; ++g)
+#pragma unroll
+      for (int j = 0; j < NT; ++j) {
+        const int n = (wn * NT + j) * 16 + fq * 4;
+        if (n < hp.Kp) *reinterpret_cast<uint2*>(sM + ((wm * 4 + g) * 16 + fr) * mpitch + n * 2) = pk[g][j];
+      }
+    wait_vmcnt<0>();
+    asm volatile("s_waitcnt lgkmcnt(0)" ::: "memory");
+    __builtin_amdgcn_s_barrier();
+    asm volatile("" ::: "memory");
+    uint2 rres[NG][4];
+#pragma unroll
+    for (int gi = 0; gi < NG; ++gi)
+#pragma unroll
+      for (int ti = 0; ti < 4; ++ti) {
+        const int y = y0 + wm * 4 + g0 + gi, n = ti * 16 + fq * 4;
+        rres[gi][ti] = (res && y < p.Ho && x < p.Wo && n < hp.Cout2) ? *reinterpret_cast<const uint2*>(res + ((long long)y * p.Wo + x) * p.res_ld + n) : uint2{0u, 0u};
+      }
+    const int t2n = (hp.Cout2 + 15) >> 4;
+    const int rowb = hp.Kp * 2;
+
+    f32x4 fin[NG][4];
+#pragma unroll
+    for (int gi = 0; gi < NG; ++gi)
+#pragma unroll
+      for (int ti = 0; ti < 4; ++ti) fin[gi][ti] = f32x4{0.f, 0.f, 0.f, 0.f};
+    const unsigned char* mrow = sM + ((wm * 4 + g0) * 16 + fr) * mpitch + fq * 16;
+    const unsigned char* wrow = smem + fr * rowb + fq * 16;
+#pragma unroll
+    for (int kb = 0; kb < NPAD / 32; ++kb) {
+      if (kb * 32 >= hp.Kp) continue;
+      s16x8 bfr[NG];
+#pragma unroll
+      for (int gi = 0; gi < NG; ++gi) bfr[gi] = *reinterpret_cast<const s16x8*>(mrow + gi * 16 * mpitch + kb * 64);
+#pragma unroll
+      for (int ti = 0; ti < 4; ++ti) {
+        if (ti >= t2n) continue;
+        const s16x8 af = *reinterpret_cast<const s16x8*>(wrow + ti * 16 * rowb + kb * 64);
+#pragma unroll
+        for (int gi = 0; gi < NG; ++gi) fin[gi][ti] = mfma16<H>(af, bfr[gi], fin[gi][ti]);
+      }
+    }
+
+#pragma unroll
+    for (int ti = 0; ti < 4; ++ti) {
+      const int n = ti * 16 + fq * 4;
+      if (n >= hp.Cout2) continue;
+      const f32x4 sc2 = *reinterpret_cast<const f32x4*>(sK + 2 * NPAD + n);
+      const f32x4 sh2 = *reinterpret_cast<const f32x4*>(sK + 2 * NPAD + 64 + n);
+#pragma unroll
+      for (int gi = 0; gi < NG; ++gi) {
+        const int y = y0 + wm * 4 + g0 + gi;
+        if (!(y < p.Ho && x < p.Wo)) continue;
+        const long long pix = (long long)y * p.Wo + x;
+        float yv[4];
+#pragma unroll
+        for (int r = 0; r < 4; ++r) {
+          const float v = fin[gi][ti][r] * sc2[r] + sh2[r];
+          yv[r] = v > 0.f ? v : v * hp.slope2;
+        }
+        uint2 o2;
+        o2.x = pack2<H>(yv[0], yv[1]);
+        o2.y = pack2<H>(yv[2], yv[3]);
+        if (res) {
+          const H* ph = reinterpret_cast<const H*>(&o2);
+          const H* rh = reinterpret_cast<const H*>(&rres[gi][ti]);
+          H oh[4];
+#pragma unroll
+          for (int r = 0; r < 4; ++r) oh[r] = from_f32<H>(to_f32<H>(ph[r]) + to_f32<H>(rh[r]));
+          o2 = *reinterpret_cast<const uint2*>(oh);
+        }
+        *reinterpret_cast<uint2*>(out + pix * p.out_ld + n) = o2;
+      }
+    }
+    return;
   }
 
   H* __restrict__ out = reinterpret_cast<H*>(p.out) + (long long)b * p.Ho * p.Wo * p.out_ld;
@@ -253,11 +395,18 @@
 };
 constexpr int kNumHCfg = sizeof(kHCfg) / sizeof(kHCfg[0]);
 
-template <typename H, int NT, int WN, bool UP = false, int STRIDE = 1>
-int launch_h(const ConvP& p, hipStream_t s) {
+static size_t pw_lds_body(int npad, int th, size_t halo, int mid, int cout2) {
+  const size_t kp = (size_t)cdiv(mid, 32) * 32;
+  const size_t tail = (size_t)cdiv(cout2, 16) * 16 * kp * 2 + (size_t)th * 16 * (kp * 2 + 16);
+  return std::max((size_t)2 * npad * 128 + halo, tail);
+}
+static size_t pw_const_bytes(int npad) { return (size_t)(2 * npad + 128) * 4; }
+
+template <typename H, int NT, int WN, bool UP = false, int STRIDE = 1, bool PW = false>
+int launch_h(const ConvP& p, hipStream_t s, const ConvPwP* pw = nullptr) {
   constexpr int TH = 4 * (4 / WN);
   constexpr int NPAD = NT * WN * 16;
-  HaloP hp;
+  HaloP hp{};
   hp.n_blocks = cdiv(p.Cout, NPAD);
   hp.CPT = p.Cin / 8;
   hp.dcpt = make_fastdiv((unsigned)hp.CPT);
@@ -269,19 +418,28 @@
   hp.PP = slots * 16;
   hp.tiles_x = cdiv(p.Wo, 16); hp.tiles_y = cdiv(p.Ho, TH);
   const int hpix = ((TH - 1) * STRIDE + 3) * (15 * STRIDE + 3);
-  const size_t halo = (size_t)hpix * hp.PP;
+  size_t halo = (size_t)hpix * hp.PP;
+  if constexpr (PW) {
+    if (!pw || hp.n_blocks != 1 || pw->Cout2 > 64 || pw->Cout2 % 8 != 0) return -1;
+    hp.w2 = pw->w2; hp.scale2 = pw->scale2; hp.shift2 = pw->shift2; hp.Cout2 = pw->Cout2; hp.slope2 = pw->act2 == CFP_ACT_LRELU ? 0.01f : 1.f;
+    hp.Kp = cdiv(p.Cout, 32) * 32;
+    hp.w2_kb = cdiv(pw->Cout2, 16) * 16 * hp.Kp * 2 / 1024;
+    if ((size_t)hp.w2_kb * 1024 > (size_t)NPAD * 128) return -1;
+    hp.koff = (int)pw_lds_body(NPAD, TH, halo, p.Cout, pw->Cout2);
+    halo = (size_t)hp.koff - (size_t)2 * NPAD * 128 + pw_const_bytes(NPAD);
+  }
   const long long tiles = (long long)p.B * hp.tiles_x * hp.tiles_y * hp.n_blocks;
-  int stages = g_halo_stages ? g_halo_stages : 2;
+  int stages = g_halo_stages && !PW ? g_halo_stages : 2;
   const size_t lds = (size_t)stages * NPAD * 128 + halo;
   if (lds > 160 * 1024 || tiles >= (1ll << 31)) return -1;
 #define HL(ST)                                                                                                                      \
   do {                                                                                                                              \
-    auto k = conv3x3_halo_kernel<H, NT, WN, ST, UP, STRIDE>;                                                                        \
+    auto k = conv3x3_halo_kernel<H, NT, WN, ST, UP, STRIDE, PW>;                                                                      \
     static bool attr = false;                                                                                                       \
     if (!attr) { if (hipFuncSetAttribute((const void*)k, hipFuncAttributeMaxDynamicSharedMemorySize, 160 * 1024) != hipSuccess) return -2; attr = true; } \
     hipLaunchKernelGGL(k, dim3((unsigned)tiles), dim3(256), lds, s, p, hp);                                                         \
   } while (0)
-  if constexpr (UP || STRIDE != 1) { HL(2); } else { if (stages == 4) HL(4); else if (stages == 3) HL(3); else HL(2); }
+  if constexpr (UP || STRIDE != 1 || PW) { HL(2); } else { if (stages == 4) HL(4); else if (stages == 3) HL(3); else HL(2); }
 #undef HL
   return 0;
 }
@@ -351,3 +509,60 @@
   }
 #undef HV
 }
+
+int conv3x3_pw_variant(int Cin, int mid, int Cout2, int stride) {
+  if (Cin < 8 || Cin > 128 || Cin % 8 != 0 || mid < 8 || mid % 8 != 0 || Cout2 < 8 || Cout2 > 64 || Cout2 % 8 != 0 || (stride != 1 && stride != 2)) return -1;
+  const int v = mid <= 64 ? 2 : mid <= 160 ? 5 : mid <= 224 ? 6 : -1;
+  if (v < 0 || (stride == 2 && v == 6)) return -1;
+  const int wn = kHCfg[v].wn, npad = kHCfg[v].nt * wn * 16, th = 4 * (4 / wn);
+  if ((size_t)cdiv(Cout2, 16) * 16 * (cdiv(mid, 32) * 32) * 2 > (size_t)npad * 128) return -1;
+  int slots = Cin / 8;
+  if (stride == 1 && slots > 1) { while ((slots & 3) != 2) ++slots; }
+  else if ((slots & 1) == 0) ++slots;
+  const size_t halo = (size_t)((th - 1) * stride + 3) * (15 * stride + 3) * slots * 16;
+  return pw_lds_body(npad, th, halo, mid, Cout2) + pw_const_bytes(npad) <= 160 * 1024 ? v : -1;
+}
+
+int conv3x3_pw_launch(const ConvP& p, const ConvPwP& pw, hipStream_t s) {
+  const int v = conv3x3_pw_variant(p.Cin, p.Cout, pw.Cout2, p.stride);
+  if (v < 0 || !conv3x3_halo_takes(p) || p.up_src != nullptr) return -3;
+#define HP(NT, WN, ST) (p.f16 ? launch_h<f16_t, NT, WN, false, ST, true>(p, s, &pw) : launch_h<bf16_t, NT, WN, false, ST, true>(p, s, &pw))
+  if (p.stride == 2) return v == 2 ? HP(4, 1, 2) : HP(5, 2, 2);
+  return v == 2 ? HP(4, 1, 1) : v == 5 ? HP(5, 2, 1) : HP(7, 2, 1);
+#undef HP
+}
+
+extern "C" int cfp_conv3x3_pw_fused_variant(int Cin, int Cmid, int Cout, int stride, int dtype) {
+  return is16(dtype) ? conv3x3_pw_variant(Cin, Cmid, Cout, stride) : -1;
+}
+
+extern "C" int cfp_conv3x3_pw_fused(const void* in, int in_ld, const void* w1, const float* scale1, const float* shift1, int act1,
+                                    const void* w2_pad, const float* scale2, const float* shift2, int act2, const void* residual, int res_ld,
+                                    void* out, int out_ld, int B, int H, int W, int Cin, int Cmid, int Cout, int stride, int pad_t, int pad_l,
+                                    int Ho, int Wo, int dtype, cfp_stream_t stream) {
+  CFP_REQUIRE(in && w1 && w2_pad && out, CFP_EINVAL, "cfp_conv3x3_pw_fused: null pointer");
+  CFP_REQUIRE(is16(dtype), CFP_EINVAL, "cfp_conv3x3_pw_fused: bf16 / f16 storage only");
+  CFP_REQUIRE(act1 >= CFP_ACT_NONE && act1 <= CFP_ACT_SIGMOID && (act2 == CFP_ACT_NONE || act2 == CFP_ACT_LRELU), CFP_EINVAL,
+              "cfp_conv3x3_pw_fused: bad activation (the 1x1 takes CFP_ACT_NONE or CFP_ACT_LRELU)");
+  CFP_REQUIRE(B > 0 && H > 0 && W > 0 && Ho > 0 && Wo > 0 && Cin > 0 && Cmid > 0 && Cout > 0, CFP_ESHAPE, "cfp_conv3x3_pw_fused: non-positive dimension");
+  CFP_REQUIRE(cfp_conv3x3_pw_fused_variant(Cin, Cmid, Cout, stride, dtype) >= 0, CFP_ESHAPE,
+              "cfp_conv3x3_pw_fused: shape not taken (cfp_conv3x3_pw_fused_variant: Cin % 8 == 0 and <= 128, Cmid % 8 == 0 and <= 224 (160 at stride 2), "
+              "Cout % 8 == 0 and <= 64, stride 1 or 2, the 1x1 weights within one weight stage)");
+  CFP_REQUIRE(in_ld % 8 == 0 && in_ld >= Cin && out_ld % 8 == 0 && out_ld >= Cout && (!residual || (res_ld % 8 == 0 && res_ld >= Cout)), CFP_ESHAPE,
+              "cfp_conv3x3_pw_fused: row pitches must be multiples of the 16-byte vector and cover the channels");
+  CFP_REQUIRE(pad_t >= 0 && pad_l >= 0 && pad_t <= 2 && pad_l <= 2 && (Ho - 1) * stride - pad_t + 2 < H + 3 && (Wo - 1) * stride - pad_l + 2 < W + 3, CFP_ESHAPE,
+              "cfp_conv3x3_pw_fused: output size inconsistent with input size");
+  CFP_REQUIRE((long long)B * Ho * Wo < (1ll << 31) && (long long)H * W * in_ld < (1ll << 31), CFP_ESHAPE, "cfp_conv3x3_pw_fused: problem too large");
+  CFP_REQUIRE(aligned16(in) && aligned16(w1) && aligned16(w2_pad) && aligned16(out) && aligned16(residual) && aligned16(scale1) && aligned16(shift1) &&
+                  aligned16(scale2) && aligned16(shift2), CFP_EINVAL, "cfp_conv3x3_pw_fused: pointers must be 16-byte aligned");
+  ConvP p{};
+  p.in = in; p.w = w1; p.out = out; p.res = residual; p.scale = scale1; p.shift = shift1;
+  p.in_ld = in_ld; p.out_ld = out_ld; p.res_ld = res_ld;
+  p.B = B; p.H = H; p.W = W; p.Cin = Cin; p.Ho = Ho; p.Wo = Wo; p.Cout = Cmid;
+  p.KH = 3; p.KW = 3; p.stride = stride; p.pad_t = pad_t; p.pad_l = pad_l;
+  p.M = B * Ho * Wo; p.K = 9 * Cin; p.act = act1; p.f16 = dtype == CFP_F16; p.dil = 1;
+  ConvPwP pw{w2_pad, scale2, shift2, Cout, act2};
+  const int rc = conv3x3_pw_launch(p, pw, reinterpret_cast<hipStream_t>(stream));
+  CFP_REQUIRE(rc == 0, CFP_EHIP, "cfp_conv3x3_pw_fused: kernel launch failed");
+  return cfp_check_launch("cfp_conv3x3_pw_fused");
+}
diff --git a/cfpnet_amd/csrc/igemm_core.h b/cfpnet_amd/csrc/igemm_core.h
--- a/cfpnet_amd/csrc/igemm_core.h
+++ b/cfpnet_amd/csrc/igemm_core.h
@@ -54,6 +54,14 @@
 void conv3x3_halo_debug_odd_pitch(int v);
 bool conv3x3_halo_takes(const ConvP& p);
 int conv3x3_halo_launch(int v, const ConvP& p, hipStream_t s);
+struct ConvPwP {
+  const void* w2;
+  const float* scale2;
+  const float* shift2;
+  int Cout2, act2;
+};
+int conv3x3_pw_variant(int Cin, int mid, int Cout2, int stride);
+int conv3x3_pw_launch(const ConvP& p, const ConvPwP& pw, hipStream_t s);
 
 template <typename T, int BN, int NTHR>
 __device__ __forceinline__ void tile_moments(const T* sC, int CP, int rows_valid, int n0, int Cout, float* __restrict__ mom_tile, int tid) {
diff --git a/cfpnet_amd/engine.py b/cfpnet_amd/engine.py
--- a/cfpnet_amd/engine.py
+++ b/cfpnet_amd/engine.py
@@ -109,6 +109,7 @@
         self.lkpm_min_rows = int(os.environ.get("CFP_LKPM_MIN_ROWS", "30000"))
         self.sr_ln_fused = os.environ.get("CFP_SR_LN_FUSED", "1") == "1"
         self.head_fused = os.environ.get("CFP_HEAD_FUSED", "1") != "0"
+        self.er_fused = os.environ.get("CFP_ER_FUSED", "12")
         hl = os.environ.get("CFP_HEAD_HILO", "00")
         self.head_hilo = (hl[0] == "1", hl[1] == "1")
         self.half = dtype in (torch.bfloat16, torch.float16)
@@ -203,6 +204,8 @@
             elif b.kind == "er":
                 self._conv(sd, q + ".exp", q + ".conv_exp.weight", bn=q + ".bn1", eps=EPS)
                 self._conv(sd, q + ".pwl", q + ".conv_pwl.weight", bn=q + ".bn2", eps=EPS)
+                if self.half and not self.weights2:
+                    self.P[q + ".pwl.wp"] = ops.pad_pw_w(self.P[q + ".pwl.w"])
             else:
                 self._conv(sd, q + ".pw", q + ".conv_pw.weight", bn=q + ".bn1", eps=EPS)
                 if self.half and self.mbconv_fused and b.stride == 1 and not self.weights2:
@@ -250,6 +253,8 @@
             self._conv(sd, f"{d}.up{i}.b", q + ".3.weight", q + ".3.bias", bn=q + ".4")
         for n in ("conv3", "conv2", "conv1", "conv0"):
             self._conv(sd, f"{d}.{n}", f"{d}.{n}.weight", f"{d}.{n}.bias")
+        if self.half and not self.weights2:
+            self.P[d + ".conv1.wp"] = ops.pad_pw_w(self.P[d + ".conv1.w"])
         for name in self.fusion:
             q = f"{d}.{name}"
             self.P[q + ".pe"] = self._dev(sd[q + ".positional_encodings"])
@@ -379,10 +384,16 @@
             if b.kind == "cn":
                 self._cv(q + ".conv", x, out, B, h, w, 3, b.stride, pads, hip.ACT_SILU, res)
             elif b.kind == "er":
-                mid = self._act(plan, f"enc{bi}.mid", B * ho * wo, b.mid)
-                self._cv(q + ".exp", x, mid, B, h, w, 3, b.stride, pads, hip.ACT_SILU)
-                self._dbg(f"enc{bi}.mid", mid)
-                self._cv(q + ".pwl", mid, out, B, ho, wo, 1, 1, None, hip.ACT_NONE, res)
+                if (self.half and (q + ".pwl.wp") in self.P and ("1" if b.stride == 1 else "2") in self.er_fused and taps is None
+                        and not self._dbg_round and ops.conv3x3_pw_fused_variant(x.C, b.mid, b.cout, b.stride, ops.DT[self.dtype]) >= 0):
+                    ops.conv3x3_pw_fused(x, self.P[q + ".exp.w"], self.P[q + ".exp.s"], self.P[q + ".exp.t"], hip.ACT_SILU, self.P[q + ".pwl.wp"],
+                                         self.P[q + ".pwl.s"], self.P[q + ".pwl.t"], out, B, h, w, b.stride, pads[0][0], pads[1][0], ho, wo,
+                                         hip.ACT_NONE, res)
+                else:
+                    mid = self._act(plan, f"enc{bi}.mid", B * ho * wo, b.mid)
+                    self._cv(q + ".exp", x, mid, B, h, w, 3, b.stride, pads, hip.ACT_SILU)
+                    self._dbg(f"enc{bi}.mid", mid)
+                    self._cv(q + ".pwl", mid, out, B, ho, wo, 1, 1, None, hip.ACT_NONE, res)
             else:
                 mid2 = self._act(plan, f"enc{bi}.dw", B * ho * wo, b.mid)
                 mbp = ops.mbconv_plan(B, h, w, x.C, b.mid) if (q + ".pw.wimg") in self.P else None
@@ -951,7 +962,7 @@
             assert geo.zone_num * geo.zone_num == Z
             self._fusion(plan, name, x, feat, zone_valid, geo, B, hh, ww, out, pos_offsets.get(name, (0, 0)), taps)
 
-        def up(i, src: Act, hs_, ws_, hd, wd):
+        def up(i, src: Act, hs_, ws_, hd, wd, first_only=False):
             M = B * hd * wd
             t1 = self._act(plan, f"up{i}.a", M, c[i])
             fits = hd > 1 and wd > 1 and B * hd * wd * cat[i].ld * 2 < 2 ** 31 - 65536 and hs_ * ws_ * src.ld * 2 < 2 ** 31 - 65536
@@ -971,6 +982,8 @@
                                None, self._ws(M, t1.C, 9 * cat[i].C))
                 else:
                     self._cv(n, cat[i].slice(0, src.C + e[i]), t1, B, hd, wd, 3, act=hip.ACT_LRELU)
+            if first_only:
+                return t1
             t2 = self._act(plan, f"up{i}.b", M, c[i])
             self._cv(f"decoder.up{i}.b", t1, t2, B, hd, wd, 3, act=hip.ACT_LRELU)
             return t2
@@ -982,12 +995,19 @@
         ph, pw = hs[4], wsz[4]
         for i, (fname, feat) in enumerate((("cross_atten3", hfeat[2]), ("cross_atten2", hfeat[1]), ("cross_atten1", hfeat[0])), start=1):
             hh, ww = hs[4 - i], wsz[4 - i]
-            t = up(i, x, ph, pw, hh, ww)
-            if taps is not None:
-                taps[f"up{i}"] = self._nchw(t, B, hh, ww)
             D = c[i + 1]
             dcat = self._act(plan, f"dcat{i}", B * hh * ww, 2 * D)
-            self._cv(f"decoder.conv{4 - i}", t, dcat.slice(0, D), B, hh, ww, 1)
+            n3, n1 = f"decoder.up{i}.b", f"decoder.conv{4 - i}"
+            if (i == 3 and self.half and (n1 + ".wp") in self.P and "d" in self.er_fused and taps is None
+                    and ops.conv3x3_pw_fused_variant(c[i], c[i], D, 1, ops.DT[self.dtype]) >= 0):
+                t1 = up(i, x, ph, pw, hh, ww, first_only=True)
+                ops.conv3x3_pw_fused(t1, self.P[n3 + ".w"], self.P[n3 + ".s"], self.P[n3 + ".t"], hip.ACT_LRELU, self.P[n1 + ".wp"],
+                                     self.P[n1 + ".s"], self.P[n1 + ".t"], dcat.slice(0, D), B, hh, ww, 1, 1, 1, hh, ww)
+            else:
+                t = up(i, x, ph, pw, hh, ww)
+                if taps is not None:
+                    taps[f"up{i}"] = self._nchw(t, B, hh, ww)
+                self._cv(n1, t, dcat.slice(0, D), B, hh, ww, 1)
             fuse(fname, dcat.slice(0, D), feat, hh, ww, dcat.slice(D, D))
             if taps is not None:
                 taps[f"conv{4 - i}"] = self._nchw(dcat.slice(0, D), B, hh, ww)
diff --git a/cfpnet_amd/hip.py b/cfpnet_amd/hip.py
--- a/cfpnet_amd/hip.py
+++ b/cfpnet_amd/hip.py
@@ -137,6 +137,8 @@
     "cfp_lkpm_tail": (_i, [_p, _i, _p, _i, _p, _i, _p, _p, _p, _p, _p, _p, _f, _i, _i, _i, _p]),
     "cfp_mbconv_plan": (_i, [_i, _i, _i, _i, _i, _p, _p]),
     "cfp_mbconv_expand_dw": (_i, [_p, _i, _p, _p, _p, _p, _p, _p, _p, _i, _p, _i, _i, _i, _i, _i, _i, _p]),
+    "cfp_conv3x3_pw_fused_variant": (_i, [_i] * 5),
+    "cfp_conv3x3_pw_fused": (_i, [_p, _i, _p, _p, _p, _i, _p, _p, _p, _i, _p, _i, _p, _i] + [_i] * 12 + [_p]),
     "cfp_hist_encoder": (_i, [_p, _p, _p, _p, _p, _p, _p, _p, _p, _i, _i, _i, _p]),
     "cfp_depth_head_fused": (_i, [_p, _i, _p, _p, _p, _p, _p, _p, _p, _p, _p, _i, _i, _i, _i, _i, _p]),
     "cfp_bin_head_fused": (_i, [_p, _i, _p, _p, _p, _p, _p, _i, _i, _i, _i, _p]),
diff --git a/cfpnet_amd/ops.py b/cfpnet_amd/ops.py
--- a/cfpnet_amd/ops.py
+++ b/cfpnet_amd/ops.py
@@ -443,15 +443,42 @@
 def permute_wout(w: torch.Tensor, dtype, hilo: bool = True, diffuse: bool = False) -> torch.Tensor:
     w = w.detach().float().reshape(w.shape[0], -1)
     assert w.shape == (256, 128)
-    pos = torch.arange(128)
-    kb, q, e = pos // 32, (pos % 32) // 8, pos % 8
-    src = 32 * kb + 16 * (e // 4) + 4 * q + (e % 4)
+    src = pw_k_order(128)
     wp = w[:, src]
     hi = (round_taps(w.reshape(256, 1, 128), dtype).reshape(256, 128)[:, src] if diffuse else wp).to(dtype)
     planes = [hi]
     if hilo:
         planes.append((wp - hi.float()).to(dtype))
     return torch.stack(planes).contiguous()
+
+
+def pw_k_order(K: int) -> torch.Tensor:
+    pos = torch.arange((K + 31) // 32 * 32)
+    kb, q, e = pos // 32, (pos % 32) // 8, pos % 8
+    src = 32 * kb + 16 * (e // 4) + 4 * q + (e % 4)
+    return torch.where(src < K, src, torch.full_like(src, -1))
+
+
+def pad_pw_w(w: torch.Tensor) -> torch.Tensor:
+    co, K = w.shape
+    out = torch.zeros((co + 15) // 16 * 16, (K + 31) // 32 * 32, dtype=w.dtype, device=w.device)
+    out[:co, :K] = w
+    return out.contiguous()
+
+
+def conv3x3_pw_fused_variant(Cin: int, Cmid: int, Cout: int, stride: int, dt: int) -> int:
+    return int(hip.load().cfp_conv3x3_pw_fused_variant(Cin, Cmid, Cout, stride, dt))
+
+
+def conv3x3_pw_fused(x: Act, w1: torch.Tensor, s1, t1, act1, w2_pad: torch.Tensor, s2, t2, out: Act, B, H, W, stride, pad_t, pad_l, Ho, Wo,
+                     act2=hip.ACT_NONE, residual: Optional[Act] = None):
+    mid = w1.shape[0]
+    assert x.rows >= B * H * W and out.rows >= B * Ho * Wo and x.dt == out.dt
+    assert w1.dtype == x.buf.dtype and tuple(w1.shape) == (mid, 9 * x.C) and w1.is_contiguous()
+    assert w2_pad.dtype == x.buf.dtype and tuple(w2_pad.shape) == ((out.C + 15) // 16 * 16, (mid + 31) // 32 * 32) and w2_pad.is_contiguous()
+    hip.call("cfp_conv3x3_pw_fused", x.ptr, x.ld, w1.data_ptr(), hip.ptr(s1), hip.ptr(t1), act1, w2_pad.data_ptr(), hip.ptr(s2), hip.ptr(t2), act2,
+             residual.ptr if residual else 0, residual.ld if residual else 0, out.ptr, out.ld, B, H, W, x.C, mid, out.C, stride, pad_t, pad_l,
+             Ho, Wo, x.dt, _s())
 
 
 def depth_head_fused(x: Act, w3, scale3, shift3, wout_perm: torch.Tensor, bias_out, centers, prob, pred, B, H, W, ram_out: Optional[Act] = None,
diff --git a/include/cfpnet_hip.h b/include/cfpnet_hip.h
--- a/include/cfpnet_hip.h
+++ b/include/cfpnet_hip.h
@@ -82,6 +82,12 @@
 int cfp_mbconv_expand_dw(const void* x, int x_ld, const void* wpw, const float* s1, const float* t1, const void* wdw,
                          const float* s2, const float* t2, void* out, int out_ld, float* partial, int B, int H, int W, int Cin,
                          int mid, int dtype, cfp_stream_t stream);
+
+int cfp_conv3x3_pw_fused_variant(int Cin, int Cmid, int Cout, int stride, int dtype);
+int cfp_conv3x3_pw_fused(const void* in, int in_ld, const void* w1, const float* scale1, const float* shift1, int act1,
+                         const void* w2_pad, const float* scale2, const float* shift2, int act2, const void* residual, int res_ld,
+                         void* out, int out_ld, int B, int H, int W, int Cin, int Cmid, int Cout, int stride, int pad_t, int pad_l,
+                         int Ho, int Wo, int dtype, cfp_stream_t stream);
 
 int cfp_se_gate_fold(const float* partial, int nsplit, float inv_hw, const float* w_reduce, const float* b_reduce,
                      const float* w_expand_t, const float* b_expand, const void* w_proj, void* w_out,
```

Result: faster. 3819 maps/s (median of 6 runs) (+2.1%).
